# apple/ml-stable-diffusion

Measured on AMD Instinct MI355X. Metric: diffusion iter/s (UNet steps/s), SD2.1-base 512x512 fp16, higher is better.
Workload: dtype fp16; 1 GPU; BASELINE config 2: SD2.1-base (865.9 M-parameter UNet), random-init, denoising iteration at 512x512 (64x64 latents), CFG batch 2 per prompt, DDIM, device-resident loop; unet=sd21-base, latent=64, attention=ORIGINAL, prompts_per_gpu=1, global_batch=2, hip_graph=True, parallelism=dp1 (independent prompts per rank, no data-path collective)

## Files before the change

### include/sd_mi355x.h

```cpp
#ifndef SD_MI355X_H
#define SD_MI355X_H

#include <stddef.h>
#include <stdint.h>

#ifdef __cplusplus
extern "C" {
#endif

typedef enum sd_status {
  SD_OK = 0,
  SD_ERR_INVALID_ARGUMENT = -1,
  SD_ERR_NOT_FOUND = -2,
  SD_ERR_HIP = -3,
  SD_ERR_UNSUPPORTED = -4,
  SD_ERR_INTERNAL = -5
} sd_status;

typedef enum sd_dtype { SD_F16 = 0, SD_F32 = 1 } sd_dtype;

typedef enum sd_attention_impl {
  SD_ATTN_ORIGINAL = 0,
  SD_ATTN_SPLIT_EINSUM = 1,
  SD_ATTN_SPLIT_EINSUM_V2 = 2
// ... 154 lines not shown
                      const void* res, void* out, int B, int Cin, int C1, int H, int W, int Cout, int ksize, int upsample, int nw,
                      int* plan_out, int iters, float* ms);
int sd_op_w8a8_pack(const int8_t* wq, int Cout, int Ctot, int ksize, int8_t* stream, size_t* bytes);
int sd_op_conv2d_w8a8_halo(const void* x, const void* x1, const int8_t* wq, const float* w_scale, float act_absmax, const float* bias,
                           const float* temb, const void* res, void* out, int B, int Cin, int C1, int H, int W, int Cout, int upsample,
                           int staging, int splitk, int* plan_out, int iters, float* ms);
int sd_op_w8a8_pack_halo(const int8_t* wq, int Cout, int Ctot, int8_t* packed, size_t* bytes);
int sd_op_subpixel_fold(const void* w, int w_f32, int Cout, int Cin, void* folded, size_t* halves);
int sd_op_subpixel_refusal(int ksize, int stride, int up, int C0, int C1, int N, int B, int Hi, int Wi, int out_mode, char* text, int text_bytes);
int sd_op_conv2d_subpixel(const void* x, const void* w, const float* bias, const void* res, void* out, int B, int Cin, int H, int W, int Cout,
                          int splitk, int staging, int* plan_out, int iters, float* ms);
int sd_op_gemm_w8a8(const void* x, const int8_t* wq, const float* w_scale, float act_absmax, const float* bias, const void* res, void* out, int B,
                    int Cin, int H, int W, int Cout, int bm, int* plan_out, int iters, float* ms);
int sd_op_w8a8_pack_gemm(const int8_t* wq, int Cout, int K, int8_t* packed, size_t* bytes);
int sd_op_layernorm_q8(const void* x, const float* ln_weight, const float* ln_bias, float act_absmax, float eps, int8_t* xq, int M, int C,
                       int iters, float* ms);
int sd_op_geglu_w8a8(const int8_t* xq, const int8_t* wq, const float* w_scale, float act_absmax, const float* bias, void* out, int M, int C,
                     int N2, int bm, int* plan_out, int iters, float* ms);
int sd_op_w8a8_pack_geglu(const int8_t* wq, int N2, int K, int8_t* packed, size_t* bytes);
int sd_op_qkv_w8a8(const int8_t* xq, const int8_t* wq, const float* w_scale, float act_absmax, const float* bias, void* out_qk, void* out_vt,
                   int B, int HW, int C, float q_scale, int vt_perm, int bm, int* plan_out, int iters, float* ms);
int sd_op_w8a8_pack_qkv(const int8_t* wq, int C, int8_t* packed, size_t* bytes);
int sd_op_quantize_weight(const float* w, int Cout, size_t per_row, int8_t* q, float* w_scale, double* sq_err);
int sd_op_absmax(const void* x, size_t n, float* absmax);
int sd_op_gemm_palettized(const void* x, const void* lut, int nbits, const uint8_t* indices, const float* bias, const void* res, void* out,
                          int B, int Cin, int H, int W, int Cout, int bm, int* plan_out, int iters, float* ms);
int sd_op_palette_pack_gemm(const uint8_t* indices, int Cout, int K, int nbits, uint8_t* stream, size_t* bytes);
int sd_op_geglu_palettized(const void* x, const float* ln_weight, const float* ln_bias, const void* lut, int nbits, const uint8_t* indices,
                           const float* bias, void* out, int M, int C, int N2, float eps, int bm, int* plan_out, int iters, float* ms);
int sd_op_palette_pack_geglu(const uint8_t* indices, int N2, int K, int nbits, uint8_t* stream, size_t* bytes);
int sd_op_conv2d_groupnorm(const void* x, const void* w, const float* bias, const void* res, const float* gn_weight,
                           const float* gn_bias, void* conv_out, void* out, int B, int Cin, int H, int W, int Cout, int ksize,
                           int groups, float eps, int silu, int tile, int producer_stats, int* entries, int iters, float* ms);
int sd_op_conv2d_groupnorm_proj(const void* x, const void* w, const float* bias, const void* res, const float* gn_weight,
                                const float* gn_bias, const void* proj_w, const float* proj_bias, void* conv_out, void* out, int B,
                                int Cin, int H, int W, int Cout, int ksize, int Nproj, int groups, float eps, int fold, int tile,
                                int* entries, int iters, float* ms);
int sd_op_conv2d_groupnorm_conv3x3(const void* x, const void* w, const float* bias, const void* res, const float* gn_weight,
                                   const float* gn_bias, const void* w2, const float* bias2, const void* res2, void* conv_out, void* out,
                                   int B, int Cin, int H, int W, int Cout, int ksize, int N2, int groups, float eps, int silu, int fold,
                                   int tile, int staging2, int* entries, int iters, float* ms);
int sd_op_ffn_out_proj(const void* g, const void* w1, const float* b1, const void* res1, const void* w2, const float* b2, const void* res2,
                       void* out, float* gn_sums, int B, int C, int S, int groups, int fused, int iters, float* ms);
int sd_op_fold_linear(const void* wp, const float* bp, const void* w2, const float* b2, void* wm_out, float* bm_out, int N, int J, int K);
int sd_op_cross_attention_fused(const void* x, const float* ln_weight, const float* ln_bias, const void* wq, const void* k,
                                const void* v, void* out, int B, int heads, int Sq, int Sk, float eps, int nst, int iters,
                                float* ms);
int sd_op_cross_attention_block(const void* x, const float* ln_weight, const float* ln_bias, const void* wq, const void* k, const void* v,
                                const void* wo, const float* bo, const void* a1, const void* wo1, const float* bo1, void* out, int B, int heads,
                                int Sq, int Sk, float eps, int fused, int iters, float* ms);
int sd_op_geglu(const void* x, const void* w, const float* bias, void* out, int M, int C, int N2, int iters, float* ms);
int sd_op_geglu_ln(const void* x, const float* ln_weight, const float* ln_bias, const void* w, const float* bias, void* out, int M, int C,
                   int N2, float eps, int kernel, int iters, float* ms);
int sd_op_qkv_ln(const void* x, const float* ln_weight, const float* ln_bias, const void* w, void* out_qk, void* out_vt, int B, int HW, int C,
                 float eps, float q_scale, int vt_perm, int kernel, int iters, float* ms);
int sd_op_gn_proj_qkv(const void* x_in, const void* conv_w, const float* gn_weight, const float* gn_bias, const void* proj_w,
                      const float* proj_bias, const float* ln_weight, const float* ln_bias, const void* wqkv, void* out_h, void* out_qk,
                      void* out_vt, int B, int H, int W, int C, int groups, float gn_eps, float ln_eps, float q_scale, int vt_perm, int fused,
                      int* entries, int iters, float* ms);
int sd_op_timestep_embedding(const float* t, float* out, int n, int dim, int flip_sin_to_cos, float freq_shift);
int sd_op_posterior_noise(const float* moments, const float* eps, const float* noise, float* out, int Cz, int h, int w, int n_images,
                          float scale_factor, float sa, float sb, int iters, float* ms);
int sd_op_sched_step(const float* noise_pred, float* latents, float* hist, const float* coef, const float* pred, const float* step_noise,
                     float guidance, int cfg, int history, int n_images, int n, float* denoised, int* step_after);
int sd_op_conv_plan(int ksize, int stride, int up, int C0, int C1, int N, int B, int Ho, int Wo, int out_mode, int flags, int n_trans,
                    int n_twins, int gnf_groups, int tile, int staging, int splitk, int copies, int* plan, unsigned long long* workspace_bytes);
int sd_op_conv_plan_kernel(int ksize, int stride, int up, int C0, int C1, int N, int B, int Ho, int Wo, int out_mode, int flags, int n_trans,
                           int n_twins, int gnf_groups, int tile, int staging, int splitk, int copies, char* text, int text_bytes);
int sd_numpy_randn(uint32_t seed, double* out, size_t n);
int sd_torch_randn(uint32_t seed, double* out, size_t n);
int sd_philox_randn(uint64_t seed, uint32_t offset, double* out, size_t n);
int sd_calibrate(int device, float* out9);
int sd_selftest_mfma(void);

typedef struct sd_safety_checker_config {
  int32_t batch, image_size , patch_size , hidden_size, intermediate_size,
          num_hidden_layers, num_attention_heads, projection_dim, num_concepts ,
          num_special , hidden_act ;
  float layer_norm_eps;
  int32_t use_graph;
} sd_safety_checker_config;
typedef struct sd_safety_checker sd_safety_checker;
int sd_safety_checker_create(const sd_safety_checker_config* cfg, const sd_weights* w, int device, sd_safety_checker** out);
void sd_safety_checker_destroy(sd_safety_checker* c);
size_t sd_safety_checker_device_bytes(const sd_safety_checker* c);
int sd_safety_checker_run(sd_safety_checker* c, const void* clip_input, float adjustment, float* has_nsfw,
                          float* concept_scores, float* image_embeds, float* last_hidden_state, int flags);
float sd_safety_checker_last_ms(const sd_safety_checker* c);
int sd_op_vit_attention(const void* qkv, void* out, int B, int S, int heads, int d, int iters, float* ms);
int sd_op_safety_head(const float* image_embeds, const float* concept_embeds, const float* special_embeds,
                      const float* concept_w, const float* special_w, float adjustment, int B, int P,
                      int n_concepts, int n_special, float* has_nsfw, float* concept_scores);

typedef struct sd_image_post {
  int32_t resize_h, resize_w;
  float image_mean[3], image_std[3];
} sd_image_post;
int sd_vae_decode_images(sd_unet* vae, const void* z, sd_dtype z_dtype, float* image, uint8_t* rgb8, sd_safety_checker* checker,
                         const sd_image_post* post, float adjustment, float* has_nsfw, float* concept_scores, int flags);
int sd_op_resample_coeffs(int in_size, int out_size, int* ksize, int32_t* bounds, int32_t* coeffs);
int sd_op_image_rgb8(const float* image, uint8_t* rgb8, int B, int H, int W, int iters, float* ms);
int sd_op_clip_input(const uint8_t* rgb8, void* clip_input, int B, int H, int W, int rh, int rw, int S, const float* mean3,
                     const float* std3, int iters, float* ms);

int sd_op_conv_f32(const float* x, const void* w, int w_kind, const float* bias, const float* res, float* out, int B, int Cin,
                   int H, int W, int N, int ksize, int stride, int upsample, int pad_mode);
int sd_op_groupnorm_f32(const float* x, const float* gamma, const float* beta, float* out, int B, int C, int H, int W, int groups,
                        float eps, int silu);
// ... 16 lines not shown
```

### ml-stable-diffusion_amd/csrc/capi_ops.cpp

```cpp
#include <algorithm>
#include <climits>
#include <cmath>
#include <cstring>
#include <initializer_list>

#include "capi_util.h"
#include "conv_plan.h"
#include "weight_prep.h"

namespace sd {
namespace {

const half_t* f16(const void* p) { return reinterpret_cast<const half_t*>(p); }

half_t* upload_nhwc(Scratch& sc, const void* x, int B, int C, int H, int W) {
  const half_t* src = f16(x);
  std::vector<half_t> t((size_t)B * C * H * W);
  for (int b = 0; b < B; ++b)
    for (int c = 0; c < C; ++c)
      for (int p = 0; p < H * W; ++p) t[((size_t)b * H * W + p) * C + c] = src[((size_t)b * C + c) * H * W + p];
  return sc.dev<half_t>(t.size(), t.data());
}
half_t* upload_tokens(Scratch& sc, const void* x, int B, int C, int S) { return upload_nhwc(sc, x, B, C, 1, S); }

// ... 1237 lines not shown
}

int sd_op_geglu_palettized(const void* x, const float* ln_weight, const float* ln_bias, const void* lut, int nbits, const uint8_t* indices,
                           const float* bias, void* out, int M, int C, int N2, float eps, int bm, int* plan_out, int iters, float* ms) {
  return guarded([&] {
    SD_REQUIRE(palette_bits_ok(nbits), kInvalidArgument, "geglu_palettized: nbits = %d, not one of 1, 2, 4, 6, 8", nbits);
    SD_REQUIRE(bm == 0 || bm == 128 || bm == 256, kInvalidArgument, "geglu_palettized: bm = %d, not 0, 128 or 256", bm);
    SD_REQUIRE(x && lut && indices && out && plan_out, kInvalidArgument, "NULL argument");
    SD_REQUIRE(M > 0 && C > 0 && N2 > 0, kInvalidArgument, "geglu_palettized: empty problem");
    SD_REQUIRE((ln_weight == nullptr) == (ln_bias == nullptr), kInvalidArgument, "geglu_palettized: ln_weight and ln_bias go together");
    palette_check_indices("geglu_palettized", indices, (size_t)N2 * C, nbits);
    static const float present = 0.f;
    ConvDesc d = token_gemm(nullptr, C, nullptr, &present, nullptr, nullptr, 1, M, N2);
    if (ln_weight) d.ln_colsum = &present;
    d.ln_eps = eps;
    d.out_mode = kOutGeglu;
    SD_REQUIRE(conv_fast_path_ok(d) && smgeglu_pal_shape_ok(d, conv_plan_pin(WeightSource::PalGeglu, bm).staging), kInvalidArgument,
               "geglu_palettized: shape not eligible for plan tile 16 (smgeglu.hip: M=%d C=%d N2=%d bm=%d - 128-row tiles only (256 is not "
               "built), C a multiple of 64 up to 2560, N2 of 160, M of 128, at least 2 x 2 tiles and a multiple of 8 of them)", M, C, N2, bm);
    std::vector<half_t> w((size_t)N2 * C), wf(w.size());
    for (size_t i = 0; i < w.size(); ++i) w[i] = f16(lut)[indices[i]];
    std::vector<float> bf(N2), cs(N2);
    fold_layernorm_rows(w.data(), bias, ln_weight, ln_bias, N2, C, 0, true, wf.data(), cs.data(), bf.data());
    Scratch sc;
    half_t* dout = sc.dev<half_t>((size_t)M * (N2 / 2));
    d.x0 = sc.dev<half_t>((size_t)M * C, f16(x));
    d.out = dout;
    d.bias = sc.dev<float>(N2, bf.data());
    HostWeights h;
    h.kind = WeightSource::PalGeglu; h.lut = lut; h.indices = indices; h.bits = nbits;
    upload_compressed(sc, d, "geglu_palettized", h, bm);
    if (ln_weight) {
      d.ln_colsum = sc.dev<float>(N2, cs.data());
      d.cw.ln_gamma = sc.dev<float>(C, ln_weight);
    }
    const ConvPlan p = conv_plan(d);
    plan_out[0] = p.tile; plan_out[1] = p.staging; plan_out[2] = p.splitk; plan_out[3] = p.slab ? 1 : 0;
    ConvWorkspace ws;
    sc.timed(iters, ms, [&] { launch_conv(d, ws, sc.stream); });
    SD_HIP(hipMemcpy(out, dout, (size_t)M * (N2 / 2) * 2, hipMemcpyDeviceToHost));
  });
}

int sd_op_palette_pack_geglu(const uint8_t* indices, int N2, int K, int nbits, uint8_t* stream, size_t* bytes) {
  return guarded([&] {
    SD_REQUIRE(indices && bytes, kInvalidArgument, "NULL argument");
    SD_REQUIRE(palette_bits_ok(nbits) && N2 > 0 && K > 0 && N2 % 32 == 0 && K % 64 == 0, kInvalidArgument,
               "palette_pack_geglu: nbits %d N2 %d K %d", nbits, N2, K);
    *bytes = smgemm_pal_bytes(N2, K, nbits);
    if (stream) smgeglu_pal_pack(indices, N2, K, nbits, stream);
  });
}

int sd_op_qkv_ln(const void* x, const float* ln_weight, const float* ln_bias, const void* w, void* out_qk, void* out_vt, int B, int HW, int C,
                 float eps, float q_scale, int vt_perm, int kernel, int iters, float* ms) {
  return guarded([&] {
    SD_REQUIRE(x && ln_weight && ln_bias && w && out_qk && out_vt && B >= 1 && HW >= 1 && C % 64 == 0 && kernel >= 0 && kernel <= 9,
               kInvalidArgument, "bad q|k|v arguments");
    Scratch sc;
    const int N = 3 * C, M = B * HW;
    const FoldedProj f = upload_ln_folded(sc, w, nullptr, ln_weight, ln_bias, N, C, false);
    half_t* dqk = sc.dev<half_t>((size_t)M * 2 * C);
    half_t* dvt = sc.dev<half_t>((size_t)B * C * HW);
    ConvDesc d = qkv_desc(sc.dev<half_t>((size_t)M * C, f16(x)), f, eps, dqk, dvt, B, 1, HW, C, q_scale, vt_perm);
    SD_REQUIRE(conv_fast_path_ok(d), kUnsupported, "q|k|v shape off the MFMA path (C=%d)", C);
    const ConvWeightCopies copies = conv_plan_copies(d);
    if (kernel == 2 || (kernel == 0 && copies.wsgemm)) {
      SD_REQUIRE(wsgemm_shape_ok(d), kInvalidArgument, "q|k|v shape not eligible for plan tile 10 (wsgemm.hip)");
      tile_for_wsgemm(sc, d);
      if (kernel == 2) d.tile = 10;
    } else if (kernel >= 3 || (kernel == 0 && copies.bvgemm)) {
      tile_for_bvgemm(sc, d, "q|k|v shape not eligible for plan tile 11 (bvgemm.hip)");
      if (kernel >= 3) {
        d.tile = 11;
        d.staging = kernel - 3;
      }
    }
    ConvWorkspace ws;
    sc.timed(iters, ms, [&] { launch_conv(d, ws, sc.stream); });
    SD_HIP(hipMemcpy(out_qk, dqk, (size_t)M * 2 * C * 2, hipMemcpyDeviceToHost));
    SD_HIP(hipMemcpy(out_vt, dvt, (size_t)B * C * HW * 2, hipMemcpyDeviceToHost));
  });
}

int sd_op_gn_proj_qkv(const void* x_in, const void* conv_w, const float* gn_weight, const float* gn_bias, const void* proj_w,
                      const float* proj_bias, const float* ln_weight, const float* ln_bias, const void* wqkv, void* out_h, void* out_qk,
                      void* out_vt, int B, int H, int W, int C, int groups, float gn_eps, float ln_eps, float q_scale, int vt_perm, int fused,
                      int* entries, int iters, float* ms) {
  return guarded([&] {
    SD_REQUIRE(x_in && conv_w && gn_weight && gn_bias && proj_w && proj_bias && ln_weight && ln_bias && wqkv && out_h && out_qk && out_vt,
               kInvalidArgument, "NULL argument");
    const int HW = H * W, M = B * HW, N = 3 * C;
    SD_REQUIRE(gn_proj_qkv_ok(C, C / 64, HW, M, HW, groups), kInvalidArgument, "gn_proj_qkv: C=%d HW=%d groups=%d", C, HW, groups);
    Scratch sc;
    half_t* dx = sc.dev<half_t>((size_t)M * C);
    ConvDesc d = conv_desc(upload_nhwc(sc, x_in, B, C, H, W), C, sc.dev<half_t>((size_t)C * C, f16(conv_w)), nullptr, nullptr, dx, B, H, W, C);
    d.splitk = 1;
    float* partial = poisoned_gn_partial(sc, B, HW, groups);
    d.gn_partial = partial;
    d.gn_groups = groups;
    float* dgw = sc.dev<float>(C, gn_weight);
    float* dgb = sc.dev<float>(C, gn_bias);
    const FoldedProj fq = upload_ln_folded(sc, wqkv, nullptr, ln_weight, ln_bias, N, C, false);
    half_t* dwp = sc.dev<half_t>((size_t)C * C, f16(proj_w));
    float* dpb = sc.dev<float>(C, proj_bias);
    half_t* dnorm = sc.dev<half_t>((size_t)M * C);
    half_t* dh = sc.dev<half_t>((size_t)M * C);
    half_t* dqk = sc.dev<half_t>((size_t)M * 2 * C);
    half_t* dvt = sc.dev<half_t>((size_t)B * C * HW);
    half_t* dwp_t = sc.dev<half_t>((size_t)C * C);
    half_t* dwq_t = sc.dev<half_t>((size_t)N * C);
    launch_xattn_out_retile_nk(dwp, dwp_t, C, C, sc.stream);
    launch_xattn_out_retile_nk(fq.w, dwq_t, N, C, sc.stream);
    ConvDesc pd = conv_desc(dnorm, C, dwp, dpb, nullptr, dh, B, H, W, C);
    ConvDesc qd = qkv_desc(dh, fq, ln_eps, dqk, dvt, B, H, W, C, q_scale, vt_perm);
    SD_REQUIRE(conv_fast_path_ok(d) && conv_fast_path_ok(pd) && conv_fast_path_ok(qd), kInvalidArgument, "gn_proj_qkv: off the MFMA path");
    ConvWorkspace ws = workspace_for(sc, {d, pd, qd});
    int n_entries = 0;
    static const bool want_clk = tune_env_set("SD_GQ_CLOCK");
    const size_t n_clk = (size_t)(M / 32) * 5 * 16;
// ... 19 lines not shown
        launch_gn_proj_qkv(g, sc.stream);
      } else {
        launch_groupnorm(dx, C, nullptr, 0, partial, dgw, dgb, dnorm, B, HW, groups, gn_eps, 0, sc.stream, n_entries);
        launch_conv(pd, ws, sc.stream);
        launch_conv(qd, ws, sc.stream);
      }
    });
    if (entries) *entries = (fused && n_entries >= 1 && n_entries <= 128) ? n_entries : 0;
    if (dclk) {
      std::vector<long long> hc(n_clk);
      SD_HIP(hipMemcpy(hc.data(), dclk, n_clk * sizeof(long long), hipMemcpyDeviceToHost));
      static const char* names[13] = {"start -> group statistics folded", "-> constants in LDS", "-> normalised tile in LDS", "-> proj_in MFMAs issued",
                                      "-> h tile in LDS", "-> q MFMAs", "-> q stored", "-> k MFMAs", "-> k stored", "-> v MFMAs", "-> V^T stored", "", ""};
      const size_t nw = n_clk / 16;
      double total = 0;
      for (int ph = 1; ph <= 11; ++ph) {
        double sum = 0, mx = 0;
        for (size_t w = 0; w < nw; ++w) {
          const double dlt = (double)(hc[w * 16 + ph] - hc[w * 16 + ph - 1]);
          sum += dlt;
          mx = std::max(mx, dlt);
        }
        total += sum / nw;
        fprintf(stderr, "gn_proj_qkv phase %2d  mean %8.0f  max %8.0f cycles   %s\n", ph, sum / nw, mx, names[ph - 1]);
      }
      fprintf(stderr, "gn_proj_qkv mean wave %8.0f cycles (%zu waves; the XCDs' counters are not synchronised: no launch-wide span)\n", total, nw);
    }
    SD_HIP(hipMemcpy(out_h, dh, (size_t)M * C * 2, hipMemcpyDeviceToHost));
    SD_HIP(hipMemcpy(out_qk, dqk, (size_t)M * 2 * C * 2, hipMemcpyDeviceToHost));
    SD_HIP(hipMemcpy(out_vt, dvt, (size_t)B * C * HW * 2, hipMemcpyDeviceToHost));
  });
}

static ConvPlan query_conv_plan(int ksize, int stride, int up, int C0, int C1, int N, int B, int Ho, int Wo, int out_mode, int flags, int n_trans,
                                int n_twins, int gnf_groups, int tile, int staging, int splitk, int copies, ConvWeightCopies& c) {
  SD_REQUIRE(ksize >= 1 && stride >= 1 && up >= 1 && C0 >= 1 && C1 >= 0 && N >= 1 && B >= 1 && Ho >= 1 && Wo >= 1 &&
                 n_trans >= 0 && n_twins >= 0 && n_twins <= 2 && gnf_groups >= 0 && copies >= -1 && copies <= 7,
             kInvalidArgument, "bad conv_plan arguments");
  static const float present[4] = {};
  const half_t* ph = reinterpret_cast<const half_t*>(present);
  ConvDesc d;
  d.x0 = d.w = ph;
  d.C0 = C0;
  if (C1 > 0) d.x1 = ph, d.C1 = C1;
  d.B = B; d.Ho = Ho; d.Wo = Wo; d.Hi = Ho * stride / up; d.Wi = Wo * stride / up;
  d.ksize = ksize; d.stride = stride; d.up = up; d.N = N; d.out_mode = out_mode;
  if (flags & 1) d.ln_colsum = present;
  if (flags & 2) d.temb = present;
  if (flags & 4) d.res = ph;
  if (flags & 8) d.gn_partial = const_cast<float*>(present), d.gn_groups = 32;
  if (flags & 16) d.bias = present;
  if (flags & 32) d.pad = 0;
  if (flags & 64) d.subpix = true;
  if (n_trans > 0) d.out_t = const_cast<half_t*>(ph), d.n_trans = n_trans, d.ldT = Ho * Wo;
  d.n_twins = n_twins;
  if (gnf_groups > 0) {
    d.gnf_partial = d.gnf_gamma = d.gnf_beta = present;
    d.gnf_groups = gnf_groups;
    d.gnf_entries = 1;
    d.gnf_silu = ksize == 3 ? 1 : 0;
  }
  d.tile = tile; d.staging = staging; d.splitk = splitk;
  if (tile == 17) {
    d.w = nullptr;
    d.cw.kind = WeightSource::I8Wstream;
    d.cw.stream = d.cw.scale = present;
    d.cw.inv_s = 1.f;
  }
  if (tile == 18) {
    d.w = nullptr;
    d.cw.kind = WeightSource::I8Halo;
    d.cw.stream = d.cw.scale = present;
    d.cw.inv_s = 1.f;
  }
  if (tile == 19) {
    d.w = nullptr;
    d.cw.kind = WeightSource::I8Gemm;
    d.cw.stream = d.cw.scale = present;
    d.cw.inv_s = 1.f;
  }
  if (tile == 20) {
    d.w = nullptr;
    d.cw.kind = WeightSource::I8Geglu;
    d.cw.stream = d.cw.scale = present;
    d.cw.inv_s = 1.f;
    d.x0_i8 = reinterpret_cast<const int8_t*>(present);
  }
  if (tile == 22) {
    d.w = nullptr;
    d.cw.kind = WeightSource::I8Qkv;
    d.cw.stream = d.cw.scale = present;
    d.cw.inv_s = 1.f;
    d.x0_i8 = reinterpret_cast<const int8_t*>(present);
  }
  c = conv_plan_copies(d);
  if (copies < 0) copies = (c.wstream ? 1 : 0) | (c.wsgemm ? 2 : 0) | (c.bvgemm ? 4 : 0);
  if (copies & 1) d.w_tiled = ph;
  if (copies & 2) d.w_ws = ph;
  if (copies & 4) d.w_bv = ph;
  return conv_plan(d);
}

int sd_op_conv_plan(int ksize, int stride, int up, int C0, int C1, int N, int B, int Ho, int Wo, int out_mode, int flags, int n_trans,
                    int n_twins, int gnf_groups, int tile, int staging, int splitk, int copies, int* plan, unsigned long long* workspace_bytes) {
  return guarded([&] {
    SD_REQUIRE(plan && workspace_bytes, kInvalidArgument, "bad conv_plan arguments");
// ... 477 lines not shown
```

### ml-stable-diffusion_amd/csrc/conv_plan.cpp

```cpp
#include "conv_plan.h"

#include <algorithm>
#include <cstring>

namespace sd {

namespace {

constexpr int BK = kConvBK;

struct Dims {
  int Ctot, M, N, K, HoWo, nk_total, tiles_x, tiles_y;
};
Dims dims_of(const ConvDesc& d) {
  Dims a;
  a.Ctot = d.C0 + (d.x1 ? d.C1 : 0);
  a.M = d.B * d.Ho * d.Wo;
  a.N = d.N;
  a.K = d.ksize * d.ksize * a.Ctot;
  a.HoWo = d.Ho * d.Wo;
  a.nk_total = a.K / BK;
  a.tiles_x = cdiv(d.Wo, 16);
  a.tiles_y = cdiv(d.Ho, 8);
  return a;
}

struct Switches {
  bool wstream, wsgemm, bvgemm, smgemm, smgeglu, reduce_stats, tuning, qkv_i8;
};
const Switches& switches() {
  static const Switches s = {tune_env_int("SD_WSTREAM", 1) != 0, tune_env_int("SD_WSGEMM", 1) != 0, tune_env_int("SD_BVGEMM", 1) != 0,
                             tune_env_int("SD_SMGEMM", 1) != 0, tune_env_int("SD_SMGEGLU", 1) != 0, tune_env_int("SD_REDUCE_STATS", 0) != 0,
                             getenv("SD_TUNE") != nullptr, tune_env_int("SD_QKV_I8", 1) != 0};
  return s;
}

struct Plan {
  int tile;
  int splitk;
  int staging = 0;
};

bool can_split(const ConvDesc& d) { return d.out_mode == kOutHalf && !d.ln_colsum && !d.out_t; }
bool can_stream(const ConvDesc& d) { return d.w_tiled != nullptr && can_split(d) && wstream_shape_ok(d); }
bool pal_stream(const ConvDesc& d) { return d.cw.kind == WeightSource::PalWstream; }
bool i8_stream(const ConvDesc& d) { return d.cw.kind == WeightSource::I8Wstream; }
bool i8_halo(const ConvDesc& d) { return d.cw.kind == WeightSource::I8Halo; }
bool halo_i8_ok(const ConvDesc& d) {
  return halo_ks_ok(d) && can_split(d) && !d.gnf_partial && !d.debug && d.C0 + (d.x1 ? d.C1 : 0) <= kHaloI8MaxCtot;
}
bool pal_gemm(const ConvDesc& d) { return d.cw.kind == WeightSource::PalGemm; }
bool pal_geglu(const ConvDesc& d) { return d.cw.kind == WeightSource::PalGeglu; }
bool i8_gemm(const ConvDesc& d) { return d.cw.kind == WeightSource::I8Gemm; }
bool i8_geglu(const ConvDesc& d) { return d.cw.kind == WeightSource::I8Geglu; }
bool i8_qkv(const ConvDesc& d) { return d.cw.kind == WeightSource::I8Qkv; }
int wstream_waves(int code) { return code == 4 ? 4 : 8; }
size_t slab_bytes(const Dims& a, int splits, bool slab) { return (splits > 1 || slab) ? (size_t)splits * a.M * a.N * sizeof(float) : 0; }

struct TunedConv { int kind, ksize, stride, up, ctot, n, m, tile, staging, splitk; };
#if __has_include("tuned_convs.inc")
static const TunedConv kTuned[] = {
#include "tuned_convs.inc"
};
static const int kNumTuned = sizeof(kTuned) / sizeof(kTuned[0]);
#else
static const TunedConv* kTuned = nullptr;
static const int kNumTuned = 0;
#endif

bool parse_plan_row(const char* line, TunedConv& r) {
  return sscanf(line, " {%d, %d, %d, %d, %d, %d, %d, %d, %d, %d}", &r.kind, &r.ksize, &r.stride, &r.up, &r.ctot, &r.n, &r.m, &r.tile,
                &r.staging, &r.splitk) == 10;
}
std::vector<TunedConv>& runtime_table() {
  static std::vector<TunedConv> table = [] {
    std::vector<TunedConv> t;
    const char* path = tune_env_set("SD_PLAN_TABLE") ? getenv("SD_PLAN_TABLE") : nullptr;
    if (!path) return t;
    FILE* f = fopen(path, "r");
    if (!f) {
      fprintf(stderr, "[sd] SD_PLAN_TABLE=%s cannot be opened - ignored\n", path);
      return t;
    }
    char line[512];
    while (fgets(line, sizeof(line), f)) {
      TunedConv r;
// ... 148 lines not shown
bool subpixel_wanted(const ConvDesc& d) {
  static const int mode = tune_env_int("SD_UP_SUBPIX", 1);
  if (mode == 0 || !halo_sp_ok(d)) return false;
  const int M = d.B * d.Ho * d.Wo;
  static const int only_m = tune_env_int("SD_UP_SUBPIX_M", 0);
  if (mode >= 2) return only_m == 0 || only_m == M;
  struct Shape { int ctot, n, m; };
  static const Shape kMeasured[] = {
      {1280, 1280, 2048},
      {640, 640, 8192},
      {0, 0, 0}};
  for (const Shape& s : kMeasured)
    if (s.ctot == d.C0 && s.n == d.N && s.m == M && s.ctot != 0) return true;
  return false;
}

bool gemm_pipe_ok(int ksize, int stride, int up, int M, int N, int K, int C0, int C1) {
  const size_t lim = (size_t)1 << 31;
  return ksize == 1 && stride == 1 && up == 1 && (size_t)M * std::max(C0, C1) * 2 < lim && (size_t)N * K * 2 < lim;
}

bool conv_fast_path_ok(const ConvDesc& d) {
  const int c1 = d.x1 ? d.C1 : 0;
  if (d.C0 % BK != 0 || c1 % BK != 0) return false;
  if (d.N % 4 != 0) return false;
  if (d.out_mode == kOutGeglu && d.N % 64 != 0) return false;
  if (!(d.ksize == 1 || d.ksize == 3)) return false;
  if (!(d.up == 1 || d.up == 2)) return false;
  return true;
}

int smqkv_i8_bm(const ConvDesc& d, int variant) {
  if (variant == 1) return 128;
  if (variant == 2) return 256;
  const long M = (long)d.B * d.Ho * d.Wo;
  return M % 128 == 0 && M / 128 * (d.N / kSmQkvCols) <= 256 ? 128 : 256;
}
bool smqkv_i8_shape_ok(const ConvDesc& d, int variant) { return smqkv_i8_tiles(d, variant) && d.C0 <= kSmI8MaxK; }
bool smqkv_i8_tiles(const ConvDesc& d, int variant) {
  if (variant < 0 || variant > 2) return false;
  if (!(d.ksize == 1 && d.stride == 1 && d.up == 1 && !d.x1 && d.out_mode == kOutHalf && !d.ln_colsum && !d.temb && !d.res && !d.gnf_partial &&
        !d.gn_partial && d.n_twins == 0 && !d.debug && !d.prof && !d.subpix))
    return false;
  const int C = d.C0;
  if (!(C >= 640 && C % kSmQkvCols == 0 && C % 64 == 0 && d.N == 3 * C && d.n_trans == 2 * C && (d.q_cols == 0 || d.q_cols == C)))
    return false;
  const long S = (long)d.Ho * d.Wo, M = d.B * S;
  if (!(S % 16 == 0 && d.ldT >= S && d.ldT % 8 == 0)) return false;
  const int bm = smqkv_i8_bm(d, variant);
  const long mt = M / bm, nt = d.N / kSmQkvCols;
  return M % bm == 0 && mt >= 2 && (mt * nt) % 8 == 0 && mt * nt <= 65535;
}

namespace {

int subpix_splits(const ConvDesc& d, const Dims& a) {
  const int steps = a.Ctot / BK;
  int s = d.splitk;
  if (s == 0) {
    const long blocks = 4L * d.B * cdiv(d.Wi, 16) * cdiv(d.Hi, 8) * cdiv(a.N, 64);
    s = 1;
    while (blocks * s < 192 && s < 16 && steps / (s * 2) >= 2) s *= 2;
  }
  s = std::min(std::max(s, 1), steps);
  return cdiv(steps, cdiv(steps, s));
}

ConvPlan plan_codes(const ConvDesc& d) {
  const CompressedWeights& cw = d.cw;
  if (i8_halo(d))
    SD_REQUIRE(conv_fast_path_ok(d) && cw.stream && cw.scale && halo_i8_ok(d), kInvalidArgument,
               "plan tile 18 (conv3x3_halo_i8.hip, int8) needs the int8 weights, the scales and a 3x3 / stride-1 shape of the halo conv with "
               "at most %d input channels (k=%d stride=%d up=%d C0=%d C1=%d N=%d)", kHaloI8MaxCtot, d.ksize, d.stride, d.up, d.C0, d.x1 ? d.C1 : 0, d.N);
  if (i8_gemm(d))
    SD_REQUIRE(conv_fast_path_ok(d) && cw.stream && cw.scale && d.staging >= 0 && d.staging <= 2 && smgemm_i8_shape_ok(d, d.staging), kInvalidArgument,
               "plan tile 19 (smgemm_i8.hip, int8) needs the int8 weights, the scales and a single-source shape of the small-M GEMM with K <= %d "
               "(k=%d C0=%d C1=%d N=%d M=%d mode=%d)", kSmI8MaxK, d.ksize, d.C0, d.x1 ? d.C1 : 0, d.N, d.B * d.Ho * d.Wo, d.out_mode);
  if (i8_geglu(d))
    SD_REQUIRE(conv_fast_path_ok(d) && cw.stream && cw.scale && d.staging >= 0 && d.staging <= 2 && smgeglu_i8_shape_ok(d, d.staging), kInvalidArgument,
               "plan tile 20 (smgeglu_i8.hip, int8) needs the int8 weights, the scales and an un-folded shape of the GEGLU kernel with K <= %d "
               "(k=%d C0=%d C1=%d N=%d M=%d mode=%d ln=%d)", kSmI8MaxK, d.ksize, d.C0, d.x1 ? d.C1 : 0, d.N, d.B * d.Ho * d.Wo, d.out_mode, d.ln_colsum ? 1 : 0);
  if (i8_qkv(d))
    SD_REQUIRE(conv_fast_path_ok(d) && switches().qkv_i8 && cw.stream && cw.scale && d.staging >= 0 && d.staging <= 2 && smqkv_i8_shape_ok(d, d.staging),
               kInvalidArgument,
               "plan tile 22 (smqkv_i8.hip, int8) needs the int8 weights, the scales and an un-folded q|k|v shape of its tiles with K <= %d "
               "(k=%d C0=%d C1=%d N=%d n_trans=%d M=%d S=%d mode=%d ln=%d%s)", kSmI8MaxK, d.ksize, d.C0, d.x1 ? d.C1 : 0, d.N, d.n_trans,
               d.B * d.Ho * d.Wo, d.Ho * d.Wo, d.out_mode, d.ln_colsum ? 1 : 0, switches().qkv_i8 ? "" : "; SD_QKV_I8=0");
  if (d.subpix) {
    SD_REQUIRE(conv_fast_path_ok(d) && halo_sp_ok(d) && (d.tile == 0 || d.tile == 21), kInvalidArgument,
               "plan tile 21 (conv3x3_halo_sp.hip) does not take this conv: %s (k=%d stride=%d up=%d C0=%d C1=%d N=%d %dx%d tile=%d)",
               halo_sp_refusal(d) ? halo_sp_refusal(d) : "another tile is pinned", d.ksize, d.stride, d.up, d.C0, d.x1 ? d.C1 : 0, d.N, d.Hi, d.Wi, d.tile);
    const Dims a = dims_of(d);
    ConvPlan r{21, d.staging ? d.staging : 3, 1, false, 0};
    r.splitk = subpix_splits(d, a);
    r.slab = r.splitk > 1;
    r.workspace_bytes = slab_bytes(a, r.splitk, r.slab);
    return r;
  }
  if (!conv_fast_path_ok(d)) return ConvPlan{-1, 0, 1, false, 0};
  switch (cw.kind) {
    case WeightSource::Fp16: break;
    case WeightSource::PalWstream:
    case WeightSource::I8Wstream: {
      const bool i8 = i8_stream(d);
      SD_REQUIRE(cw.stream && (i8 ? cw.scale != nullptr : cw.lut != nullptr) && can_split(d) && wstream_shape_ok(d), kInvalidArgument, "%s",
                 i8 ? "plan tile 17 (wstream.hip, int8) needs the int8 stream, the scales and a shape of the weight stream"
                    : "plan tile 14 (wstream.hip, palettized) needs the index stream, the LUT and a shape of the weight stream");
      ConvPlan r{i8 ? 17 : 14, d.staging, 1, true, 0};
      r.splitk = wstream_splits(d, wstream_waves(d.staging));
      r.workspace_bytes = slab_bytes(dims_of(d), r.splitk, true);
      return r;
    }
    case WeightSource::I8Halo: {
      const Dims a = dims_of(d);
      const Plan p = choose_plan(d, a);
      ConvPlan r{18, p.staging, 1, true, 0};
      const int steps = a.Ctot / BK;
      r.splitk = cdiv(steps, cdiv(steps, p.splitk));
      r.slab = r.splitk > 1 || d.n_twins > 0;
      r.workspace_bytes = slab_bytes(a, r.splitk, r.slab);
      return r;
    }
    case WeightSource::PalGemm:
      SD_REQUIRE(cw.stream && cw.lut && palette_bits_ok(cw.bits) && !d.x1 && d.staging >= 0 && d.staging <= 2 && smgemm_shape_ok(d, d.staging), kInvalidArgument,
                 "plan tile 15 (smgemm.hip, palettized) needs the index stream, the LUT and a single-source shape of the small-M GEMM");
      return ConvPlan{15, smgemm_bm(d, d.staging) == 32 ? 1 : 2, 1, false, 0};
    case WeightSource::I8Gemm:
      return ConvPlan{19, smgemm_bm(d, d.staging) == 32 ? 1 : 2, 1, false, 0};
    case WeightSource::PalGeglu:
      SD_REQUIRE(cw.stream && cw.lut && palette_bits_ok(cw.bits) && (cw.ln_gamma != nullptr) == (d.ln_colsum != nullptr) && smgeglu_pal_shape_ok(d, d.staging),
                 kInvalidArgument,
                 "plan tile 16 (smgeglu.hip, palettized) needs the index stream, the LUT, the norm weight with the LayerNorm fold and a shape of "
                 "the GEGLU kernel with 128-row tiles");
      return ConvPlan{16, 1, 1, false, 0};
    case WeightSource::I8Geglu:
      return ConvPlan{20, smgeglu_bm(d, d.staging) == 128 ? 1 : 2, 1, false, 0};
    case WeightSource::I8Qkv:
      return ConvPlan{22, smqkv_i8_bm(d, d.staging) == 128 ? 1 : 2, 1, false, 0};
  }
  const Switches& sw = switches();
  const bool free_choice = d.tile == 0 && d.splitk == 0 && d.staging == 0 && g_tune.tile == 0;
  if (d.w_ws && wsgemm_shape_ok(d) && (d.tile == 10 || (sw.wsgemm && free_choice && wsgemm_wanted(d)))) return ConvPlan{10, 0, 1, false, 0};
  SD_REQUIRE(d.tile != 10, kInvalidArgument, "plan tile 10 (wsgemm.hip) needs the pre-tiled weights and an eligible GEGLU shape");
  if (sw.bvgemm && d.w_bv && free_choice && bvgemm_wanted(d)) return ConvPlan{11, 0, 1, false, 0};
  if (d.tile == 11) {
    SD_REQUIRE(d.w_bv && bvgemm_shape_ok(d), kInvalidArgument, "plan tile 11 (bvgemm.hip) needs the pre-tiled weights and an eligible 1x1 shape");
    return ConvPlan{11, d.staging, 1, false, 0};
  }
  if (d.tile == 12 || (sw.smgemm && free_choice && smgemm_wanted(d))) return ConvPlan{12, d.tile == 12 ? d.staging : 0, 1, false, 0};
  if (d.tile == 13 || (sw.smgeglu && free_choice && smgeglu_wanted(d))) return ConvPlan{13, d.tile == 13 ? d.staging : 0, 1, false, 0};

  const Dims a = dims_of(d);
  Plan p = choose_plan(d, a);
  const bool twins = d.n_twins > 0;
  if (d.gnf_partial && d.ksize == 3) {
    SD_REQUIRE(conv_gn_loader_ok(d) && d.gnf_silu == 1 && d.gnf_gamma && d.gnf_beta && d.gnf_entries >= 1 && d.gnf_entries <= 128 && !twins, kInvalidArgument,
               "GroupNorm in the conv loader: Ctot=%d groups=%d entries=%d up=%d", a.Ctot, d.gnf_groups, d.gnf_entries, d.up);
    p.tile = 7;
    if (p.staging != 2 && p.staging != 3) p.staging = 3;
    p.splitk = 1;
  } else if (d.gnf_partial) {
    SD_REQUIRE(d.ksize == 1 && d.stride == 1 && !d.x1 && d.out_mode == kOutHalf && !d.ln_colsum && !d.out_t && !twins &&
                   gemm_pipe_ok(d.ksize, d.stride, d.up, a.M, a.N, a.K, d.C0, 0) &&
                   d.gnf_gamma && d.gnf_beta && d.gnf_groups >= 1 && d.gnf_groups <= 32 && a.K % d.gnf_groups == 0 && a.K <= 2048 &&
                   d.gnf_entries >= 1 && d.gnf_entries <= 128 && a.HoWo % 64 == 0,
               kInvalidArgument, "GroupNorm fold: K=%d groups=%d entries=%d HoWo=%d", a.K, d.gnf_groups, d.gnf_entries, a.HoWo);
    p.tile = 3;
    if (p.staging != 6 && p.staging != 7 && p.staging != 8) p.staging = 6;
    p.splitk = 1;
  }
  ConvPlan r{p.tile, p.staging, 1, true, 0};
  if (p.tile == 9) {
    r.splitk = wstream_splits(d, wstream_waves(p.staging));
  } else {
    const int steps = p.tile == 7 ? a.Ctot / BK : a.nk_total;
    r.splitk = cdiv(steps, cdiv(steps, p.splitk));
    r.slab = r.splitk > 1 || twins;
  }
  r.workspace_bytes = slab_bytes(a, r.splitk, r.slab);
  return r;
}

void decode_plan(const ConvDesc& d, ConvPlan& p) {
  const Dims a = dims_of(d);
  int code = p.staging;
  switch (p.tile) {
    case -1: p.kernel = ConvKernel::Generic; return;
    case 9: case 14: case 17:
      p.kernel = p.tile == 9 ? ConvKernel::Wstream : p.tile == 14 ? ConvKernel::WstreamPal : ConvKernel::WstreamI8;
      p.waves = wstream_waves(code);
      return;
    case 10: p.kernel = ConvKernel::Wsgemm; return;
    case 11:
      p.kernel = ConvKernel::Bvgemm;
      p.variant = code >= 1 && code <= 6 ? code : bvgemm_auto_variant(d);
      return;
    case 12: case 15: case 19:
      p.kernel = p.tile == 12 ? ConvKernel::Smgemm : p.tile == 15 ? ConvKernel::SmgemmPal : ConvKernel::SmgemmI8;
      p.bm = code >= 0 && code <= 2 ? smgemm_bm(d, code) : 0;
      return;
    case 13: case 16: case 20:
      p.kernel = p.tile == 13 ? ConvKernel::Smgeglu : p.tile == 16 ? ConvKernel::SmgegluPal : ConvKernel::SmgegluI8;
      p.bm = code >= 0 && code <= 2 ? smgeglu_bm(d, code) : 0;
      return;
    case 22:
      p.kernel = ConvKernel::SmqkvI8;
      p.bm = code >= 0 && code <= 2 ? smqkv_i8_bm(d, code) : 0;
      return;
    default: break;
  }
  if (p.tile == 18) {
    tile_dims(7, p.bm, p.bn);
    p.kernel = ConvKernel::HaloI8;
    p.stages = code >= 3 ? 4 : code == 2 ? 3 : 2;
    return;
  }
  if (p.tile == 21) {
    tile_dims(7, p.bm, p.bn);
    p.kernel = ConvKernel::HaloSubpix;
    p.stages = code == 2 ? 3 : 4;
    return;
  }
  tile_dims(p.tile, p.bm, p.bn);
  if (p.tile == 7) {
    p.kernel = ConvKernel::HaloKs;
    if (d.gnf_partial) p.stages = code >= 3 && halo_gnl_lds_bytes(4, a.Ctot) <= kLdsBudget ? 4 : 3;
    else p.stages = code >= 5 ? 8 : code == 4 ? 6 : code == 3 ? 4 : code == 2 ? 3 : 2;
    return;
  }
  p.kernel = ConvKernel::Igemm;
  p.stages = 2;
  const bool lnf = d.ln_colsum != nullptr;
  auto fits = [&](int nst, int kgroups = 1) { return ring_fits(p.bm, p.bn, nst, kgroups); };
  if (lnf && code == 1) code = 0;
  if (code == 1) {
    p.reg_staged = true;
    return;
  }
  if (!lnf && d.out_mode == kOutHalfT) {
    if (code >= 2) p.stages = 3;
    return;
  }
  if (code == 12 || code == 13) {
    const bool two_groups = !lnf && cdiv(a.nk_total, p.splitk) >= 4;
    if (two_groups && code == 13 && fits(4, 2)) p.stages = 4, p.kgroups = 2;
    else if (two_groups && fits(3, 2)) p.stages = 3, p.kgroups = 2;
    if (p.kgroups == 2) return;
    code -= 10;
  }
  if (code >= 6 && code <= 8 && gemm_pipe_ok(d.ksize, d.stride, d.up, a.M, a.N, a.K, d.C0, d.x1 ? d.C1 : 0)) {
    p.kernel = ConvKernel::GemmPipe;
    p.stages = code == 8 ? 2 : (code == 7 && fits(4)) ? 4 : 3;
    return;
  }
  if (code >= 6) code = 3;
  const int asked = code >= 5 ? 8 : code == 4 ? 6 : code == 3 ? 4 : code == 2 ? 3 : 2;
  for (int nst : {8, 6, 4, 3, 2})
    if (nst <= asked && fits(nst)) {
      p.stages = nst;
      return;
    }
}

}

ConvPlan conv_plan(const ConvDesc& d) {
  ConvPlan p = plan_codes(d);
  decode_plan(d, p);
  return p;
}

std::string conv_plan_kernel_name(const ConvPlan& p) {
  const std::string tile = std::to_string(p.bm) + "x" + std::to_string(p.bn), ring = " ring" + std::to_string(p.stages);
  switch (p.kernel) {
    case ConvKernel::Igemm: return "igemm " + tile + ring + (p.kgroups == 2 ? " kg2" : "") + (p.reg_staged ? " regs" : "");
    case ConvKernel::GemmPipe: return "gemm_pipe " + tile + ring;
    case ConvKernel::HaloKs: return "halo_ks" + ring;
    case ConvKernel::HaloI8: return "halo_i8" + ring;
    case ConvKernel::HaloSubpix: return "conv3x3_halo_sp" + ring;
    case ConvKernel::Wstream: return "wstream waves" + std::to_string(p.waves);
    case ConvKernel::WstreamPal: return "wstream_pal waves" + std::to_string(p.waves);
    case ConvKernel::WstreamI8: return "wstream_i8 waves" + std::to_string(p.waves);
    case ConvKernel::Wsgemm: return "wsgemm";
    case ConvKernel::Bvgemm: return "bvgemm v" + std::to_string(p.variant);
    case ConvKernel::Smgemm: return "smgemm bm" + std::to_string(p.bm);
    case ConvKernel::SmgemmPal: return "smgemm_pal bm" + std::to_string(p.bm);
    case ConvKernel::SmgemmI8: return "smgemm_i8 bm" + std::to_string(p.bm);
    case ConvKernel::Smgeglu: return "smgeglu bm" + std::to_string(p.bm);
    case ConvKernel::SmgegluPal: return "smgeglu_pal bm" + std::to_string(p.bm);
    case ConvKernel::SmgegluI8: return "smgeglu_i8 bm" + std::to_string(p.bm);
    case ConvKernel::SmqkvI8: return "smqkv_i8 bm" + std::to_string(p.bm);
    default: return "generic";
  }
}

size_t conv_workspace_bytes(const ConvDesc& d) {
  if (!conv_fast_path_ok(d) || pal_gemm(d) || pal_geglu(d) || i8_gemm(d) || i8_geglu(d) || i8_qkv(d)) return 0;
  const Dims a = dims_of(d);
  if (d.subpix) return halo_sp_ok(d) ? slab_bytes(a, subpix_splits(d, a), false) : 0;
  const Plan p = choose_plan(d, a);
  int splits = (switches().tuning && can_split(d)) ? std::max(p.splitk, 16) : p.splitk;
  const bool stream = can_stream(d) || ((pal_stream(d) || i8_stream(d)) && can_split(d) && wstream_shape_ok(d));
  if (stream) splits = std::max(splits, wstream_splits(d, 4));
  return slab_bytes(a, splits, d.n_twins > 0 || stream);
}

ConvWeightCopies conv_plan_copies(const ConvDesc& d0) {
  ConvWeightCopies c{false, false, false};
  if (!conv_fast_path_ok(d0) || d0.subpix) return c;
  ConvDesc d = d0;
  d.w_tiled = d.w_ws = d.w_bv = nullptr;
  const Switches& sw = switches();
  const int k = d.ksize, M = d.B * d.Ho * d.Wo;
  const bool ws_candidate = sw.tuning ? ((k == 3 && M <= 512) || (k == 1 && M <= 128)) : plan_is_wstream(d);
  c.wstream = sw.wstream && wstream_shape_ok(d) && ws_candidate;
  c.wsgemm = sw.wsgemm && wsgemm_wanted(d);
  c.bvgemm = sw.bvgemm && !c.wsgemm && bvgemm_wanted(d);
  return c;
}

namespace {
ConvPlan fp16_plan(const ConvDesc& d0, const ConvWeightCopies& c) {
  static const half_t present = 0;
  ConvDesc d = d0;
  d.cw = CompressedWeights{};
  d.w_tiled = c.wstream ? &present : nullptr;
  d.w_ws = c.wsgemm ? &present : nullptr;
  d.w_bv = c.bvgemm ? &present : nullptr;
  return conv_plan(d);
}
}

WeightPin conv_plan_pin(WeightSource kind, int n) {
  switch (kind) {
    case WeightSource::PalWstream: return {kind, 14, n == 4 ? 4 : 0};
    case WeightSource::I8Wstream: return {kind, 17, n == 4 ? 4 : 0};
    case WeightSource::I8Halo: return {kind, 18, n};
    case WeightSource::PalGemm: return {kind, 15, n == 32 ? 1 : n == 64 ? 2 : 0};
    case WeightSource::I8Gemm: return {kind, 19, n == 32 ? 1 : n == 64 ? 2 : 0};
    case WeightSource::PalGeglu: return {kind, 16, n == 128 ? 1 : n == 256 ? 2 : 0};
    case WeightSource::I8Geglu: return {kind, 20, n == 128 ? 1 : n == 256 ? 2 : 0};
    case WeightSource::I8Qkv: return {kind, 22, n == 128 ? 1 : n == 256 ? 2 : 0};
    default: return {};
  }
}

WeightPin conv_plan_weights(const ConvDesc& d, StoredWeights held, bool opt_in) {
  if (held == StoredWeights::Fp16 || !conv_fast_path_ok(d)) return {};
  const Switches& sw = switches();
  const bool palette = held == StoredWeights::Palette, one_by_one = opt_in && palette && d.ksize == 1 && !d.x1;
  if (one_by_one && d.out_mode == kOutGeglu && sw.smgeglu) {
    const ConvPlan p = fp16_plan(d, conv_plan_copies(d));
    if (p.kernel == ConvKernel::Smgeglu && smgeglu_pal_shape_ok(d, 0)) return conv_plan_pin(WeightSource::PalGeglu, p.bm);
  }
  if (opt_in && held == StoredWeights::W8A8 && d.ksize == 1 && !d.x1 && d.out_mode == kOutGeglu && sw.smgeglu) {
    const ConvPlan p = fp16_plan(d, conv_plan_copies(d));
    ConvDesc plain = d;
    plain.ln_colsum = nullptr;
    if (p.kernel == ConvKernel::Smgeglu && smgeglu_i8_shape_ok(plain, p.bm == 128 ? 1 : 2)) return conv_plan_pin(WeightSource::I8Geglu, p.bm);
  }
  if (opt_in && held == StoredWeights::W8A8 && d.ksize == 1 && !d.x1 && d.out_mode == kOutHalf && d.n_trans > 0 && sw.qkv_i8) {
    ConvDesc plain = d;
// ... 12 lines not shown
  if (opt_in && held == StoredWeights::W8A8 && d.ksize == 1 && !d.x1 && d.out_mode == kOutHalf && sw.smgemm && !d.ln_colsum) {
    const ConvPlan p = fp16_plan(d, conv_plan_copies(d));
    if (p.kernel == ConvKernel::Smgemm && smgemm_i8_shape_ok(d, 0)) return conv_plan_pin(WeightSource::I8Gemm, p.bm);
  }
  if (held == StoredWeights::W8A8 && halo_i8_ok(d)) {
    const ConvPlan p = fp16_plan(d, conv_plan_copies(d));
    if (p.kernel == ConvKernel::HaloKs) {
      WeightPin pin = conv_plan_pin(WeightSource::I8Halo, p.staging);
      pin.splitk = p.splitk;
      return pin;
    }
  }
  return {};
}

bool conv_plan_is_tuned(const ConvDesc& d) {
  if (!conv_fast_path_ok(d)) return false;
  const Dims a = dims_of(d);
  for (int i = 0; i < kNumTuned; ++i)
    if (table_match(kTuned[i], d, a)) return true;
  return false;
}

int conv_plan_table_set(const char* text) {
  std::vector<TunedConv>& t = runtime_table();
  t.clear();
  if (!text) return 0;
  const char* p = text;
  while (*p) {
    const char* e = strchr(p, '\n');
    std::string line(p, e ? (size_t)(e - p) : strlen(p));
    TunedConv r;
    if (parse_plan_row(line.c_str(), r)) t.push_back(r);
    if (!e) break;
    p = e + 1;
  }
  return (int)t.size();
}

void conv_tune_set_candidate(int tile, int staging, int splitk) {
  g_tune.tile = tile;
  g_tune.staging = staging;
  g_tune.splitk = splitk;
}

void conv_plan_log(const ConvDesc& d, const ConvPlan& p, int n_fast) {
  static const bool on = tune_env_set("SD_LOG_CONVS");
  if (!on) return;
  const Dims a = dims_of(d);
  const int c1 = d.x1 ? d.C1 : 0;
  if (p.tile == 9 || p.tile == 14 || p.tile == 17)
    fprintf(stderr, "[sd conv] k%d up%d C0=%d C1=%d M=%d N=%d K=%d tile=%d nw=%d slabs=%d twins=%d bits=%d\n", d.ksize, d.up, d.C0, c1, a.M, a.N,
            a.K, p.tile, p.waves, p.splitk, d.n_twins, p.tile == 14 ? d.cw.bits : p.tile == 17 ? 8 : 16);
  else if (p.tile == 12 || p.tile == 13)
    fprintf(stderr, "[sd conv] k1 s1 up1 C0=%d C1=%d M=%d N=%d K=%d mode=%d tile=%d bm=%d n_fast=%d\n", d.C0, c1, a.M, a.N, a.K, d.out_mode, p.tile, p.bm,
            n_fast);
  else if (p.tile == 15 || p.tile == 16)
    fprintf(stderr, "[sd conv] k1 s1 up1 C0=%d C1=%d M=%d N=%d K=%d mode=%d tile=%d bm=%d n_fast=%d bits=%d\n", d.C0, c1, a.M, a.N, a.K, d.out_mode,
            p.tile, p.bm, n_fast, d.cw.bits);
  else if (p.tile == 19 || p.tile == 20 || p.tile == 22)
    fprintf(stderr, "[sd conv] k1 s1 up1 C0=%d C1=%d M=%d N=%d K=%d mode=%d tile=%d bm=%d n_fast=%d bits=8\n", d.C0, c1, a.M, a.N, a.K, d.out_mode, p.tile,
            p.bm, n_fast);
  else if (p.tile == 18)
    fprintf(stderr, "[sd conv] k%d s%d up%d C0=%d C1=%d M=%d N=%d K=%d mode=%d tile=%d splitk=%d bits=8\n", d.ksize, d.stride, d.up, d.C0, c1, a.M, a.N,
            a.K, d.out_mode, p.tile, p.splitk);
  else if (p.tile == 21)
    fprintf(stderr, "[sd conv] k%d s%d up%d C0=%d C1=%d M=%d N=%d K=%d mode=%d tile=%d splitk=%d subpix K'=%d\n", d.ksize, d.stride, d.up, d.C0, c1, a.M,
            a.N, a.K, d.out_mode, p.tile, p.splitk, 4 * a.Ctot);
  else
    fprintf(stderr, "[sd conv] k%d s%d up%d C0=%d C1=%d M=%d N=%d K=%d mode=%d tile=%d splitk=%d\n", d.ksize, d.stride, d.up, d.C0, c1, a.M, a.N,
            a.K, d.out_mode, p.tile, p.splitk);
}

bool choose_tile_order(double a_bytes, double w_bytes, double nbm, double nbn, bool ab_switch) {
  const double l2 = 3.5e6;
  const double m_fast_cost = w_bytes + a_bytes * (a_bytes <= l2 ? std::min(8.0, nbn) : nbn);
  const double n_fast_cost = a_bytes + w_bytes * (w_bytes <= l2 ? std::min(8.0, nbm) : nbm);
  static const int forced = tune_env_int("SD_TILE_ORDER", -1);
  if (ab_switch && forced == 2) return nbn > 1 && a_bytes * (nbn - 1) > 7.0 * w_bytes;
  if (ab_switch && forced >= 0) return forced != 0;
  return nbn > 1 && n_fast_cost < m_fast_cost;
}

bool conv_reduce_stats_on() { return switches().reduce_stats; }

}
```

### ml-stable-diffusion_amd/csrc/conv_plan.h

```cpp
#pragma once
#include <string>

#include "kernels.h"

namespace sd {

enum class ConvKernel { Generic, Igemm, GemmPipe, HaloKs, HaloI8, HaloSubpix, Wstream, WstreamPal, WstreamI8, Wsgemm, Bvgemm, Smgemm, SmgemmPal, SmgemmI8, Smgeglu, SmgegluPal, SmgegluI8, SmqkvI8 };

struct ConvPlan {
  int tile;
  int staging;
  int splitk;
  bool slab;
  size_t workspace_bytes;
  ConvKernel kernel = ConvKernel::Generic;
  int bm = 0, bn = 0;
  int stages = 0;
  int kgroups = 1;
  bool reg_staged = false;
  int waves = 0;
  int variant = 0;
};
ConvPlan conv_plan(const ConvDesc& d);

struct ConvWeightCopies {
  bool wstream, wsgemm, bvgemm;
};
ConvWeightCopies conv_plan_copies(const ConvDesc& d);

enum class StoredWeights { Fp16, Palette, W8A8 };
struct WeightPin {
  WeightSource kind = WeightSource::Fp16;
  int tile = 0, staging = 0;
  int splitk = 0;
};
WeightPin conv_plan_weights(const ConvDesc& d, StoredWeights held, bool opt_in);
WeightPin conv_plan_pin(WeightSource kind, int n);

void conv_plan_log(const ConvDesc& d, const ConvPlan& p, int n_fast = 0);

std::string conv_plan_kernel_name(const ConvPlan& p);

bool choose_tile_order(double a_bytes, double w_bytes, double nbm, double nbn, bool ab_switch);

bool conv_reduce_stats_on();

constexpr int kConvBK = 64;
bool halo_ks_ok(const ConvDesc& d);
const char* halo_sp_refusal(const ConvDesc& d);
inline bool halo_sp_ok(const ConvDesc& d) { return halo_sp_refusal(d) == nullptr; }
bool subpixel_wanted(const ConvDesc& d);
bool gemm_pipe_ok(int ksize, int stride, int up, int M, int N, int K, int C0, int C1);

constexpr size_t kLdsBudget = 160 * 1024;
constexpr size_t ring_bytes(int bm, int bn, int nst) { return (size_t)nst * (bm + bn) * kConvBK * sizeof(half_t); }
constexpr bool ring_fits(int bm, int bn, int nst, int kgroups = 1) { return kgroups * ring_bytes(bm, bn, nst) + 2 * bn * sizeof(float) <= kLdsBudget; }
constexpr int kHaloLdsRows = 184;
constexpr size_t halo_lds_bytes(int bn, int d) {
  return ((size_t)2 * kHaloLdsRows * kConvBK + (size_t)d * bn * kConvBK) * sizeof(half_t) + bn * sizeof(float);
}
constexpr size_t halo_gnl_lds_bytes(int d, int ctot) {
  const size_t k_loop = halo_lds_bytes(64, d) - 64 * sizeof(float) + (((size_t)6 * ctot + 15) & ~(size_t)15);
  const size_t epilogue = 32 * 1024 + 128 * (64 + 8) * 2 + 64 * sizeof(float);
  return k_loop > epilogue ? k_loop : epilogue;
}
constexpr int kHaloI8Pitch = 20, kHaloI8Rows = 204;
constexpr size_t halo_i8_lds_bytes(int d) {
  return (size_t)kHaloLdsRows * kConvBK * sizeof(half_t) + (size_t)2 * kHaloI8Rows * kConvBK + (size_t)d * 64 * kConvBK + 2 * 64 * sizeof(float);
}
constexpr int kHaloI8MaxCtot = 14784;
static_assert(127LL * 127 * 9 * kHaloI8MaxCtot < (1LL << 31) && 127LL * 127 * 9 * (kHaloI8MaxCtot + 64) >= (1LL << 31), "int32 bound of plan tile 18");
constexpr int kSmI8MaxK = 133120;
static_assert(127LL * 127 * kSmI8MaxK < (1LL << 31) && 127LL * 127 * (kSmI8MaxK + 64) >= (1LL << 31), "int32 bound of plan tile 19");

constexpr int kSmQkvCols = 160;
bool smqkv_i8_shape_ok(const ConvDesc& d, int variant);
bool smqkv_i8_tiles(const ConvDesc& d, int variant);
int smqkv_i8_bm(const ConvDesc& d, int variant);

}
```

### ml-stable-diffusion_amd/csrc/igemm.hip

```cpp
#include "igemm_device.h"

namespace sd {

namespace {

template <int BM, int BN, int WGM, int WGN, bool TRANS_OUT, bool GLDS, int NST, int DBG = 0, bool LNF = false, int KG = 1>
__global__ __launch_bounds__(256 * KG) void igemm_kernel(IgemmArgs a) {
  static_assert(WGM * WGN == 4, "4 waves");
  static_assert(KG == 1 || (KG == 2 && GLDS && NST >= 3 && !LNF && !TRANS_OUT && DBG == 0), "in-workgroup split-K: ring variants of the plain epilogue");
  static_assert(!(LNF && TRANS_OUT), "LayerNorm fold uses the in-lane row layout of the non-transposed tile");
  constexpr int TM = BM / WGM / 32;
  constexpr int TN = BN / WGN / 32;
  constexpr int XR = BM / 32;
  constexpr int WR = BN / 32;
  constexpr int ROW = GLDS ? BK : LDS_ROW;

  const bool prof = (DBG & 4) && blockIdx.x == 0 && blockIdx.y == 0 && threadIdx.x == 0;
  long long prof_t[4];
  long long prof_w0 = 0;
  if (prof) { prof_t[0] = clock64(); prof_w0 = wall_clock64(); }
  extern __shared__ __attribute__((aligned(16))) char smem[];
  const int kg = KG > 1 ? __builtin_amdgcn_readfirstlane((int)threadIdx.x >> 8) : 0;
  half_t* Xs = reinterpret_cast<half_t*>(smem) + (size_t)kg * NST * (BM + BN) * ROW;
  half_t* Ws = Xs + NST * BM * ROW;
// ... 934 lines not shown
      a.gn_partial = d.gn_partial;
      a.gn_G = d.gn_groups;
      a.gn_cpg = a.N / d.gn_groups;
      a.gn_T = slabs;
      hipLaunchKernelGGL(splitk_reduce_stats_kernel, dim3(slabs, a.B), dim3(256), lds, s, a, ppb);
      return slabs;
    }
  }
  const size_t total4 = (size_t)a.M * a.N / 4;
  const int blocks = (int)std::min<size_t>((total4 + 255) / 256, 2048);
  hipLaunchKernelGGL(splitk_reduce_kernel, dim3(blocks), dim3(256), 0, s, a);
  return 0;
}

half_t* g_zero_chunk = nullptr;

}

const half_t* device_zero_chunk() {
  if (!g_zero_chunk) {
    SD_HIP(hipMalloc(reinterpret_cast<void**>(&g_zero_chunk), 256));
    SD_HIP(hipMemset(g_zero_chunk, 0, 256));
    SD_HIP(hipDeviceSynchronize());
  }
  return g_zero_chunk;
}

const half_t* zero_chunk() {
  SD_REQUIRE(g_zero_chunk, kInternal, "conv launch before any handle allocated the zero chunk (device_zero_chunk)");
  return g_zero_chunk;
}

int launch_conv(const ConvDesc& d, const ConvWorkspace& ws, hipStream_t s) {
  SD_REQUIRE(conv_fast_path_ok(d), kInvalidArgument, "launch_conv: shape not MFMA-tileable (C0=%d C1=%d N=%d k=%d)",
             d.C0, d.C1, d.N, d.ksize);
  SD_REQUIRE(!d.ln_colsum || (d.ksize == 1 && !d.x1 && d.bias && d.out_mode != kOutHalfT), kInvalidArgument,
             "LayerNorm fold needs a 1x1 single-source GEMM with a (folded) bias");
  SD_REQUIRE(!d.out_t || (d.out_mode == kOutHalf && d.n_trans % 64 == 0 && d.n_trans < d.N && (d.Ho * d.Wo) % 8 == 0 &&
                          d.ldT % 8 == 0 && !d.res && !d.temb),
             kInvalidArgument, "fused q|k|v: n_trans %d N %d HoWo %d ldT %d", d.n_trans, d.N, d.Ho * d.Wo, d.ldT);
  SD_REQUIRE(!d.vt_perm || (d.out_t && (d.Ho * d.Wo) % 16 == 0), kInvalidArgument, "permuted V^T needs the fused q|k|v epilogue and HoWo %% 16 == 0");
  SD_REQUIRE(d.q_cols == 0 || (d.out_t && d.q_cols % 4 == 0 && d.q_cols <= d.n_trans), kInvalidArgument, "pre-scaled queries need the fused q|k|v epilogue (q_cols %d)", d.q_cols);
  const ConvPlan p = conv_plan(d);
  switch (p.kernel) {
    case ConvKernel::Wsgemm: launch_wsgemm(d, s); return 0;
    case ConvKernel::Bvgemm: launch_bvgemm(d, p, s); return 0;
    case ConvKernel::Smgemm: launch_smgemm(d, p, s); return 0;
    case ConvKernel::Smgeglu: launch_smgeglu(d, p, s); return 0;
    case ConvKernel::SmgegluPal: launch_smgeglu_pal(d, p, s); return 0;
    case ConvKernel::SmgemmPal: launch_smgemm_pal(d, p, s); return 0;
    case ConvKernel::SmgemmI8: launch_smgemm_i8(d, p, s); return 0;
    case ConvKernel::SmgegluI8: launch_smgeglu_i8(d, p, s); return 0;
    case ConvKernel::SmqkvI8: launch_smqkv_i8(d, p, s); return 0;
    default: break;
  }
  IgemmArgs a = planned_args(d, p, ws.partial);
  const bool twins = d.n_twins > 0;
  SD_REQUIRE(!twins || (d.out_mode == kOutHalf && !d.ln_colsum && !d.out_t && !d.debug && reduce_twin_ok(a.HoWo, a.N, d.n_twins, d.twin)),
             kInvalidArgument, "GroupNorm twins need a plain fp16 output and whole (sample, group) slices (HoWo=%d N=%d)", a.HoWo, a.N);
  const bool have_ws = !p.slab || (ws.partial && ws.partial_bytes >= p.workspace_bytes);
  if (p.kernel == ConvKernel::Wstream || p.kernel == ConvKernel::WstreamPal || p.kernel == ConvKernel::WstreamI8) SD_REQUIRE(have_ws, kInternal, "wstream workspace too small (%zu < %zu)", ws.partial_bytes, p.workspace_bytes);
  SD_REQUIRE(have_ws, kInternal, "split-K workspace too small (%zu < %zu)", ws.partial_bytes, p.workspace_bytes);
  conv_plan_log(d, p);
  int gn_entries = 0;
  switch (p.kernel) {
    case ConvKernel::Wstream:
      launch_wstream(d, ws.partial, p.waves, s);
      break;
    case ConvKernel::WstreamPal:
      launch_wstream_pal(d, ws.partial, p.waves, s);
      break;
    case ConvKernel::WstreamI8:
      launch_wstream_i8(d, ws.partial, p.waves, s);
      break;
    case ConvKernel::HaloKs: gn_entries = launch_halo_ks(d, p, ws.partial, s); break;
    case ConvKernel::HaloI8: gn_entries = launch_halo_i8(d, p, ws.partial, s); break;
    case ConvKernel::HaloSubpix: gn_entries = launch_halo_sp(d, p, ws.partial, s); break;
    case ConvKernel::Igemm:
    case ConvKernel::GemmPipe: {
      const bool trans = d.out_mode == kOutHalfT;
      set_tile_order(a, p.bm, p.bn);
      if (d.debug && d.debug < 64) {
        const bool ok = p.bm == 128 && p.bn == 128 ? launch_debug_mode<128, 128>(a, d.debug, s) : launch_debug_mode<64, 64>(a, d.debug, s);
        SD_REQUIRE(ok && !trans, kInvalidArgument, "no ablation kernel for debug mode %d", d.debug);
        return 0;
      }
      if (!trans) gn_entries = setup_gn_stats(d, a, p.bm);
      if (p.bm == 128 && p.bn == 128) launch_tile<128, 128>(a, p, trans, s);
      else if (p.bm == 128) launch_tile<128, 64>(a, p, trans, s);
      else if (p.bn == 64) launch_tile<64, 64>(a, p, trans, s);
      else launch_tile<64, 128>(a, p, trans, s);
      break;
    }
    default: SD_REQUIRE(false, kInternal, "launch_conv: plan '%s' has no launcher here", conv_plan_kernel_name(p).c_str());
  }
  if (twins) {
    launch_reduce_twin(a.partial, a.splitk, a.M, a.N, a.HoWo, a.bias, a.temb, a.temb_stride, a.res, a.out, d.n_twins, d.twin, s);
  } else if (a.slab) {
    gn_entries = launch_slab_combine(d, a, s);
  }
  SD_HIP(hipGetLastError());
  return gn_entries;
}

bool gn_side_gemm_ok(const ConvDesc& d) {
  if (!(d.ksize == 1 && d.stride == 1 && d.up == 1 && d.out_mode == kOutHalf && !d.ln_colsum && !d.out_t && d.n_twins == 0 && !d.gnf_partial &&
// ... 57 lines not shown
```

### ml-stable-diffusion_amd/csrc/kernels.h

```cpp
#pragma once
#include "sd_common.h"

namespace sd {

enum OutMode : int {
  kOutHalf = 0,
  kOutHalfT = 1,
  kOutGeglu = 2,
};

struct GnTwin {
  half_t* y = nullptr;
  int ld = 0, c_off = 0;
  int cpg = 0;
  const float* gamma = nullptr;
  const float* beta = nullptr;
  float eps = 1e-5f;
  int silu = 0;
};

enum class WeightSource { Fp16, PalWstream, PalGemm, PalGeglu, I8Wstream, I8Halo, I8Gemm, I8Geglu, I8Qkv };
struct CompressedWeights {
  WeightSource kind = WeightSource::Fp16;
  const void* stream = nullptr;
// ... 3 lines not shown
  const float* scale = nullptr;
  float inv_s = 0.f;
  bool palettized() const { return kind == WeightSource::PalWstream || kind == WeightSource::PalGemm || kind == WeightSource::PalGeglu; }
  const uint8_t* pal() const { return palettized() ? static_cast<const uint8_t*>(stream) : nullptr; }
  bool int8() const { return kind == WeightSource::I8Wstream || kind == WeightSource::I8Halo || kind == WeightSource::I8Gemm || kind == WeightSource::I8Geglu || kind == WeightSource::I8Qkv; }
  const int8_t* i8() const { return int8() ? static_cast<const int8_t*>(stream) : nullptr; }
};

struct ConvDesc {
  const half_t* x0 = nullptr;
  const half_t* x1 = nullptr;
  const int8_t* x0_i8 = nullptr;
  int C0 = 0, C1 = 0;
  const half_t* w = nullptr;
  const float* bias = nullptr;
  const float* temb = nullptr;
  int temb_stride = 0;
  const half_t* res = nullptr;
  half_t* out = nullptr;
  int B = 1, Hi = 1, Wi = 1;
  int Ho = 1, Wo = 1;
  int ksize = 1, stride = 1, up = 1;
  int pad = -1;
  int N = 0;
  int out_mode = kOutHalf;
  int ldT = 0;
  int tile = 0;
  int splitk = 0;
  long long* prof = nullptr;
  int debug = 0;
  int staging = 0;
  const float* ln_colsum = nullptr;
  float ln_eps = 1e-5f;
  half_t* out_t = nullptr;
  int n_trans = 0;
  int vt_perm = 0;
  float q_scale = 1.f;
  int q_cols = 0;
  float* gn_partial = nullptr;
  int gn_groups = 0;
  const float* gnf_partial = nullptr;
  const float* gnf_gamma = nullptr;
  const float* gnf_beta = nullptr;
  float gnf_eps = 1e-6f;
  int gnf_groups = 0, gnf_entries = 0;
  int gnf_silu = 0;
  const half_t* w_tiled = nullptr;
  CompressedWeights cw;
  const half_t* w_ws = nullptr;
  const half_t* w_bv = nullptr;
  GnTwin twin[2];
  int n_twins = 0;
  bool subpix = false;
};

constexpr int kGnMaxSlabs = 256;

struct ConvWorkspace {
  float* partial = nullptr;
  size_t partial_bytes = 0;
};

size_t conv_workspace_bytes(const ConvDesc& d);
const half_t* device_zero_chunk();
int launch_conv(const ConvDesc& d, const ConvWorkspace& ws, hipStream_t s);
struct ConvPlan;
bool conv_fast_path_ok(const ConvDesc& d);
bool conv_gn_loader_ok(const ConvDesc& d);
void conv_tune_set_candidate(int tile, int staging, int splitk);
bool conv_plan_is_tuned(const ConvDesc& d);
int conv_plan_table_set(const char* text);

bool wstream_shape_ok(const ConvDesc& d);
int wstream_splits(const ConvDesc& d, int nw);
size_t wstream_tiled_halves(int N, int Ctot, int ksize);
void launch_wstream_retile(const half_t* w, half_t* wt, int N, int Ctot, int ksize, hipStream_t s);
int launch_wstream(const ConvDesc& d, float* partial, int nw, hipStream_t s);
int launch_wstream_pal(const ConvDesc& d, float* partial, int nw, hipStream_t s);
int launch_wstream_i8(const ConvDesc& d, float* partial, int nw, hipStream_t s);
bool reduce_twin_ok(int HW, int N, int n_twins, const GnTwin* tw);
void launch_reduce_twin(const float* partial, int S, int M, int N, int HW, const float* bias, const float* temb, int temb_stride,
                        const half_t* res, half_t* out, int n_twins, const GnTwin* tw, hipStream_t s);

bool wsgemm_shape_ok(const ConvDesc& d);
bool wsgemm_wanted(const ConvDesc& d);
size_t wsgemm_tiled_halves(int N);
void launch_wsgemm_retile(const half_t* w, half_t* wt, int N, bool geglu, hipStream_t s);
void launch_wsgemm(const ConvDesc& d, hipStream_t s);

bool bvgemm_shape_ok(const ConvDesc& d);
size_t bvgemm_tiled_halves(int N, int K);
void launch_bvgemm_retile(const half_t* w, half_t* wt, int N, int K, bool geglu, hipStream_t s);
void launch_bvgemm(const ConvDesc& d, const ConvPlan& p, hipStream_t s);
int bvgemm_auto_variant(const ConvDesc& d);
bool bvgemm_wanted(const ConvDesc& d);

bool smgemm_shape_ok(const ConvDesc& d, int variant);
bool smgemm_wanted(const ConvDesc& d);
void launch_smgemm(const ConvDesc& d, const ConvPlan& p, hipStream_t s);
int smgemm_bm(const ConvDesc& d, int variant);
void launch_smgemm_pal(const ConvDesc& d, const ConvPlan& p, hipStream_t s);
bool smgemm_i8_shape_ok(const ConvDesc& d, int variant);
void launch_smgemm_i8(const ConvDesc& d, const ConvPlan& p, hipStream_t s);

void launch_wfold(const half_t* wp, const float* bp, const half_t* w2, const float* b2, half_t* merged, float* bm, int N, int J, int K,
                  hipStream_t s);

bool smgeglu_shape_ok(const ConvDesc& d, int variant);
bool smgeglu_wanted(const ConvDesc& d);
int smgeglu_bm(const ConvDesc& d, int variant);
void launch_smgeglu(const ConvDesc& d, const ConvPlan& p, hipStream_t s);
size_t smgeglu_prof_entries(const ConvDesc& d, int variant);
bool smgeglu_pal_shape_ok(const ConvDesc& d, int variant);
void launch_smgeglu_pal(const ConvDesc& d, const ConvPlan& p, hipStream_t s);
bool smgeglu_i8_shape_ok(const ConvDesc& d, int variant);
void launch_smgeglu_i8(const ConvDesc& d, const ConvPlan& p, hipStream_t s);
void launch_smqkv_i8(const ConvDesc& d, const ConvPlan& p, hipStream_t s);

void run_calibration(int device, float* out);

int launch_conv_generic(const ConvDesc& d, int act_silu_out, hipStream_t s);

void launch_conv_small_n(const ConvDesc& d, float* out_nchw_f32, hipStream_t s);

enum AttnImpl : int { kAttnOriginal = 0, kAttnSplitEinsum = 1, kAttnSplitEinsumV2 = 2 };

struct AttnDesc {
  const half_t* q = nullptr;
  const half_t* k = nullptr;
  const half_t* vt = nullptr;
  half_t* out = nullptr;
  int B = 1, heads = 1, d = 64, Sq = 0, Sk = 0;
  int ldq = 0, ldk = 0, ldv = 0, ldo = 0;
  int impl = kAttnOriginal;
  int variant = 0;
  int vt_perm = 0;
  int q_prescaled = 0;
  float* sk_part = nullptr;
  size_t sk_part_bytes = 0;
  unsigned* sk_cnt = nullptr;
  int sk_cnt_n = 0;
  int sk_force = 0;
  int sk_upw = 0;
};
inline float attention_q_prescale(int d) { return 1.4426950408889634f / sqrtf((float)d); }
void launch_attention(const AttnDesc& d, hipStream_t s);
bool attention_supported(int d);
bool attention8_ok(const AttnDesc& d);
bool attention8_shape_ok(int d, int Sq, int Sk);
void launch_attention8(const AttnDesc& d, hipStream_t s);
bool attention8_sk_scratch(const AttnDesc& d, size_t* part_bytes, int* n_counters);

struct XAttnDesc {
  const half_t* x = nullptr;
  const half_t* wq = nullptr;
  const float* bias = nullptr;
  const float* colsum = nullptr;
  const half_t* k = nullptr;
  const half_t* vt = nullptr;
  half_t* out = nullptr;
  int M = 0, C = 0, S = 0, L = 0, ldv = 0, heads = 0;
  float ln_eps = 1e-5f;
  int impl = kAttnOriginal;
  int nst = 0;
};
bool xattn_fused_ok(int C, int heads, int S, int L);
void launch_xattn_fused(const XAttnDesc& d, hipStream_t s);

struct XAttnOutDesc {
  const half_t* x = nullptr;
// ... 77 lines not shown
void launch_groupnorm(const half_t* x0, int C0, const half_t* x1, int C1, float* partial, const float* gamma,
                      const float* beta, half_t* y, int B, int HW, int G, float eps, int silu, hipStream_t s,
                      int producer_entries = 0, const ConvDesc* side = nullptr);
bool gn_side_gemm_ok(const ConvDesc& d);
void launch_gn_apply_side(const half_t* x0, int C0, const half_t* x1, int C1, const float* partial, int entries, const float* gamma,
                          const float* beta, half_t* y, int B, int HW, int G, float eps, int silu, int slabs, int ppb, const ConvDesc& side,
                          hipStream_t s);
void launch_gn_fused_side(int vw, const half_t* x0, int C0, const half_t* x1, int C1, const float* gamma, const float* beta, half_t* y, int B,
                          int HW, int G, float eps, int silu, const ConvDesc& side, hipStream_t s);
bool groupnorm_wants_producer_stats(int HW, int C, int G);

void launch_row_softmax(half_t* x, int rows, int cols, float scale, hipStream_t s);

struct ConvF32Desc {
  const float* x = nullptr;
  const void* w = nullptr;
  int w_kind = 0;
  const float* bias = nullptr;
  const float* res = nullptr;
  float* out = nullptr;
  int B = 1, Hi = 1, Wi = 1, Cin = 0, Ho = 1, Wo = 1, N = 0;
  int ksize = 1, stride = 1, up = 1;
  int pad = -1;
};
void launch_conv_f32(const ConvF32Desc& d, hipStream_t s);
size_t groupnorm_f32_scratch_bytes(int B, int G);
void launch_groupnorm_f32(const float* x, void* scratch, const float* gamma, const float* beta, float* y, int B, int HW, int C, int G,
                          float eps, int silu, hipStream_t s);
void launch_row_softmax_f32(float* x, int rows, int cols, float scale, hipStream_t s);
void launch_nchw_to_nhwc_f32(const void* src, int src_is_f32, float* dst, int B, int C, int H, int W, hipStream_t s);
void launch_nhwc_to_nchw_f32f32(const float* src, float* dst, int B, int C, int H, int W, hipStream_t s);

std::vector<float> timestep_freq_table(int dim, float freq_shift);
void launch_timestep_embedding(const float* t, const float* freq, float* out, int n, int dim, hipStream_t s);
void launch_gemv(const half_t* w, const float* bias, const float* x, int ldx, float* out, int ldo, int B, int N,
                 int K, int silu_in, int silu_out, int accumulate, hipStream_t s);
void launch_nchw_to_nhwc(const void* src, int src_is_f32, half_t* dst, int B, int C, int H, int W, hipStream_t s);
void launch_nhwc_to_nchw_f32(const half_t* src, float* dst, int B, int C, int H, int W, hipStream_t s);
void launch_half_to_float(const half_t* src, float* dst, size_t n, hipStream_t s);
void launch_float_to_half(const float* src, half_t* dst, size_t n, hipStream_t s);
void launch_add_half(const half_t* a, const half_t* b, half_t* y, size_t n, hipStream_t s);
void launch_sum_half(const half_t* const* srcs, int nsrc, half_t* y, size_t n, hipStream_t s);
void launch_bc1s_to_tokens(const half_t* src, half_t* dst, int B, int C, int S, hipStream_t s);

struct LoopTables {
  const float* timesteps;
  const float* coef;
  int* step;
  const float* in_scale;
  unsigned* ticket;
  const float* temb_tab;
  float* temb_dst;
  int temb_rows, temb_ld, temb_n;
  const float* noise_tab = nullptr;
  const float* pred = nullptr;
  float* denoised = nullptr;
};
void launch_loop_prep(const float* latents, half_t* sample, float* tbuf, LoopTables t, int Bimg, int C, int H,
                      int W, int cfg, hipStream_t s);
void launch_cfg_sched_step(const float* noise_pred, float* latents, float* eps_hist, LoopTables t, float guidance,
                           int Bimg, int CHW, int cfg, int hist, hipStream_t s);

void launch_posterior_noise(const float* moments, const float* eps, const float* noise, float* out, size_t n, int n_images,
                            float scale, float sa, float sb, hipStream_t s);

void launch_image_rgb8(const float* image, uint8_t* rgb8, int B, int H, int W, hipStream_t s);
constexpr int kResampleBits = 22;
int resample_ksize(int in_size, int out_size);
void resample_coeffs(int in_size, int out_size, int32_t* bounds, int32_t* coeffs);
struct ClipInputPlan {
  int H = 0, W = 0, rh = 0, rw = 0, S = 0, ksh = 0, ksv = 0;
  std::vector<int32_t> hbounds, hcoeffs, vbounds, vcoeffs;
  size_t lds_bytes = 0;
};
ClipInputPlan plan_clip_input(int H, int W, int rh, int rw, int S);
struct ClipInputDesc {
  const int32_t *hbounds, *hcoeffs, *vbounds, *vcoeffs;
  int H, W, S, top, left, ksh, ksv;
  float mean[3], std[3];
};
void launch_clip_input(const uint8_t* rgb8, half_t* out, int B, const ClipInputDesc& d, size_t lds_bytes, hipStream_t s);

void launch_absmax_half(const half_t* x0, size_t n0, const half_t* x1, size_t n1, float* slot, hipStream_t s);

void launch_lds_poison(hipStream_t s);
void launch_count_nonfinite_half(const void* p, size_t bytes, unsigned long long* out, hipStream_t s);

}
```

### ml-stable-diffusion_amd/csrc/misc.hip

```cpp
#include <cmath>
#include <cstdint>

#include "kernels.h"

namespace sd {
namespace {

__global__ void timestep_embedding_kernel(const float* __restrict__ t, const float* __restrict__ freq,
                                          float* __restrict__ out, int n, int dim) {
  const int half = dim / 2;
  const int idx = blockIdx.x * blockDim.x + threadIdx.x;
  if (idx >= n * half) return;
  const int row = idx / half, i = idx - row * half;
  const float arg = t[row] * freq[i];
  out[(size_t)row * dim + i] = cosf(arg);
  out[(size_t)row * dim + half + i] = sinf(arg);
}

__device__ __forceinline__ float silu_f(float v) {
  return v * __builtin_amdgcn_rcpf(1.0f + __builtin_amdgcn_exp2f(-1.4426950408889634f * v));
}

template <int CTRL>
__device__ __forceinline__ float dpp_mov(float x) {
  return __builtin_bit_cast(float, __builtin_amdgcn_update_dpp(0, __builtin_bit_cast(int, x), CTRL, 0xF, 0xF, true));
}
__device__ __forceinline__ float wave_sum(float v) {
  v += dpp_mov<0xB1>(v);
  v += dpp_mov<0x4E>(v);
  v += dpp_mov<0x141>(v);
  v += dpp_mov<0x140>(v);
  const unsigned u = __float_as_uint(v);
  const auto r = __builtin_amdgcn_permlane16_swap(u, u, false, false);
  const unsigned r0 = r[0], r1 = r[1];
  v = __uint_as_float(r0) + __uint_as_float(r1);
  const unsigned u2 = __float_as_uint(v);
  const auto q = __builtin_amdgcn_permlane32_swap(u2, u2, false, false);
  const unsigned q0 = q[0], q1 = q[1];
  return __uint_as_float(q0) + __uint_as_float(q1);
}

template <int BMAX, int GEMV_KITERS, int ROWS>
__global__ __launch_bounds__(256) void gemv_kernel(const half_t* __restrict__ w, const float* __restrict__ bias,
                                                   const float* __restrict__ x, int ldx, float* __restrict__ out,
                                                   int ldo, int B, int N, int K, int silu_in, int silu_out,
                                                   int accumulate) {
  const int lane = threadIdx.x & 63;
  const int n0 = (blockIdx.x * 4 + (threadIdx.x >> 6)) * ROWS;
  if (n0 >= N) return;
  half8 wv[ROWS][GEMV_KITERS];
#pragma unroll
  for (int r = 0; r < ROWS; ++r) {
    const half_t* wr = w + (size_t)min(n0 + r, N - 1) * K;
#pragma unroll
    for (int i = 0; i < GEMV_KITERS; ++i) {
      const int k = (lane + 64 * i) * 8;
      wv[r][i] = *reinterpret_cast<const half8*>(wr + min(k, K - 8));
    }
  }
  float xr[BMAX][GEMV_KITERS][8];
#pragma unroll
  for (int b = 0; b < BMAX; ++b) {
    const float* xb = x + (size_t)min(b, B - 1) * ldx;
#pragma unroll
    for (int i = 0; i < GEMV_KITERS; ++i) {
      const int k = (lane + 64 * i) * 8;
      const bool in = k < K;
      const floatx4 lo = *reinterpret_cast<const floatx4*>(xb + min(k, K - 8));
      const floatx4 hi = *reinterpret_cast<const floatx4*>(xb + min(k, K - 8) + 4);
#pragma unroll
      for (int e = 0; e < 8; ++e) {
        float v = e < 4 ? lo[e] : hi[e - 4];
        if (silu_in) v = silu_f(v);
        xr[b][i][e] = in ? v : 0.f;
      }
    }
  }
  float acc[ROWS][BMAX];
#pragma unroll
  for (int r = 0; r < ROWS; ++r)
#pragma unroll
    for (int b = 0; b < BMAX; ++b) {
      float s = 0.f;
#pragma unroll
      for (int i = 0; i < GEMV_KITERS; ++i)
#pragma unroll
        for (int e = 0; e < 8; ++e) s = fmaf((float)wv[r][i][e], xr[b][i][e], s);
      acc[r][b] = s;
    }
#pragma unroll
  for (int r = 0; r < ROWS; ++r)
#pragma unroll
    for (int b = 0; b < BMAX; ++b) acc[r][b] = wave_sum(acc[r][b]);
  float mine = 0.f;
#pragma unroll
  for (int r = 0; r < ROWS; ++r)
#pragma unroll
    for (int b = 0; b < BMAX; ++b) mine = (lane == r * BMAX + b) ? acc[r][b] : mine;
  const int n = n0 + lane / BMAX, b = lane % BMAX;
  if (lane < ROWS * BMAX && n < N && b < B) {
    float v = mine + (bias ? bias[n] : 0.f);
    if (silu_out) v = silu_f(v);
    float* dst = out + (size_t)b * ldo + n;
    *dst = accumulate ? (*dst + v) : v;
  }
}

__global__ void nchw_to_nhwc_kernel(const void* __restrict__ src, int src_is_f32, half_t* __restrict__ dst, int B,
                                    int C, int HW) {
  const size_t total = (size_t)B * C * HW;
  for (size_t idx = (size_t)blockIdx.x * blockDim.x + threadIdx.x; idx < total;
       idx += (size_t)gridDim.x * blockDim.x) {
    const int c = (int)(idx % C);
    const size_t bp = idx / C;
    const int p = (int)(bp % HW);
    const int b = (int)(bp / HW);
    const size_t s = ((size_t)b * C + c) * HW + p;
    dst[idx] = src_is_f32 ? (half_t) reinterpret_cast<const float*>(src)[s] : reinterpret_cast<const half_t*>(src)[s];
  }
}

__global__ void nhwc_to_nchw_f32_kernel(const half_t* __restrict__ src, float* __restrict__ dst, int B, int C, int HW) {
  const size_t total = (size_t)B * C * HW;
  for (size_t idx = (size_t)blockIdx.x * blockDim.x + threadIdx.x; idx < total;
       idx += (size_t)gridDim.x * blockDim.x) {
    const int p = (int)(idx % HW);
    const size_t bc = idx / HW;
    const int c = (int)(bc % C);
    const int b = (int)(bc / C);
    dst[idx] = (float)src[((size_t)b * HW + p) * C + c];
  }
}

__global__ void half_to_float_kernel(const half_t* __restrict__ s, float* __restrict__ d, size_t n) {
  for (size_t i = (size_t)blockIdx.x * blockDim.x + threadIdx.x; i < n; i += (size_t)gridDim.x * blockDim.x)
    d[i] = (float)s[i];
}
__global__ void float_to_half_kernel(const float* __restrict__ s, half_t* __restrict__ d, size_t n) {
  for (size_t i = (size_t)blockIdx.x * blockDim.x + threadIdx.x; i < n; i += (size_t)gridDim.x * blockDim.x)
    d[i] = (half_t)s[i];
}
__global__ void add_half_kernel(const half_t* __restrict__ a, const half_t* __restrict__ b, half_t* __restrict__ y,
                                size_t n8) {
  for (size_t i = (size_t)blockIdx.x * blockDim.x + threadIdx.x; i < n8; i += (size_t)gridDim.x * blockDim.x) {
    const half8 x = reinterpret_cast<const half8*>(a)[i], z = reinterpret_cast<const half8*>(b)[i];
    half8 o;
#pragma unroll
    for (int e = 0; e < 8; ++e) o[e] = (half_t)((float)x[e] + (float)z[e]);
    reinterpret_cast<half8*>(y)[i] = o;
  }
}
struct SumSrc {
  const half_t* p[4];
};
__global__ void sum_half_kernel(SumSrc src, int nsrc, half_t* __restrict__ y, size_t n8) {
  for (size_t i = (size_t)blockIdx.x * blockDim.x + threadIdx.x; i < n8; i += (size_t)gridDim.x * blockDim.x) {
    float acc[8];
    const half8 x = reinterpret_cast<const half8*>(src.p[0])[i];
#pragma unroll
    for (int e = 0; e < 8; ++e) acc[e] = (float)x[e];
    for (int k = 1; k < nsrc; ++k) {
      const half8 z = reinterpret_cast<const half8*>(src.p[k])[i];
#pragma unroll
      for (int e = 0; e < 8; ++e) acc[e] += (float)z[e];
    }
    half8 o;
#pragma unroll
    for (int e = 0; e < 8; ++e) o[e] = (half_t)acc[e];
    reinterpret_cast<half8*>(y)[i] = o;
  }
}
__global__ void bc1s_to_tokens_kernel(const half_t* __restrict__ src, half_t* __restrict__ dst, int B, int C, int S) {
  const size_t total = (size_t)B * C * S;
  for (size_t idx = (size_t)blockIdx.x * blockDim.x + threadIdx.x; idx < total;
       idx += (size_t)gridDim.x * blockDim.x) {
    const int c = (int)(idx % C);
    const size_t bs = idx / C;
    const int s = (int)(bs % S);
    const int b = (int)(bs / S);
    dst[idx] = src[((size_t)b * C + c) * S + s];
  }
}

__global__ void loop_prep_kernel(const float* __restrict__ latents, half_t* __restrict__ sample,
                                 float* __restrict__ tbuf, LoopTables t, int Bimg, int C, int HW, int cfg) {
  const int step = *t.step;
  const size_t per = (size_t)C * HW;
  const size_t total = (size_t)Bimg * per;
  for (size_t idx = (size_t)blockIdx.x * blockDim.x + threadIdx.x; idx < total;
       idx += (size_t)gridDim.x * blockDim.x) {
    const int c = (int)(idx % C);
    const size_t bp = idx / C;
    const int p = (int)(bp % HW);
    const int b = (int)(bp / HW);
    const half_t v = (half_t)(latents[((size_t)b * C + c) * HW + p] * (t.in_scale ? t.in_scale[step] : 1.0f));
    for (int r = 0; r < cfg; ++r) sample[((size_t)(r * Bimg + b) * HW + p) * C + c] = v;
  }
  if (blockIdx.x == 0 && threadIdx.x < cfg * Bimg) tbuf[threadIdx.x] = t.timesteps[step];
  if (t.temb_tab) {
    const size_t rowsz = (size_t)t.temb_ld, blk = (size_t)t.temb_rows * rowsz;
    const float* src = t.temb_tab + (size_t)step * blk;
    const size_t n4 = (size_t)t.temb_rows * (t.temb_n / 4);
    for (size_t i = (size_t)blockIdx.x * blockDim.x + threadIdx.x; i < n4; i += (size_t)gridDim.x * blockDim.x) {
      const size_t r = i / (t.temb_n / 4), c = i - r * (t.temb_n / 4);
      reinterpret_cast<floatx4*>(t.temb_dst + r * rowsz)[c] = reinterpret_cast<const floatx4*>(src + r * rowsz)[c];
    }
  }
}

__global__ __launch_bounds__(256) void cfg_sched_step_kernel(const float* __restrict__ noise_pred,
                                                              float* __restrict__ latents, float* __restrict__ eps_hist,
                                                              LoopTables t, float guidance, int Bimg, int CHW, int cfg,
                                                              int hist) {
  const int step = *t.step;
  const float* cf = t.coef + (size_t)step * 8;
  const float cx = cf[0], cm = cf[1], ma = cf[5], mb = cf[6];
  const bool push = cf[7] == 0.f;
  const size_t total = (size_t)Bimg * CHW;
  for (size_t idx = (size_t)blockIdx.x * blockDim.x + threadIdx.x; idx < total; idx += (size_t)gridDim.x * blockDim.x) {
    float eps = noise_pred[idx];
    if (cfg == 2) {
      const float c = noise_pred[total + idx];
      eps = eps + guidance * (c - eps);
    }
    const float x0 = latents[idx];
    if (t.denoised) {
      const float* pr = t.pred + (size_t)step * 8;
      float d = fmaf(pr[0], x0, pr[1] * eps);
      for (int j = 0; j < hist; ++j) d = fmaf(pr[2 + j], eps_hist[(size_t)j * total + idx], d);
      t.denoised[idx] = d;
    }
    const float m = ma * x0 + mb * eps;
    float x = cx * x0 + cm * m;
    for (int j = hist - 1; j >= 0; --j) {
      const float old = eps_hist[(size_t)j * total + idx];
      x += cf[2 + j] * old;
      if (push && j + 1 < hist) eps_hist[(size_t)(j + 1) * total + idx] = old;
    }
    if (push && hist > 0) eps_hist[idx] = m;
    if (t.noise_tab) x += t.noise_tab[(size_t)step * total + idx];
    latents[idx] = x;
  }
  __syncthreads();
  if (threadIdx.x == 0) {
    const unsigned arrived = __hip_atomic_fetch_add(t.ticket, 1u, __ATOMIC_RELAXED, __HIP_MEMORY_SCOPE_AGENT);
    if (arrived == gridDim.x - 1) {
      *t.ticket = 0;
      *t.step = step + 1;
    }
  }
}

__device__ __forceinline__ float posterior_latent(float mean, float logvar, float eps, float scale) {
  const float lv = fminf(fmaxf(logvar, -30.0f), 20.0f);
  return fmaf(expf(0.5f * lv), eps, mean) * scale;
}
template <bool VEC>
__global__ __launch_bounds__(256) void posterior_noise_kernel(const float* __restrict__ moments, const float* __restrict__ eps,
                                                               const float* __restrict__ noise, float* __restrict__ out, size_t n,
                                                               int n_images, float scale, float sa, float sb) {
  const size_t stride = (size_t)gridDim.x * blockDim.x;
  if (VEC) {
    const size_t n4 = n / 4;
    const floatx4* mean4 = reinterpret_cast<const floatx4*>(moments);
    const floatx4* logvar4 = reinterpret_cast<const floatx4*>(moments + n);
    const floatx4* eps4 = reinterpret_cast<const floatx4*>(eps);
    for (size_t i = (size_t)blockIdx.x * blockDim.x + threadIdx.x; i < n4; i += stride) {
      const floatx4 m = mean4[i], lv = logvar4[i], e = eps4[i];
      floatx4 z;
#pragma unroll
      for (int k = 0; k < 4; ++k) z[k] = posterior_latent(m[k], lv[k], e[k], scale);
      for (int b = 0; b < n_images; ++b) {
        const floatx4 nz = reinterpret_cast<const floatx4*>(noise + (size_t)b * n)[i];
        floatx4 o;
#pragma unroll
        for (int k = 0; k < 4; ++k) o[k] = fmaf(sa, z[k], sb * nz[k]);
        reinterpret_cast<floatx4*>(out + (size_t)b * n)[i] = o;
      }
    }
  } else {
    for (size_t i = (size_t)blockIdx.x * blockDim.x + threadIdx.x; i < n; i += stride) {
      const float z = posterior_latent(moments[i], moments[n + i], eps[i], scale);
      for (int b = 0; b < n_images; ++b) out[(size_t)b * n + i] = fmaf(sa, z, sb * noise[(size_t)b * n + i]);
    }
  }
}

inline int grid_for(size_t n) { return (int)std::min<size_t>((n + 255) / 256, 2048); }

}

std::vector<float> timestep_freq_table(int dim, float freq_shift) {
  const int half = dim / 2;
  std::vector<float> f(half);
  for (int i = 0; i < half; ++i) {
    const float exponent = (-9.210340371976184f * (float)i) / ((float)half - freq_shift);
    f[i] = (float)std::exp((double)exponent);
  }
  return f;
}

void launch_timestep_embedding(const float* t, const float* freq, float* out, int n, int dim, hipStream_t s) {
  const int total = n * (dim / 2);
  hipLaunchKernelGGL(timestep_embedding_kernel, dim3(cdiv(total, 256)), dim3(256), 0, s, t, freq, out, n, dim);
  SD_HIP(hipGetLastError());
}

void launch_gemv(const half_t* w, const float* bias, const float* x, int ldx, float* out, int ldo, int B, int N,
                 int K, int silu_in, int silu_out, int accumulate, hipStream_t s) {
  SD_REQUIRE(K % 8 == 0 && K <= 64 * 8 * 6, kUnsupported, "gemv: K=%d must be a multiple of 8 and <= 3072", K);
  for (int b0 = 0; b0 < B; b0 += 4) {
    const int nb = std::min(4, B - b0);
    const float* xp = x + (size_t)b0 * ldx;
    float* op = out + (size_t)b0 * ldo;
    if (K <= 64 * 8 * 3) {
      if (nb <= 2)
        hipLaunchKernelGGL((gemv_kernel<2, 3, 8>), dim3(cdiv(N, 4 * 8)), dim3(256), 0, s, w, bias, xp, ldx, op, ldo, nb, N, K,
                           silu_in, silu_out, accumulate);
      else
        hipLaunchKernelGGL((gemv_kernel<4, 3, 8>), dim3(cdiv(N, 4 * 8)), dim3(256), 0, s, w, bias, xp, ldx, op, ldo, nb, N, K,
                           silu_in, silu_out, accumulate);
    } else {
      hipLaunchKernelGGL((gemv_kernel<4, 6, 4>), dim3(cdiv(N, 4 * 4)), dim3(256), 0, s, w, bias, xp, ldx, op, ldo, nb, N, K,
                         silu_in, silu_out, accumulate);
    }
  }
  SD_HIP(hipGetLastError());
}

void launch_nchw_to_nhwc(const void* src, int src_is_f32, half_t* dst, int B, int C, int H, int W, hipStream_t s) {
  const size_t n = (size_t)B * C * H * W;
  hipLaunchKernelGGL(nchw_to_nhwc_kernel, dim3(grid_for(n)), dim3(256), 0, s, src, src_is_f32, dst, B, C, H * W);
  SD_HIP(hipGetLastError());
}
void launch_nhwc_to_nchw_f32(const half_t* src, float* dst, int B, int C, int H, int W, hipStream_t s) {
  const size_t n = (size_t)B * C * H * W;
  hipLaunchKernelGGL(nhwc_to_nchw_f32_kernel, dim3(grid_for(n)), dim3(256), 0, s, src, dst, B, C, H * W);
  SD_HIP(hipGetLastError());
}
void launch_half_to_float(const half_t* src, float* dst, size_t n, hipStream_t s) {
  hipLaunchKernelGGL(half_to_float_kernel, dim3(grid_for(n)), dim3(256), 0, s, src, dst, n);
  SD_HIP(hipGetLastError());
}
void launch_float_to_half(const float* src, half_t* dst, size_t n, hipStream_t s) {
  hipLaunchKernelGGL(float_to_half_kernel, dim3(grid_for(n)), dim3(256), 0, s, src, dst, n);
  SD_HIP(hipGetLastError());
}
void launch_add_half(const half_t* a, const half_t* b, half_t* y, size_t n, hipStream_t s) {
  SD_REQUIRE(n % 8 == 0, kInvalidArgument, "add_half: n %% 8 != 0");
  hipLaunchKernelGGL(add_half_kernel, dim3(grid_for(n / 8)), dim3(256), 0, s, a, b, y, n / 8);
  SD_HIP(hipGetLastError());
}
void launch_sum_half(const half_t* const* srcs, int nsrc, half_t* y, size_t n, hipStream_t s) {
  SD_REQUIRE(n % 8 == 0 && nsrc >= 1 && nsrc <= 4, kInvalidArgument, "sum_half: n %% 8 != 0 or %d sources", nsrc);
  SumSrc src{};
  for (int i = 0; i < nsrc; ++i) src.p[i] = srcs[i];
  hipLaunchKernelGGL(sum_half_kernel, dim3(grid_for(n / 8)), dim3(256), 0, s, src, nsrc, y, n / 8);
  SD_HIP(hipGetLastError());
}
void launch_bc1s_to_tokens(const half_t* src, half_t* dst, int B, int C, int S, hipStream_t s) {
  const size_t n = (size_t)B * C * S;
  hipLaunchKernelGGL(bc1s_to_tokens_kernel, dim3(grid_for(n)), dim3(256), 0, s, src, dst, B, C, S);
  SD_HIP(hipGetLastError());
}

void launch_loop_prep(const float* latents, half_t* sample, float* tbuf, LoopTables t, int Bimg, int C, int H, int W,
                      int cfg, hipStream_t s) {
  const size_t n = (size_t)Bimg * C * H * W;
  hipLaunchKernelGGL(loop_prep_kernel, dim3(grid_for(n)), dim3(256), 0, s, latents, sample, tbuf, t, Bimg, C, H * W,
                     cfg);
  SD_HIP(hipGetLastError());
}

void launch_cfg_sched_step(const float* noise_pred, float* latents, float* eps_hist, LoopTables t, float guidance,
                           int Bimg, int CHW, int cfg, int hist, hipStream_t s) {
  const size_t n = (size_t)Bimg * CHW;
  hipLaunchKernelGGL(cfg_sched_step_kernel, dim3(std::min(grid_for(n), 64)), dim3(256), 0, s, noise_pred, latents,
                     eps_hist, t, guidance, Bimg, CHW, cfg, hist);
// ... 77 lines not shown
```

### ml-stable-diffusion_amd/csrc/net.cpp

```cpp
#include "net.h"

#include <algorithm>
#include <type_traits>

#include "conv_plan.h"
#include "weight_prep.h"

namespace sd {

Net::Net(const sd_unet_config& cfg, const WeightStore& ws, int device)
    : cfg_(cfg), ws_(&ws), f32_(cfg.compute_fp32 != 0), pal_tensors_((int)ws.palettes()), i8_marked_((int)ws.w8a8_marks()) {
  SD_REQUIRE(cfg.n_levels >= 1 && cfg.n_levels <= SD_MAX_LEVELS, kInvalidArgument, "n_levels=%d", cfg.n_levels);
  SD_REQUIRE(cfg.batch >= 1 && cfg.height >= 1 && cfg.width >= 1, kInvalidArgument, "bad batch/size");
  SD_REQUIRE(cfg.norm_num_groups >= 1 && cfg.norm_num_groups <= 64, kUnsupported, "norm_num_groups=%d",
             cfg.norm_num_groups);
  open(device);
}

void Net::seal() {
  ll_.seal();
  ws_ = nullptr;
}

Tensor Net::new_tensor(int B, int H, int W, int C) {
// ... 224 lines not shown
Tensor Net::conv_f32(std::vector<Op>& ops, const std::string& name, const Tensor& x, const ConvArgs& a) {
  const int cout = a.cout, k = a.k;
  const float* b = a.bias ? upload_vec(name + ".bias", cout) : nullptr;
  SD_REQUIRE(!a.x2 && !a.temb && !a.ln_colsum && a.out_mode == kOutHalf && !a.silu_out, kInternal, "%s: not a VAE conv", name.c_str());
  const float* w = upload_conv_weight_f32(name, cout, x.C, k);
  const ConvGeom g = conv_geom(name, x, a);
  Tensor out = new_tensor(x.B, g.Ho, g.Wo, cout);
  ConvF32Desc fd;
  fd.x = x.f();
  fd.w = w;
  fd.w_kind = 1;
  fd.bias = b;
  fd.res = reinterpret_cast<const float*>(a.res);
  fd.out = out.f();
  fd.B = x.B; fd.Hi = x.H; fd.Wi = x.W; fd.Cin = x.C; fd.Ho = g.Ho; fd.Wo = g.Wo; fd.N = cout;
  fd.ksize = k; fd.stride = a.stride; fd.up = a.up; fd.pad = g.pad;
  ops.push_back([fd](hipStream_t s) { launch_conv_f32(fd, s); });
  char buf[256];
  snprintf(buf, sizeof(buf), "conv%dx%d fp32 %d->%d @%dx%d %s", k, k, x.C, cout, g.Ho, g.Wo, name.c_str());
  ops.back().label = buf;
  ops.back().flop = 2.0 * x.B * g.Ho * g.Wo * (double)cout * x.C * k * k;
  return out;
}

ConvDesc Net::conv_shape(const std::string& name, const Tensor& x, const ConvArgs& a) const {
  const Tensor* x2 = a.x2;
  const bool ln = a.ln_colsum != nullptr;
  ConvDesc d;
  d.x0 = x.p;
  d.C0 = x.C;
  if (x2) {
    SD_REQUIRE(x2->B == x.B && x2->H == x.H && x2->W == x.W, kInternal, "%s: concat shape mismatch", name.c_str());
    d.x1 = x2->p;
    d.C1 = x2->C;
  }
  d.temb = a.temb;
  d.temb_stride = kTembCap;
  d.res = a.res;
  d.B = x.B;
  d.Hi = x.H;
  d.Wi = x.W;
  const ConvGeom g = conv_geom(name, x, a);
  d.Ho = g.Ho;
  d.Wo = g.Wo;
  d.pad = g.pad;
  d.ksize = a.k;
  d.stride = a.stride;
  d.up = a.up;
  d.N = a.cout;
  d.out_mode = a.out_mode;
  d.ldT = a.ldT;
  d.ln_colsum = a.ln_colsum;
  d.x0_i8 = a.x_i8;
  if (ln || a.x_i8) {
    d.vt_perm = a.vt_perm ? 1 : 0;
    d.q_scale = a.q_scale;
    d.q_cols = a.q_cols;
  }
  return d;
}

Tensor Net::conv_w(std::vector<Op>& ops, const std::string& name, const ConvWeights& weights, const float* bias, const Tensor& x, const ConvArgs& a) {
  const Tensor* x2 = a.x2;
  const int cout = a.cout, k = a.k;
  const bool geglu = a.out_mode == kOutGeglu, ln = a.ln_colsum != nullptr;
  const half_t* w = weights.w;
  ConvDesc d = conv_shape(name, x, a);
  d.w = w;
  d.bias = bias;
  d.cw = weights.cw;
  d.tile = weights.pin.tile;
  d.staging = weights.pin.staging;
  d.splitk = weights.pin.splitk;
  d.subpix = weights.subpix;
  Tensor out;
  const bool qkv = (ln || a.x_i8) && a.n_trans > 0;
  if (qkv) {
    out = new_tensor(x.B, d.Ho, d.Wo, a.n_trans);
    *a.vt_out = ll_.arena.alloc_n<half_t>((size_t)x.B * (cout - a.n_trans) * a.ldT);
    d.out_t = *a.vt_out;
    d.n_trans = a.n_trans;
  } else if (a.out_mode == kOutHalfT) {
    out.B = x.B; out.H = 1; out.W = a.ldT; out.C = cout;
    out.p = ll_.arena.alloc_n<half_t>((size_t)x.B * cout * a.ldT);
  } else {
    out = new_tensor(x.B, d.Ho, d.Wo, geglu ? cout / 2 : cout);
  }
  d.out = out.p;
  SD_REQUIRE(!ln || (conv_fast_path_ok(d) && !a.silu_out), kInternal, "%s: LayerNorm fold / fused q|k|v off the MFMA path",
             name.c_str());
  std::shared_ptr<GnHook> hook;
  if (a.out_mode == kOutHalf && !qkv) {
    hook = std::make_shared<GnHook>();
    out.gn = hook;
    hook->ops_pos = (int)ops.size();
    hook->ops_list = &ops;
  }
  auto with_hook = [hook](const ConvDesc& d0) {
    ConvDesc dd = d0;
    if (hook) {
      dd.gn_partial = hook->partial;
      dd.gn_groups = hook->groups;
    }
    return dd;
  };
  const int cin = x.C + (x2 ? x2->C : 0);
// ... 271 lines not shown
```

### ml-stable-diffusion_amd/csrc/net.h

```cpp
#pragma once
#include "../../include/sd_mi355x.h"
#include "conv_plan.h"
#include "launch_list.h"

namespace sd {

constexpr int kTembCap = 65536;
inline int round_up(int x, int a) { return (x + a - 1) / a * a; }

struct GnHook {
  float* partial = nullptr;
  int groups = 0;
  int entries = 0;
  bool fresh = false;
  void produced(int n) {
    entries = n;
    fresh = true;
  }
  int consume() {
    const int n = fresh ? entries : 0;
    fresh = false;
    return n;
  }
  int ops_pos = -1;
  const void* ops_list = nullptr;
};

struct Tensor {
  half_t* p = nullptr;
  int B = 0, H = 0, W = 0, C = 0;
  std::shared_ptr<GnHook> gn;
  int M() const { return B * H * W; }
  size_t numel() const { return (size_t)B * H * W * C; }
  float* f() const { return reinterpret_cast<float*>(p); }
};

struct OpTime {
  std::string label;
  double flop;
  float ms;
};

struct ConvArgs {
  const Tensor* x2 = nullptr;
  int cout = 0;
  int k = 1, stride = 1, up = 1;
  bool bias = true;
  const float* temb = nullptr;
  const half_t* res = nullptr;
  int out_mode = kOutHalf;
  int ldT = 0;
  bool silu_out = false;
  int pad = -1;
  const float* ln_colsum = nullptr;
  int n_trans = 0;
  half_t** vt_out = nullptr;
  bool vt_perm = false;
  float q_scale = 1.f;
  int q_cols = 0;
  bool keep_compressed = false;
  bool subpix = false;
  const int8_t* x_i8 = nullptr;
};

struct ConvWeights {
  const half_t* w = nullptr;
  CompressedWeights cw;
  WeightPin pin;
  bool subpix = false;
  ConvWeights(const half_t* fp16, bool folded = false) : w(fp16), subpix(folded) {}
  ConvWeights(const CompressedWeights& c, const WeightPin& p) : cw(c), pin(p) {}
};

class Net {
 public:
  virtual ~Net() { close(); }
  Net(const Net&) = delete;
  float time_forward(int warmup, int iters);
  std::vector<OpTime> profile(int iters);
  virtual void set_attention(int impl);
  void drop_graphs() { invalidate_graphs(); }
  size_t device_bytes() const { return ll_.arena.bytes(); }
  size_t arena_used_bytes() const { return ll_.arena.used(); }
  void palette_info(int* n_palettized, int* n_streamed, size_t* stream_bytes) const {
    *n_palettized = pal_tensors_;
    *n_streamed = pal_streamed_;
    *stream_bytes = pal_stream_bytes_;
  }
  void w8a8_info(int* n_marked, int* n_applied, size_t* bytes) const {
    *n_marked = i8_marked_;
    *n_applied = i8_applied_;
    *bytes = i8_bytes_;
  }
  int activation_range(int index, std::string* name, float* absmax);
  const std::vector<std::string>& w8a8_applied() const { return i8_names_; }
  const sd_unet_config& config() const { return cfg_; }

 protected:
  Net(const sd_unet_config& cfg, const WeightStore& ws, int device);
  void open(int device) { ll_.open(device); }
  void seal();
  void close() { ll_.close(); }

  Tensor new_tensor(int B, int H, int W, int C);
  half_t* upload_conv_weight(const std::string& name, int cout, int cin, int k, bool geglu);
  float* upload_conv_weight_f32(const std::string& name, int cout, int cin, int k);
  half_t* upload_subpixel_weight(const std::string& name, int cout, int cin);
  float* upload_vec(const std::string& name, int n, bool geglu = false);
  Tensor conv(std::vector<Op>& ops, const std::string& name, const Tensor& x, const ConvArgs& a);
  Tensor conv_w(std::vector<Op>& ops, const std::string& name, const ConvWeights& w, const float* bias, const Tensor& x, const ConvArgs& a);
  WeightPin weight_plan(const std::string& name, const Tensor& x, const ConvArgs& a, bool ln) const;
  ConvWeights upload_compressed(const std::string& name, const WeightPin& pin, int cin, const ConvArgs& a, const std::string& ln_name = std::string());
  bool observes_geglu(const std::string& name, const Tensor& x, const ConvArgs& a, bool ln) const;
  void observe_tensor(std::vector<Op>& ops, const std::string& name, const Tensor& t, const std::vector<std::string>& report_as = {});
// ... 56 lines not shown
```

### ml-stable-diffusion_amd/csrc/unet.cpp

```cpp
#include "unet.h"
#include "conv_plan.h"
#include "weight_prep.h"

#ifndef SD_GN_QKV_DEFAULT
#define SD_GN_QKV_DEFAULT 1
#endif

#include <algorithm>
#include <cmath>
#include <cstdlib>
#include <cstring>

namespace sd {

namespace {

const sd_unet_config& checked_size(const sd_unet_config& cfg) {
  if (!cfg.is_controlnet && cfg.n_levels >= 1 && cfg.n_levels <= SD_MAX_LEVELS) {
    const int q = 1 << (cfg.n_levels - 1);
    SD_REQUIRE(cfg.height % q == 0 && cfg.width % q == 0, kInvalidArgument,
               "latent size %dx%d: a UNet of %d levels needs height and width that divide by %d", cfg.height, cfg.width, cfg.n_levels, q);
  }
  return cfg;
}
// ... 146 lines not shown
  ops.back().flop = 4.0 * q.B * (double)q.C * Sq * Sk;
  return o;
}

Tensor UNet::transformer_block(std::vector<Op>& ops, const std::string& b, const Tensor& h, int heads, const std::string* proj_out,
                               const Tensor* tres, bool* tail_done, const PreQkv* pre) {
  const int C = h.C, S = h.H * h.W, L = cfg_.context_len;
  const int ldv = round_up(S, 8);
  Tensor qk;
  bool vt_perm = false;
  bool q_pre = false;
  half_t* vtp;
  if (pre) {
    qk = pre->qk;
    vtp = pre->vt;
    vt_perm = pre->vt_perm;
    q_pre = pre->q_pre;
  } else if (can_fold_ln(h, 3 * C, false) && S % 8 == 0 && (2 * C) % 64 == 0) {
    const std::string qname = b + ".attn1.to_qkv";
    const std::vector<std::string> parts = {b + ".attn1.to_q", b + ".attn1.to_k", b + ".attn1.to_v"};
    vt_perm = attention8_shape_ok(C / heads, S, S) && S % 16 == 0;
    q_pre = vt_perm;
    ConvArgs qa{.cout = 3 * C, .ldT = ldv, .n_trans = 2 * C, .vt_out = &vtp, .vt_perm = vt_perm,
                .q_scale = q_pre ? attention_q_prescale(C / heads) : 1.f, .q_cols = q_pre ? C : 0};
    const WeightPin qpin = qkv_plan(qname, parts, h, qa);
    if (observes_qkv(qname, parts, h, qa)) observe_tensor(ops, qname, layer_norm(ops, b + ".norm1", h), parts);
    if (qpin.kind == WeightSource::I8Qkv) {
      const ConvWeights qw = upload_qkv_i8(parts, qpin, C, C);
      float* qb = nullptr;
      if (ws_->has(parts[0] + ".bias") || ws_->has(parts[1] + ".bias") || ws_->has(parts[2] + ".bias")) {
        std::vector<float> hb((size_t)3 * C, 0.f);
        for (int i = 0; i < 3; ++i)
          if (ws_->has(parts[i] + ".bias")) {
            const HostTensor& tb = ws_->get(parts[i] + ".bias");
            SD_REQUIRE((int)tb.numel() == C, kInvalidArgument, "%s.bias: bad shape", parts[i].c_str());
            std::copy(tb.data.begin(), tb.data.end(), hb.begin() + (size_t)i * C);
          }
        qb = ll_.arena.alloc_n<float>(hb.size());
        SD_HIP(hipMemcpy(qb, hb.data(), hb.size() * sizeof(float), hipMemcpyHostToDevice));
      }
      const float* nw = upload_vec(b + ".norm1.weight", C);
      const float* nb = upload_vec(b + ".norm1.bias", C);
      const int M = h.M();
      int8_t* xq = ll_.arena.alloc_n<int8_t>((size_t)M * C);
      const half_t* xp = h.p;
      const float inv_s = qw.cw.inv_s;
      ops.push_back([=](hipStream_t s) { launch_layernorm_q8(xp, nw, nb, xq, M, C, 1e-5f, inv_s, s); });
      ops.back().label = "layernorm_q8 " + b + ".norm1";
      qa.x_i8 = xq;
      qk = conv_w(ops, qname, qw, qb, h, qa);
    } else {
      LnFold f = fold_layernorm(b + ".norm1", parts, C, C, false);
      qa.ln_colsum = f.colsum;
      qk = conv_w(ops, qname, f.w, f.bias, h, qa);
    }
  } else {
    Tensor n1 = layer_norm(ops, b + ".norm1", h);
    qk = conv_stacked(ops, {b + ".attn1.to_q", b + ".attn1.to_k"}, n1, C);
    vtp = conv(ops, b + ".attn1.to_v", n1, {.cout = C, .bias = false, .out_mode = kOutHalfT, .ldT = ldv}).p;
  }
  Tensor q = qk;
  q.C = C;
  Tensor a1 = attention(ops, q, qk.p + C, vtp, heads, S, S, 2 * C, ldv, 2 * C, vt_perm, q_pre);
  static const int xo_mode = tune_env_int("SD_XATTN_OUT", 3);
  const bool xo_branch = xo_mode != 0 && can_fold_ln(h, C, false) && xattn_fused_ok(C, heads, S, L) && xattn_out_ok(C, heads, S, L) &&
                         (heads == 5 || xo_mode == 2);
  const bool xo_pre = xo_branch && xo_mode == 3 && heads == 5;
  Tensor h1;
  if (!xo_pre) h1 = conv(ops, b + ".attn1.to_out.0", a1, {.cout = C, .res = h.p, .keep_compressed = true});
  const int ldvc = round_up(L, 8);
  Tensor k2 = conv(ctx_ops_, b + ".attn2.to_k", ctx_, {.cout = C, .bias = false});
  Tensor vt2 = conv(ctx_ops_, b + ".attn2.to_v", ctx_, {.cout = C, .bias = false, .out_mode = kOutHalfT, .ldT = ldvc});
  Tensor a2;
  Tensor h2;
  bool branch_done = false;
  if (xo_branch) {
    LnFold f = fold_layernorm(b + ".norm2", {b + ".attn2.to_q"}, C, C, false);
    half_t* wq_t = ll_.arena.alloc_n<half_t>((size_t)C * C);
    launch_xattn_out_retile(f.w, wq_t, C, ll_.stream);
    const half_t* wo = upload_conv_weight(b + ".attn2.to_out.0", C, C, 1, false);
    half_t* wo_t = ll_.arena.alloc_n<half_t>((size_t)C * C);
    launch_xattn_out_retile(wo, wo_t, C, ll_.stream);
    h2 = new_tensor(h.B, h.H, h.W, C);
    XAttnOutDesc xd;
    xd.x = xo_pre ? a1.p : h1.p;
    if (xo_pre) {
      const half_t* wo1 = upload_conv_weight(b + ".attn1.to_out.0", C, C, 1, false);
      half_t* wo1_t = ll_.arena.alloc_n<half_t>((size_t)C * C);
      launch_xattn_out_retile(wo1, wo1_t, C, ll_.stream);
      xd.h0 = h.p;
      xd.wo1_t = wo1_t;
      xd.o1_bias = upload_vec(b + ".attn1.to_out.0.bias", C);
    }
    xd.wq_t = wq_t;
    xd.q_bias = f.bias;
    xd.q_colsum = f.colsum;
    xd.k = k2.p;
    xd.vt = vt2.p;
    xd.wo_t = wo_t;
    xd.o_bias = upload_vec(b + ".attn2.to_out.0.bias", C);
    xd.out = h2.p;
    xd.M = h.M();
    xd.C = C;
    xd.S = S;
    xd.L = L;
    xd.ldv = ldvc;
// ... 677 lines not shown
      SD_HIP(hipMemcpyAsync(io.residual_outputs[i], res_out_[i], cn_out_[i].numel() * sizeof(float), kind, ll_.stream));
  } else {
    SD_REQUIRE(io.noise_pred != nullptr, kInvalidArgument, "missing output 'noise_pred'");
    SD_HIP(hipMemcpyAsync(io.noise_pred, noise_pred_,
                          (size_t)cfg_.batch * cfg_.out_channels * cfg_.height * cfg_.width * sizeof(float), kind,
                          ll_.stream));
  }
  SD_HIP(hipStreamSynchronize(ll_.stream));
}

void UNet::denoise_loop(const sd_unet_io& io, float* latents, int n_images, int n_steps, const float* timesteps,
                        const float* coef, const float* sample_scale, int history, float guidance, float* history_io,
                        float* ms_per_step, const float* pred, int every, sd_progress_fn fn, void* user, int* steps_done) {
  SD_HIP(hipSetDevice(ll_.device));
  SD_REQUIRE(!cfg_.is_controlnet, kInvalidArgument, "denoise_loop needs a UNet handle");
  const int cfgmul = guidance > 1.0f ? 2 : 1;
  SD_REQUIRE(cfgmul * n_images == cfg_.batch, kInvalidArgument,
             "UNet batch %d != %d images x %d (guidance_scale %s 1)", cfg_.batch, n_images, cfgmul,
             cfgmul == 2 ? ">" : "<=");
  SD_REQUIRE(cfg_.in_channels == cfg_.out_channels, kInvalidArgument, "loop needs in_channels == out_channels");
  SD_REQUIRE(history >= 0 && history <= 3 && n_steps >= 1, kInvalidArgument, "bad history (%d, max 3) / n_steps (%d)",
             history, n_steps);
  SD_REQUIRE(in_res_nchw_.empty() || !attached_.empty(), kInvalidArgument,
             "a UNet built with support_controlnet needs attached ControlNets for the device-resident loop "
             "(sd_unet_attach_controlnets); host residuals only travel through sd_unet_forward");
  const int C = cfg_.in_channels, H = cfg_.height, W = cfg_.width;
  const size_t lat_n = (size_t)n_images * C * H * W;
  const size_t hist_n = (size_t)3 * cfg_.batch * C * H * W;
  if (!latents_) {
    latents_ = ll_.arena.alloc_n<float>((size_t)cfg_.batch * C * H * W);
    eps_hist_ = ll_.arena.alloc_n<float>(hist_n);
    step_ = ll_.arena.alloc_n<int>(2);
  }
  if (tab_cap_ < n_steps) {
    tab_cap_ = std::max(n_steps, 1024);
    tab_timesteps_ = ll_.arena.alloc_n<float>(tab_cap_);
    tab_coef_ = ll_.arena.alloc_n<float>((size_t)tab_cap_ * 8);
    tab_scale_ = ll_.arena.alloc_n<float>(tab_cap_);
    if (loop_graph_) { (void)hipGraphExecDestroy(loop_graph_); loop_graph_ = nullptr; }
  }
  upload_inputs(io, true);
  SD_HIP(hipMemcpyAsync(latents_, latents, lat_n * sizeof(float), hipMemcpyHostToDevice, ll_.stream));
  SD_HIP(hipMemcpyAsync(tab_timesteps_, timesteps, (size_t)n_steps * sizeof(float), hipMemcpyHostToDevice, ll_.stream));
  SD_HIP(hipMemcpyAsync(tab_coef_, coef, (size_t)n_steps * 8 * sizeof(float), hipMemcpyHostToDevice, ll_.stream));
  SD_HIP(hipMemsetAsync(step_, 0, 2 * sizeof(int), ll_.stream));
  SD_HIP(hipMemsetAsync(eps_hist_, 0, hist_n * sizeof(float), ll_.stream));
  if (history_io && history > 0)
    for (int j = 0; j < history; ++j)
      SD_HIP(hipMemcpyAsync(eps_hist_ + (size_t)j * lat_n, history_io + (size_t)j * lat_n, lat_n * sizeof(float),
                            hipMemcpyHostToDevice, ll_.stream));
  if (sample_scale)
    SD_HIP(hipMemcpyAsync(tab_scale_, sample_scale, (size_t)n_steps * sizeof(float), hipMemcpyHostToDevice, ll_.stream));
  static const bool hoist_off = tune_env_set("SD_NO_TEMB_TABLE");
  const bool hoist = !hoist_off && tpath_.ok && temb_w_all_ && temb_used_ > 0 && temb_used_ % 4 == 0;
  if (hoist) {
    const int Bt = cfg_.batch, rows = n_steps * Bt;
    if (temb_tab_cap_ < n_steps) {
      temb_tab_cap_ = std::max(n_steps, 64);
      const size_t r = (size_t)temb_tab_cap_ * Bt;
      temb_tab_ = ll_.arena.alloc_n<float>(r * kTembCap);
      tt_tab_ = ll_.arena.alloc_n<float>(r);
      tsin_tab_ = ll_.arena.alloc_n<float>(r * tpath_.c0);
      e1_tab_ = ll_.arena.alloc_n<float>(r * tpath_.tdim);
      emb_tab_ = ll_.arena.alloc_n<float>(r * tpath_.tdim);
      if (loop_graph_) { (void)hipGraphExecDestroy(loop_graph_); loop_graph_ = nullptr; }
    }
    std::vector<float> tt((size_t)rows);
    for (int i = 0; i < n_steps; ++i)
      for (int b = 0; b < Bt; ++b) tt[(size_t)i * Bt + b] = timesteps[i];
    SD_HIP(hipMemcpyAsync(tt_tab_, tt.data(), tt.size() * sizeof(float), hipMemcpyHostToDevice, ll_.stream));
    SD_HIP(hipStreamSynchronize(ll_.stream));
    const int c0 = tpath_.c0, td = tpath_.tdim;
    launch_timestep_embedding(tt_tab_, tpath_.freq, tsin_tab_, rows, c0, ll_.stream);
    launch_gemv(tpath_.w1, tpath_.b1, tsin_tab_, c0, e1_tab_, td, rows, td, c0, 0, 1, 0, ll_.stream);
    launch_gemv(tpath_.w2, tpath_.b2, e1_tab_, td, emb_tab_, td, rows, td, td, 0, 0, 0, ll_.stream);
    launch_gemv(temb_w_all_, temb_b_all_, emb_tab_, td, temb_tab_, kTembCap, rows, temb_used_, td, 1, 0, 0, ll_.stream);
  }
  LoopTables tab{tab_timesteps_, tab_coef_, step_, sample_scale ? tab_scale_ : nullptr,
                 reinterpret_cast<unsigned*>(step_ + 1), hoist ? temb_tab_ : nullptr, temb_all_, cfg_.batch, kTembCap, temb_used_};
  if (io.step_noise) {
    const size_t need = (size_t)n_steps * lat_n;
    if (noise_cap_ < need) {
      const size_t cap = std::max(need + need / 2, (size_t)64 * lat_n);
      noise_tab_ = ll_.arena.alloc_n<float>(cap);
      noise_cap_ = cap;
      if (loop_graph_) { (void)hipGraphExecDestroy(loop_graph_); loop_graph_ = nullptr; }
    }
    SD_HIP(hipMemcpyAsync(noise_tab_, io.step_noise, need * sizeof(float), hipMemcpyHostToDevice, ll_.stream));
    tab.noise_tab = noise_tab_;
  }
  const bool tap = pred != nullptr;
  if (tap) {
    if (pred_cap_ < n_steps) {
      pred_cap_ = std::max(n_steps, 1024);
      tab_pred_ = ll_.arena.alloc_n<float>((size_t)pred_cap_ * 8);
      if (!denoised_) denoised_ = ll_.arena.alloc_n<float>((size_t)cfg_.batch * C * H * W);
      if (loop_graph_) { (void)hipGraphExecDestroy(loop_graph_); loop_graph_ = nullptr; }
    }
    SD_HIP(hipMemcpyAsync(tab_pred_, pred, (size_t)n_steps * 8 * sizeof(float), hipMemcpyHostToDevice, ll_.stream));
    tab.pred = tab_pred_;
    tab.denoised = denoised_;
  }
  auto step_ops = [&]() {
    launch_loop_prep(latents_, x_in_.p, tbuf_, tab, n_images, C, H, W, cfgmul, ll_.stream);
    run_attached();
    run_main(!hoist);
    launch_cfg_sched_step(noise_pred_, latents_, eps_hist_, tab, guidance, n_images, C * H * W, cfgmul, history,
                          ll_.stream);
  };
  const int key = n_images * 128 + (io.step_noise ? 64 : 0) + (hoist ? 32 : 0) + (tap ? 16 : 0) + history * 4 + (cfgmul - 1) * 2 +
                  (sample_scale ? 1 : 0);
  const bool pairs = fn != nullptr;
  std::unique_ptr<EventList> ev;
  if (ms_per_step) ev = std::make_unique<EventList>(pairs ? (size_t)n_steps * 2 : (size_t)n_steps + 1);
  if (cfg_.use_graph) {
    int gbits;
    std::memcpy(&gbits, &guidance, 4);
    const int full_key = key ^ (gbits * 31);
    if (!loop_graph_ || loop_graph_key_ != full_key) {
      if (loop_graph_) { (void)hipGraphExecDestroy(loop_graph_); loop_graph_ = nullptr; }
      if (!ll_.graph) {
        launch_loop_prep(latents_, x_in_.p, tbuf_, tab, n_images, C, H, W, cfgmul, ll_.stream);
        run_attached();
        run_main(true);
        SD_HIP(hipStreamSynchronize(ll_.stream));
      }
      loop_graph_ = capture_graph(ll_.stream, step_ops);
      loop_graph_key_ = full_key;
    }
  }
  if (fn) {
    snap_latents_.resize(lat_n);
// ... 45 lines not shown
```

### ml-stable-diffusion_amd/csrc/unet.h

```cpp
#pragma once
#include "net.h"

namespace sd {

struct PreQkv {
  Tensor qk;
  half_t* vt = nullptr;
  bool vt_perm = false;
  bool q_pre = false;
};

class UNet : public Net {
 public:
  UNet(const sd_unet_config& cfg, const WeightStore& ws, int device);
  ~UNet() override;

  void forward(const sd_unet_io& io);
  void denoise_loop(const sd_unet_io& io, float* latents, int n_images, int n_steps, const float* timesteps,
                    const float* coef, const float* sample_scale, int history, float guidance, float* history_io,
                    float* ms_per_step, const float* pred = nullptr, int every = 1, sd_progress_fn fn = nullptr,
                    void* user = nullptr, int* steps_done = nullptr);
  bool in_progress_handler() const { return in_handler_; }
  void attach_controlnets(const std::vector<UNet*>& cns);
  void set_controlnet_cond(const void* cond, int flags);
// ... 9 lines not shown
  };
  LnFold fold_layernorm(const std::string& ln, const std::vector<std::string>& names, int cin, int cout_each,
                        bool geglu, bool upload_w = true);
  bool can_fold_ln(const Tensor& x, int cout, bool geglu) const;
  Tensor conv_stacked(std::vector<Op>& ops, const std::vector<std::string>& names, const Tensor& x, int cout_each);
  Tensor layer_norm(std::vector<Op>& ops, const std::string& name, const Tensor& x);
  Tensor time_resnet(std::vector<Op>& ops, const std::string& p, const Tensor& x, const Tensor* x2, int cout);
  Tensor transformer(std::vector<Op>& ops, const std::string& p, const Tensor& x, int heads, int depth);
  Tensor transformer_block(std::vector<Op>& ops, const std::string& b, const Tensor& h, int heads, const std::string* proj_out = nullptr,
                           const Tensor* tres = nullptr, bool* tail_done = nullptr, const PreQkv* pre = nullptr);
  Tensor attention(std::vector<Op>& ops, const Tensor& q, const half_t* k, const half_t* vt, int heads, int Sq,
                   int Sk, int ldk, int ldv, int ldq, bool vt_perm = false, bool q_prescaled = false);
  float* sk_part_ = nullptr;
  size_t sk_part_bytes_ = 0;
  unsigned* sk_cnt_ = nullptr;
  int sk_cnt_n_ = 0;
  void down_and_mid(std::vector<Op>& ops, Tensor& h, std::vector<Tensor>& skips);
  const float* register_temb(const std::string& name, int cout);
  void finalize_temb();
  void upload_inputs(const sd_unet_io& io, bool loop_mode);
  void run_as_controlnet(hipStream_t s, const half_t* x_nhwc, const float* tbuf);
  void set_context_from(const half_t* ehs_dev, hipStream_t s);
  void run_attached();
  void invalidate_graphs() override;
  void run_eager() override;
  void run_main(bool with_time);
  std::vector<const std::vector<Op>*> forward_lists() const override { return {&in_ops_, &time_ops_, &ll_.ops, &out_ops_}; }

  hipStream_t cn_stream_ = nullptr;
  hipEvent_t ev_cn_fork_ = nullptr, ev_cn_join_ = nullptr;
  int cn_join_pos_ = -1;
  bool cn_forked_ = false;

  half_t* in_sample_ = nullptr;
  half_t* in_timestep_ = nullptr;
  half_t* in_ehs_ = nullptr;
  half_t* in_time_ids_ = nullptr;
  half_t* in_text_embeds_ = nullptr;
  half_t* in_cond_ = nullptr;
  std::vector<half_t*> in_res_nchw_;
  std::vector<Tensor> res_nhwc_;
  std::vector<std::vector<int>> res_shapes_;
  float* noise_pred_ = nullptr;
  std::vector<float*> res_out_;
  std::vector<Tensor> cn_out_;

  Tensor x_in_;
  float* tbuf_ = nullptr;
  float* emb_ = nullptr;
  float* temb_all_ = nullptr;
  float* temb_tab_ = nullptr;
  int temb_tab_cap_ = 0;
  float *tt_tab_ = nullptr, *tsin_tab_ = nullptr, *e1_tab_ = nullptr, *emb_tab_ = nullptr;
  struct TimePath {
    const float* freq = nullptr;
    const half_t *w1 = nullptr, *w2 = nullptr;
    const float *b1 = nullptr, *b2 = nullptr;
    int c0 = 0, tdim = 0;
    bool ok = false;
  } tpath_;
  int temb_used_ = 0;
  std::vector<std::pair<std::string, int>> temb_layers_;
  half_t* temb_w_all_ = nullptr;
  float* temb_b_all_ = nullptr;
  Tensor ctx_;

  std::vector<Op> in_ops_, time_ops_, ctx_ops_, cond_ops_;
  std::vector<Op> out_ops_;
  std::vector<UNet*> attached_;
  std::vector<uint16_t> last_ehs_, last_cond_;
  bool have_ctx_ = false, have_cond_ = false;
  hipGraphExec_t loop_graph_ = nullptr;
  int loop_graph_key_ = -1;

  float* latents_ = nullptr;
  float* eps_hist_ = nullptr;
  float* tab_timesteps_ = nullptr;
  float* tab_coef_ = nullptr;
  float* tab_scale_ = nullptr;
  int* step_ = nullptr;
  int tab_cap_ = 0;
  float* noise_tab_ = nullptr;
  size_t noise_cap_ = 0;
  float* tab_pred_ = nullptr;
  int pred_cap_ = 0;
  float* denoised_ = nullptr;
  std::vector<float> snap_latents_, snap_denoised_;
  bool in_handler_ = false;
};

}
```

### ml-stable-diffusion_amd/python_hip_stable_diffusion/_lib.py

```python
import ctypes as C
import os

import numpy as np

_HERE = os.path.dirname(os.path.abspath(__file__))
LIB_PATH = os.environ.get("SD_MI355X_LIB", os.path.join(os.path.dirname(_HERE), "lib", "libsdmi355.so"))

SD_MAX_LEVELS = 6
SD_FLAG_DEVICE_PTRS = 1
ATTENTION_IMPLEMENTATIONS = {"ORIGINAL": 0, "SPLIT_EINSUM": 1, "SPLIT_EINSUM_V2": 2}


class LibraryNotBuilt(ImportError):
    pass


class UNetConfig(C.Structure):
    _fields_ = [
        ("batch", C.c_int32), ("in_channels", C.c_int32), ("out_channels", C.c_int32),
        ("height", C.c_int32), ("width", C.c_int32), ("n_levels", C.c_int32),
        ("block_out_channels", C.c_int32 * SD_MAX_LEVELS),
        ("down_cross_attn", C.c_int32 * SD_MAX_LEVELS),
        ("up_cross_attn", C.c_int32 * SD_MAX_LEVELS),
        ("layers_per_block", C.c_int32),
# ... 83 lines not shown
    ("sd_op_qkv_w8a8", _I, [_P, _P, _FP, _F, _FP, _P, _P, _I, _I, _I, _F, _I, _I, C.POINTER(_I), _I, _FP]),
    ("sd_op_w8a8_pack_qkv", _I, [_P, _I, _P, C.POINTER(C.c_size_t)]),
    ("sd_op_quantize_weight", _I, [_FP, _I, C.c_size_t, _P, _FP, C.POINTER(C.c_double)]),
    ("sd_op_absmax", _I, [_P, C.c_size_t, _FP]),
    ("sd_unet_create", _I, [C.POINTER(UNetConfig), _P, _I, C.POINTER(_P)]),
    ("sd_unet_destroy", None, [_P]),
    ("sd_unet_set_attention", _I, [_P, _I]),
    ("sd_unet_num_residuals", _I, [_P]),
    ("sd_unet_device_bytes", C.c_size_t, [_P]),
    ("sd_unet_arena_used_bytes", C.c_size_t, [_P]),
    ("sd_unet_palette_info", _I, [_P, C.POINTER(_I), C.POINTER(_I), C.POINTER(C.c_size_t)]),
    ("sd_unet_forward", _I, [_P, C.POINTER(UNetIO)]),
    ("sd_unet_time_forward", _I, [_P, _I, _I, _FP]),
    ("sd_unet_denoise_loop", _I, [_P, C.POINTER(UNetIO), _FP, _I, _I, _FP, _FP, _FP, _I, _F, _FP, _FP]),
    ("sd_unet_denoise_loop_progress", _I, [_P, C.POINTER(UNetIO), _FP, _I, _I, _FP, _FP, _FP, _I, _F, _FP, _FP, _FP, _I, _P, _P,
                                           C.POINTER(_I)]),
    ("sd_tune_set_candidate", _I, [_I, _I, _I]),
    ("sd_tune_set_plan_table", _I, [C.c_char_p, C.c_void_p, C.POINTER(C.c_int)]),
    ("sd_unet_profile", _I, [_P, _I, _I, _FP, C.POINTER(C.c_double), C.c_char_p, _I, C.POINTER(_I)]),
    ("sd_unet_attach_controlnets", _I, [_P, C.POINTER(_P), _I]),
    ("sd_controlnet_set_cond", _I, [_P, _P, _I]),
    ("sd_vae_decoder_create", _I, [C.POINTER(UNetConfig), _P, _I, C.POINTER(_P)]),
    ("sd_vae_decode", _I, [_P, _P, _I, _FP, _I]),
    ("sd_vae_encoder_create", _I, [C.POINTER(UNetConfig), _P, _I, C.POINTER(_P)]),
    ("sd_vae_encode", _I, [_P, _P, _I, _FP, _I]),
    ("sd_vae_encode_latents", _I, [_P, _P, _I, _FP, _FP, _I, _F, _F, _F, _FP, _I]),
    ("sd_text_encoder_create", _I, [_P, _P, _I, C.POINTER(_P)]),
    ("sd_text_encoder_destroy", None, [_P]),
    ("sd_text_encoder_device_bytes", C.c_size_t, [_P]),
    ("sd_text_encoder_encode", _I, [_P, C.POINTER(C.c_int32), _I, _FP, _FP, _FP]),
    ("sd_op_attention", _I, [_I, _P, _P, _P, _P, _I, _I, _I, _I, _I, _I, _I, _FP]),
    ("sd_op_layernorm", _I, [_P, _FP, _FP, _P, _I, _I, _I, _F, _I, _FP]),
    ("sd_op_groupnorm", _I, [_P, _FP, _FP, _P, _I, _I, _I, _I, _I, _F, _I, _I, _FP]),
    ("sd_op_groupnorm_shortcut", _I, [_P, _P, _FP, _FP, _P, _FP, _P, _P, _I, _I, _I, _I, _I, _I, _I, _F, _I, _I, _I, _FP]),
    ("sd_op_conv2d", _I, [_P, _P, _FP, _P, _P, _I, _I, _I, _I, _I, _I, _I, _I, _I, _I, _I, _I, _FP]),
    ("sd_op_conv2d_ex", _I, [_P, _P, _P, _FP, _FP, _P, _P, _I, _I, _I, _I, _I, _I, _I, _I, _I, _I, _I, _FP, _FP, _F, _I, _P, _I, _I, _I,
                             C.POINTER(_I), _I, _FP]),
    ("sd_op_conv2d_palettized", _I, [_P, _P, _P, _I, _P, _FP, _P, _P, _I, _I, _I, _I, _I, _I, _I, _I, _I, C.POINTER(_I), _I, _FP]),
    ("sd_op_palette_pack", _I, [_P, _I, _I, _I, _I, _P, C.POINTER(C.c_size_t)]),
    ("sd_op_gemm_palettized", _I, [_P, _P, _I, _P, _FP, _P, _P, _I, _I, _I, _I, _I, _I, C.POINTER(_I), _I, _FP]),
    ("sd_op_palette_pack_gemm", _I, [_P, _I, _I, _I, _P, C.POINTER(C.c_size_t)]),
    ("sd_op_geglu_palettized", _I, [_P, _FP, _FP, _P, _I, _P, _FP, _P, _I, _I, _I, C.c_float, _I, C.POINTER(_I), _I, _FP]),
    ("sd_op_palette_pack_geglu", _I, [_P, _I, _I, _I, _P, C.POINTER(C.c_size_t)]),
    ("sd_op_conv2d_groupnorm", _I, [_P, _P, _FP, _P, _FP, _FP, _P, _P, _I, _I, _I, _I, _I, _I, _I, _F, _I, _I, _I, C.POINTER(_I), _I, _FP]),
    ("sd_op_conv2d_groupnorm_proj", _I, [_P, _P, _FP, _P, _FP, _FP, _P, _FP, _P, _P, _I, _I, _I, _I, _I, _I, _I, _I, _F, _I, _I, C.POINTER(_I), _I, _FP]),
    ("sd_op_conv2d_groupnorm_conv3x3", _I, [_P, _P, _FP, _P, _FP, _FP, _P, _FP, _P, _P, _P, _I, _I, _I, _I, _I, _I, _I, _I, _F, _I, _I, _I, _I,
                                            C.POINTER(_I), _I, _FP]),
    ("sd_op_cross_attention_fused", _I, [_P, _FP, _FP, _P, _P, _P, _P, _I, _I, _I, _I, _F, _I, _I, _FP]),
    ("sd_op_ffn_out_proj", _I, [_P, _P, _FP, _P, _P, _FP, _P, _P, _FP, _I, _I, _I, _I, _I, _I, _FP]),
    ("sd_op_fold_linear", _I, [_P, _FP, _P, _FP, _P, _FP, _I, _I, _I]),
    ("sd_op_cross_attention_block", _I, [_P, _FP, _FP, _P, _P, _P, _P, _FP, _P, _P, _FP, _P, _I, _I, _I, _I, _F, _I, _I, _FP]),
    ("sd_op_geglu", _I, [_P, _P, _FP, _P, _I, _I, _I, _I, _FP]),
    ("sd_op_geglu_ln", _I, [_P, _FP, _FP, _P, _FP, _P, _I, _I, _I, C.c_float, _I, _I, _FP]),
    ("sd_op_qkv_ln", _I, [_P, _FP, _FP, _P, _P, _P, _I, _I, _I, C.c_float, C.c_float, _I, _I, _I, _FP]),
    ("sd_op_gn_proj_qkv", _I, [_P, _P, _FP, _FP, _P, _FP, _FP, _FP, _P, _P, _P, _P, _I, _I, _I, _I, _I, C.c_float, C.c_float, C.c_float, _I, _I,
                               C.POINTER(C.c_int), _I, _FP]),
    ("sd_op_timestep_embedding", _I, [_FP, _FP, _I, _I, _I, _F]),
    ("sd_op_posterior_noise", _I, [_FP, _FP, _FP, _FP, _I, _I, _I, _I, _F, _F, _F, _I, _FP]),
    ("sd_op_sched_step", _I, [_FP, _FP, _FP, _FP, _FP, _FP, _F, _I, _I, _I, _I, _FP, C.POINTER(_I)]),
    ("sd_op_conv_plan", _I, [_I] * 18 + [C.POINTER(C.c_int), C.POINTER(C.c_ulonglong)]),
    ("sd_op_conv_plan_kernel", _I, [_I] * 18 + [C.c_char_p, _I]),
    ("sd_numpy_randn", _I, [C.c_uint32, C.POINTER(C.c_double), C.c_size_t]),
    ("sd_torch_randn", _I, [C.c_uint32, C.POINTER(C.c_double), C.c_size_t]),
    ("sd_philox_randn", _I, [C.c_uint64, C.c_uint32, C.POINTER(C.c_double), C.c_size_t]),
    ("sd_calibrate", _I, [_I, _FP]),
    ("sd_selftest_mfma", _I, []),
    ("sd_safety_checker_create", _I, [C.POINTER(SafetyCheckerConfig), _P, _I, C.POINTER(_P)]),
    ("sd_safety_checker_destroy", None, [_P]),
    ("sd_safety_checker_device_bytes", C.c_size_t, [_P]),
    ("sd_safety_checker_last_ms", C.c_float, [_P]),
    ("sd_safety_checker_run", _I, [_P, _P, _F, _FP, _FP, _FP, _FP, _I]),
    ("sd_op_vit_attention", _I, [_P, _P, _I, _I, _I, _I, _I, _FP]),
    ("sd_op_safety_head", _I, [_FP, _FP, _FP, _FP, _FP, _F, _I, _I, _I, _I, _FP, _FP]),
    ("sd_op_vae_attention", _I, [_P, _P, _P, _P, _I, _I, _I, _I, _FP]),
    ("sd_vae_decode_images", _I, [_P, _P, _I, _FP, _P, _P, C.POINTER(ImagePost), _F, _FP, _FP, _I]),
    ("sd_op_resample_coeffs", _I, [_I, _I, C.POINTER(_I), _P, _P]),
    ("sd_op_image_rgb8", _I, [_FP, _P, _I, _I, _I, _I, _FP]),
    ("sd_op_clip_input", _I, [_P, _P, _I, _I, _I, _I, _I, _I, _FP, _FP, _I, _FP]),
    ("sd_op_conv_f32", _I, [_FP, _P, _I, _FP, _FP, _FP, _I, _I, _I, _I, _I, _I, _I, _I, _I]),
    ("sd_op_groupnorm_f32", _I, [_FP, _FP, _FP, _FP, _I, _I, _I, _I, _I, _F, _I]),
    ("sd_op_row_softmax", _I, [_P, _I, _I, _F, _I]),
    ("sd_op_gemv", _I, [_P, _FP, _FP, _FP, _I, _I, _I, _I, _I, _I]),
    ("sd_op_clip_attention", _I, [_P, _P, _I, _I, _I]),
    ("sd_op_clip_embed", _I, [C.POINTER(C.c_int32), _P, _P, _P, _I, _I, _I]),
    ("sd_op_clip_act", _I, [_P, C.c_size_t, _I]),
    ("sd_op_layout", _I, [_I, _P, _P, _I, _I, _I, _I]),
    ("sd_op_sum_half", _I, [C.POINTER(_P), _I, _P, C.c_size_t, _I]),
    ("sd_op_vit_patch_rows", _I, [_P, _P, _I, _I, _I, _I]),
    ("sd_op_vit_tokens", _I, [_P, _P, _P, _P, _I, _I, _I]),
]


def lib():
    global _lib
    if _lib is not None:
        return _lib
    if not os.path.exists(LIB_PATH):
        raise LibraryNotBuilt(
            f"{LIB_PATH} is missing - build it with `python -c 'import __graft_entry__ as g; g.build()'` "
            f"or `make -C ml-stable-diffusion_amd/csrc`. There is no CPU fallback.")
    if not os.environ.get("SD_MI355X_NO_TORCH"):
        try:
            import torch
        except Exception:
            pass
    handle = C.CDLL(LIB_PATH, mode=C.RTLD_GLOBAL)
    for name, restype, argtypes in SYMBOLS:
# ... 719 lines not shown


def fold_linear(wp, bp, w2, b2):
    wp, w2, bp, b2 = f16(wp), f16(w2), f32(bp), f32(b2)
    N, J = wp.shape
    K = w2.shape[1]
    if w2.shape[0] != J or bp.shape != (N,) or b2.shape != (J,):
        raise ValueError("fold_linear: inconsistent shapes")
    wm = np.empty((N, K), np.float16)
    bm = np.empty(N, np.float32)
    check(lib().sd_op_fold_linear(ptr(wp), fptr(bp), ptr(w2), fptr(b2), ptr(wm), fptr(bm), N, J, K))
    return wm, bm


def cross_attention_fused(x, ln_weight, ln_bias, wq, k, v, heads, eps=1e-5, nst=0, iters=1):
    x, k, v, wq = f16(x), f16(k), f16(v), f16(wq)
    B, Cn, _, Sq = x.shape
    Sk = k.shape[3]
    if Cn != heads * 64 or k.shape[1] != Cn or v.shape != k.shape or wq.shape != (Cn, Cn):
        raise ValueError("cross_attention_fused: inconsistent shapes")
    ln_weight, ln_bias = f32(ln_weight), f32(ln_bias)
    out = np.empty_like(x)
    ms = C.c_float(0)
    check(lib().sd_op_cross_attention_fused(ptr(x), fptr(ln_weight), fptr(ln_bias), ptr(wq), ptr(k), ptr(v), ptr(out), B, heads,
                                            Sq, Sk, eps, nst, iters, C.byref(ms)))
    return out, ms.value


def geglu(x, w, bias=None, iters=1):
    x, w = f16(x), f16(w)
    M, Cn = x.shape
    N2 = w.shape[0]
    bias = None if bias is None else f32(bias)
    out = np.empty((M, N2 // 2), np.float16)
    ms = C.c_float(0)
    check(lib().sd_op_geglu(ptr(x), ptr(w), fptr(bias), ptr(out), M, Cn, N2, iters, C.byref(ms)))
    return out, ms.value


def geglu_ln(x, w, bias=None, ln_weight=None, ln_bias=None, eps=1e-5, kernel=0, iters=1):
    x, w = f16(x), f16(w)
    M, Cn = x.shape
    N2 = w.shape[0]
    bias = None if bias is None else f32(bias)
    ln_weight = None if ln_weight is None else f32(ln_weight)
    ln_bias = None if ln_bias is None else f32(ln_bias)
    out = np.empty((M, N2 // 2), np.float16)
    ms = C.c_float(0)
    check(lib().sd_op_geglu_ln(ptr(x), fptr(ln_weight), fptr(ln_bias), ptr(w), fptr(bias), ptr(out), M, Cn, N2, eps, kernel, iters,
                               C.byref(ms)))
    return out, ms.value


def qkv_ln(x, ln_weight, ln_bias, w, batch, q_scale=1.0, vt_perm=True, eps=1e-5, kernel=0, iters=1):
    x, w = f16(x), f16(w)
    M, Cn = x.shape
    HW = M // batch
    out_qk = np.empty((M, 2 * Cn), np.float16)
    out_vt = np.empty((batch, Cn, HW), np.float16)
    ms = C.c_float(0)
    check(lib().sd_op_qkv_ln(ptr(x), fptr(f32(ln_weight)), fptr(f32(ln_bias)), ptr(w), ptr(out_qk), ptr(out_vt), batch, HW, Cn, eps, q_scale,
                             int(vt_perm), kernel, iters, C.byref(ms)))
    return out_qk, out_vt, ms.value


def gn_proj_qkv(x_in, conv_w, gn_weight, gn_bias, proj_w, proj_bias, ln_weight, ln_bias, wqkv, groups=32, gn_eps=1e-6, ln_eps=1e-5,
                q_scale=1.0, vt_perm=True, fused=True, iters=1):
    x_in, conv_w, proj_w, wqkv = f16(x_in), f16(conv_w), f16(proj_w), f16(wqkv)
    B, Cn, H, W = x_in.shape
    M = B * H * W
    h = np.empty((M, Cn), np.float16)
    qk = np.empty((M, 2 * Cn), np.float16)
    vt = np.empty((B, Cn, H * W), np.float16)
    ms, entries = C.c_float(0), C.c_int(0)
    check(lib().sd_op_gn_proj_qkv(ptr(x_in), ptr(conv_w), fptr(f32(gn_weight)), fptr(f32(gn_bias)), ptr(proj_w), fptr(f32(proj_bias)),
                                  fptr(f32(ln_weight)), fptr(f32(ln_bias)), ptr(wqkv), ptr(h), ptr(qk), ptr(vt), B, H, W, Cn, groups, gn_eps,
                                  ln_eps, q_scale, int(vt_perm), int(fused), C.byref(entries), iters, C.byref(ms)))
    return h, qk, vt, entries.value, ms.value


def conv_plan(ksize, stride, up, C0, C1, N, B, Ho, Wo, out_mode=0, flags=0, n_trans=0, n_twins=0, gnf_groups=0, tile=0, staging=0, splitk=0,
              copies=-1):
    plan = (C.c_int * 7)()
    ws = C.c_ulonglong(0)
    desc = (ksize, stride, up, C0, C1, N, B, Ho, Wo, out_mode, flags, n_trans, n_twins, gnf_groups, tile, staging, splitk, copies)
    check(lib().sd_op_conv_plan(*desc, plan, C.byref(ws)))
    text = C.create_string_buffer(64)
    check(lib().sd_op_conv_plan_kernel(*desc, text, len(text)))
    return {"tile": plan[0], "staging": plan[1], "splitk": plan[2], "slab": bool(plan[3]), "workspace_bytes": int(ws.value),
            "copies": (bool(plan[4]), bool(plan[5]), bool(plan[6])), "kernel": text.value.decode()}


def timestep_embedding(t, dim, flip_sin_to_cos=True, freq_shift=0.0):
    t = f32(t)
    out = np.empty((t.shape[0], dim), np.float32)
    check(lib().sd_op_timestep_embedding(fptr(t), fptr(out), t.shape[0], dim, int(flip_sin_to_cos), freq_shift))
    return out


def posterior_noise(moments, eps, noise, scale_factor, sa, sb, iters=1):
    moments, eps, noise = f32(moments), f32(eps), f32(noise)
    if noise.ndim != 4:
        raise ValueError("posterior_noise: noise must be (n_images, Cz, h, w)")
    n_images, Cz, h, w = noise.shape
    if moments.size != 2 * Cz * h * w or moments.shape[-3:] != (2 * Cz, h, w) or eps.shape[-3:] != (Cz, h, w) or eps.size != Cz * h * w:
        raise ValueError("posterior_noise: moments must be (2*Cz, h, w) and eps (Cz, h, w) for noise (n_images, Cz, h, w)")
    out = np.empty_like(noise)
    ms = C.c_float(0)
    check(lib().sd_op_posterior_noise(fptr(moments), fptr(eps), fptr(noise), fptr(out), Cz, h, w, n_images, float(scale_factor), float(sa),
                                      float(sb), iters, C.byref(ms)))
    return out, ms.value


def sched_step(noise_pred, latents, coef, guidance=1.0, hist=None, pred=None, step_noise=None):
    noise_pred, lat, coef = f32(noise_pred), f32(latents).copy(), f32(coef)
# ... 202 lines not shown
```

Measured before the change: 244.1 it/s.

## Add fp16 LayerNorm-folded q|k|v kernel and dedupe timestep-embedding table rows

Adds a new fp16 smqkv kernel (plan tile 23) for the LayerNorm-folded q|k|v projection. It applies the LN statistics, bias and q scaling in the epilogue and writes V transposed. The planner picks it automatically for the measured shape M=2048, C=640 when weights are plain fp16. Separately, the precomputed timestep-embedding table now keeps one row per step instead of one per batch element, and the gemv kernel gains a loop mode; the old duplicated layout stays behind an env flag. This adds a kernel specialised to one shape, and the per-step loop kernel now broadcasts a single row to every batch entry.

New measurement: 245.3 it/s (median of 6 runs). About the same (+0.5%).

```diff
diff --git a/include/sd_mi355x.h b/include/sd_mi355x.h
--- a/include/sd_mi355x.h
+++ b/include/sd_mi355x.h
@@ -230,8 +230,8 @@
 int sd_op_geglu(const void* x, const void* w, const float* bias, void* out, int M, int C, int N2, int iters, float* ms);
 int sd_op_geglu_ln(const void* x, const float* ln_weight, const float* ln_bias, const void* w, const float* bias, void* out, int M, int C,
                    int N2, float eps, int kernel, int iters, float* ms);
-int sd_op_qkv_ln(const void* x, const float* ln_weight, const float* ln_bias, const void* w, void* out_qk, void* out_vt, int B, int HW, int C,
-                 float eps, float q_scale, int vt_perm, int kernel, int iters, float* ms);
+int sd_op_qkv_ln(const void* x, const float* ln_weight, const float* ln_bias, const void* w, const float* bias, void* out_qk, void* out_vt, int B,
+                 int HW, int C, float eps, float q_scale, int vt_perm, int kernel, int iters, float* ms);
 int sd_op_gn_proj_qkv(const void* x_in, const void* conv_w, const float* gn_weight, const float* gn_bias, const void* proj_w,
                       const float* proj_bias, const float* ln_weight, const float* ln_bias, const void* wqkv, void* out_h, void* out_qk,
                       void* out_vt, int B, int H, int W, int C, int groups, float gn_eps, float ln_eps, float q_scale, int vt_perm, int fused,
diff --git a/ml-stable-diffusion_amd/csrc/capi_ops.cpp b/ml-stable-diffusion_amd/csrc/capi_ops.cpp
--- a/ml-stable-diffusion_amd/csrc/capi_ops.cpp
+++ b/ml-stable-diffusion_amd/csrc/capi_ops.cpp
@@ -1313,20 +1313,25 @@
   });
 }
 
-int sd_op_qkv_ln(const void* x, const float* ln_weight, const float* ln_bias, const void* w, void* out_qk, void* out_vt, int B, int HW, int C,
-                 float eps, float q_scale, int vt_perm, int kernel, int iters, float* ms) {
-  return guarded([&] {
-    SD_REQUIRE(x && ln_weight && ln_bias && w && out_qk && out_vt && B >= 1 && HW >= 1 && C % 64 == 0 && kernel >= 0 && kernel <= 9,
+int sd_op_qkv_ln(const void* x, const float* ln_weight, const float* ln_bias, const void* w, const float* bias, void* out_qk, void* out_vt, int B,
+                 int HW, int C, float eps, float q_scale, int vt_perm, int kernel, int iters, float* ms) {
+  return guarded([&] {
+    SD_REQUIRE(x && ln_weight && ln_bias && w && out_qk && out_vt && B >= 1 && HW >= 1 && C % 64 == 0 &&
+                   ((kernel >= 0 && kernel <= 9) || (kernel >= 100 && kernel <= 102)),
                kInvalidArgument, "bad q|k|v arguments");
     Scratch sc;
     const int N = 3 * C, M = B * HW;
-    const FoldedProj f = upload_ln_folded(sc, w, nullptr, ln_weight, ln_bias, N, C, false);
+    const FoldedProj f = upload_ln_folded(sc, w, bias, ln_weight, ln_bias, N, C, false);
     half_t* dqk = sc.dev<half_t>((size_t)M * 2 * C);
     half_t* dvt = sc.dev<half_t>((size_t)B * C * HW);
     ConvDesc d = qkv_desc(sc.dev<half_t>((size_t)M * C, f16(x)), f, eps, dqk, dvt, B, 1, HW, C, q_scale, vt_perm);
     SD_REQUIRE(conv_fast_path_ok(d), kUnsupported, "q|k|v shape off the MFMA path (C=%d)", C);
     const ConvWeightCopies copies = conv_plan_copies(d);
-    if (kernel == 2 || (kernel == 0 && copies.wsgemm)) {
+    if (kernel >= 100) {
+      SD_REQUIRE(smqkv_shape_ok(d, kernel - 100), kInvalidArgument, "q|k|v shape not eligible for plan tile 23 (smqkv.hip): C=%d M=%d HW=%d", C, M, HW);
+      d.tile = 23;
+      d.staging = kernel - 100;
+    } else if (kernel == 2 || (kernel == 0 && copies.wsgemm)) {
       SD_REQUIRE(wsgemm_shape_ok(d), kInvalidArgument, "q|k|v shape not eligible for plan tile 10 (wsgemm.hip)");
       tile_for_wsgemm(sc, d);
       if (kernel == 2) d.tile = 10;
@@ -1452,6 +1457,7 @@
   if (flags & 16) d.bias = present;
   if (flags & 32) d.pad = 0;
   if (flags & 64) d.subpix = true;
+  if (flags & 128) d.smqkv = true;
   if (n_trans > 0) d.out_t = const_cast<half_t*>(ph), d.n_trans = n_trans, d.ldT = Ho * Wo;
   d.n_twins = n_twins;
   if (gnf_groups > 0) {
diff --git a/ml-stable-diffusion_amd/csrc/conv_plan.cpp b/ml-stable-diffusion_amd/csrc/conv_plan.cpp
--- a/ml-stable-diffusion_amd/csrc/conv_plan.cpp
+++ b/ml-stable-diffusion_amd/csrc/conv_plan.cpp
@@ -26,12 +26,12 @@
 }
 
 struct Switches {
-  bool wstream, wsgemm, bvgemm, smgemm, smgeglu, reduce_stats, tuning, qkv_i8;
+  bool wstream, wsgemm, bvgemm, smgemm, smgeglu, reduce_stats, tuning, qkv_i8, smqkv;
 };
 const Switches& switches() {
   static const Switches s = {tune_env_int("SD_WSTREAM", 1) != 0, tune_env_int("SD_WSGEMM", 1) != 0, tune_env_int("SD_BVGEMM", 1) != 0,
                              tune_env_int("SD_SMGEMM", 1) != 0, tune_env_int("SD_SMGEGLU", 1) != 0, tune_env_int("SD_REDUCE_STATS", 0) != 0,
-                             getenv("SD_TUNE") != nullptr, tune_env_int("SD_QKV_I8", 1) != 0};
+                             getenv("SD_TUNE") != nullptr, tune_env_int("SD_QKV_I8", 1) != 0, tune_env_int("SD_SMQKV", 1) != 0};
   return s;
 }
 
@@ -286,7 +286,28 @@
   return M % bm == 0 && mt >= 2 && (mt * nt) % 8 == 0 && mt * nt <= 65535;
 }
 
+bool smqkv_shape_ok(const ConvDesc& d, int variant) {
+  if (!(d.cw.kind == WeightSource::Fp16 && d.ln_colsum && d.bias && !d.x0_i8)) return false;
+  ConvDesc plain = d;
+  plain.ln_colsum = nullptr;
+  return smqkv_i8_tiles(plain, variant);
+}
+bool smqkv_wanted(int M, int C) {
+  struct Shape { int m, c; };
+  static const Shape kMeasured[] = {
+      {2048, 640},
+      {0, 0}};
+  for (const Shape& s : kMeasured)
+    if (s.m == M && s.c == C && s.m != 0) return true;
+  return false;
+}
+
 namespace {
+
+bool takes_smqkv(const ConvDesc& d) {
+  return d.smqkv && switches().smqkv && d.tile == 0 && d.splitk == 0 && d.staging == 0 && g_tune.tile == 0 && smqkv_shape_ok(d, 0) &&
+         smqkv_wanted(d.B * d.Ho * d.Wo, d.C0);
+}
 
 int subpix_splits(const ConvDesc& d, const Dims& a) {
   const int steps = a.Ctot / BK;
@@ -373,6 +394,13 @@
       return ConvPlan{22, smqkv_i8_bm(d, d.staging) == 128 ? 1 : 2, 1, false, 0};
   }
   const Switches& sw = switches();
+  if (d.tile == 23) {
+    SD_REQUIRE(d.staging >= 0 && d.staging <= 2 && smqkv_shape_ok(d, d.staging), kInvalidArgument,
+               "plan tile 23 (smqkv.hip) needs fp16 weights, the LayerNorm fold and a q|k|v shape of tile 22's tiles (C0=%d N=%d n_trans=%d M=%d S=%d "
+               "ln=%d code=%d)", d.C0, d.N, d.n_trans, d.B * d.Ho * d.Wo, d.Ho * d.Wo, d.ln_colsum ? 1 : 0, d.staging);
+    return ConvPlan{23, d.staging, 1, false, 0};
+  }
+  if (takes_smqkv(d)) return ConvPlan{23, 0, 1, false, 0};
   const bool free_choice = d.tile == 0 && d.splitk == 0 && d.staging == 0 && g_tune.tile == 0;
   if (d.w_ws && wsgemm_shape_ok(d) && (d.tile == 10 || (sw.wsgemm && free_choice && wsgemm_wanted(d)))) return ConvPlan{10, 0, 1, false, 0};
   SD_REQUIRE(d.tile != 10, kInvalidArgument, "plan tile 10 (wsgemm.hip) needs the pre-tiled weights and an eligible GEGLU shape");
@@ -437,8 +465,8 @@
       p.kernel = p.tile == 13 ? ConvKernel::Smgeglu : p.tile == 16 ? ConvKernel::SmgegluPal : ConvKernel::SmgegluI8;
       p.bm = code >= 0 && code <= 2 ? smgeglu_bm(d, code) : 0;
       return;
-    case 22:
-      p.kernel = ConvKernel::SmqkvI8;
+    case 22: case 23:
+      p.kernel = p.tile == 22 ? ConvKernel::SmqkvI8 : ConvKernel::Smqkv;
       p.bm = code >= 0 && code <= 2 ? smqkv_i8_bm(d, code) : 0;
       return;
     default: break;
@@ -524,6 +552,7 @@
     case ConvKernel::SmgegluPal: return "smgeglu_pal bm" + std::to_string(p.bm);
     case ConvKernel::SmgegluI8: return "smgeglu_i8 bm" + std::to_string(p.bm);
     case ConvKernel::SmqkvI8: return "smqkv_i8 bm" + std::to_string(p.bm);
+    case ConvKernel::Smqkv: return "smqkv bm" + std::to_string(p.bm);
     default: return "generic";
   }
 }
@@ -542,6 +571,7 @@
 ConvWeightCopies conv_plan_copies(const ConvDesc& d0) {
   ConvWeightCopies c{false, false, false};
   if (!conv_fast_path_ok(d0) || d0.subpix) return c;
+  if (d0.tile == 23 || takes_smqkv(d0)) return c;
   ConvDesc d = d0;
   d.w_tiled = d.w_ws = d.w_bv = nullptr;
   const Switches& sw = switches();
@@ -660,7 +690,7 @@
   if (p.tile == 9 || p.tile == 14 || p.tile == 17)
     fprintf(stderr, "[sd conv] k%d up%d C0=%d C1=%d M=%d N=%d K=%d tile=%d nw=%d slabs=%d twins=%d bits=%d\n", d.ksize, d.up, d.C0, c1, a.M, a.N,
             a.K, p.tile, p.waves, p.splitk, d.n_twins, p.tile == 14 ? d.cw.bits : p.tile == 17 ? 8 : 16);
-  else if (p.tile == 12 || p.tile == 13)
+  else if (p.tile == 12 || p.tile == 13 || p.tile == 23)
     fprintf(stderr, "[sd conv] k1 s1 up1 C0=%d C1=%d M=%d N=%d K=%d mode=%d tile=%d bm=%d n_fast=%d\n", d.C0, c1, a.M, a.N, a.K, d.out_mode, p.tile, p.bm,
             n_fast);
   else if (p.tile == 15 || p.tile == 16)
diff --git a/ml-stable-diffusion_amd/csrc/conv_plan.h b/ml-stable-diffusion_amd/csrc/conv_plan.h
--- a/ml-stable-diffusion_amd/csrc/conv_plan.h
+++ b/ml-stable-diffusion_amd/csrc/conv_plan.h
@@ -5,7 +5,7 @@
 
 namespace sd {
 
-enum class ConvKernel { Generic, Igemm, GemmPipe, HaloKs, HaloI8, HaloSubpix, Wstream, WstreamPal, WstreamI8, Wsgemm, Bvgemm, Smgemm, SmgemmPal, SmgemmI8, Smgeglu, SmgegluPal, SmgegluI8, SmqkvI8 };
+enum class ConvKernel { Generic, Igemm, GemmPipe, HaloKs, HaloI8, HaloSubpix, Wstream, WstreamPal, WstreamI8, Wsgemm, Bvgemm, Smgemm, SmgemmPal, SmgemmI8, Smgeglu, SmgegluPal, SmgegluI8, SmqkvI8, Smqkv };
 
 struct ConvPlan {
   int tile;
@@ -77,5 +77,7 @@
 bool smqkv_i8_shape_ok(const ConvDesc& d, int variant);
 bool smqkv_i8_tiles(const ConvDesc& d, int variant);
 int smqkv_i8_bm(const ConvDesc& d, int variant);
+bool smqkv_shape_ok(const ConvDesc& d, int variant);
+bool smqkv_wanted(int M, int C);
 
 }
diff --git a/ml-stable-diffusion_amd/csrc/igemm.hip b/ml-stable-diffusion_amd/csrc/igemm.hip
--- a/ml-stable-diffusion_amd/csrc/igemm.hip
+++ b/ml-stable-diffusion_amd/csrc/igemm.hip
@@ -1010,6 +1010,7 @@
     case ConvKernel::SmgemmI8: launch_smgemm_i8(d, p, s); return 0;
     case ConvKernel::SmgegluI8: launch_smgeglu_i8(d, p, s); return 0;
     case ConvKernel::SmqkvI8: launch_smqkv_i8(d, p, s); return 0;
+    case ConvKernel::Smqkv: launch_smqkv(d, p, s); return 0;
     default: break;
   }
   IgemmArgs a = planned_args(d, p, ws.partial);
diff --git a/ml-stable-diffusion_amd/csrc/kernels.h b/ml-stable-diffusion_amd/csrc/kernels.h
--- a/ml-stable-diffusion_amd/csrc/kernels.h
+++ b/ml-stable-diffusion_amd/csrc/kernels.h
@@ -79,6 +79,7 @@
   GnTwin twin[2];
   int n_twins = 0;
   bool subpix = false;
+  bool smqkv = false;
 };
 
 constexpr int kGnMaxSlabs = 256;
@@ -143,6 +144,7 @@
 bool smgeglu_i8_shape_ok(const ConvDesc& d, int variant);
 void launch_smgeglu_i8(const ConvDesc& d, const ConvPlan& p, hipStream_t s);
 void launch_smqkv_i8(const ConvDesc& d, const ConvPlan& p, hipStream_t s);
+void launch_smqkv(const ConvDesc& d, const ConvPlan& p, hipStream_t s);
 
 void run_calibration(int device, float* out);
 
@@ -326,6 +328,7 @@
   const float* temb_tab;
   float* temb_dst;
   int temb_rows, temb_ld, temb_n;
+  int temb_dup = 0;
   const float* noise_tab = nullptr;
   const float* pred = nullptr;
   float* denoised = nullptr;
diff --git a/ml-stable-diffusion_amd/csrc/misc.hip b/ml-stable-diffusion_amd/csrc/misc.hip
--- a/ml-stable-diffusion_amd/csrc/misc.hip
+++ b/ml-stable-diffusion_amd/csrc/misc.hip
@@ -40,7 +40,7 @@
   return __uint_as_float(q0) + __uint_as_float(q1);
 }
 
-template <int BMAX, int GEMV_KITERS, int ROWS>
+template <int BMAX, int GEMV_KITERS, int ROWS, bool LOOP>
 __global__ __launch_bounds__(256) void gemv_kernel(const half_t* __restrict__ w, const float* __restrict__ bias,
                                                    const float* __restrict__ x, int ldx, float* __restrict__ out,
                                                    int ldo, int B, int N, int K, int silu_in, int silu_out,
@@ -58,51 +58,60 @@
       wv[r][i] = *reinterpret_cast<const half8*>(wr + min(k, K - 8));
     }
   }
-  float xr[BMAX][GEMV_KITERS][8];
-#pragma unroll
-  for (int b = 0; b < BMAX; ++b) {
-    const float* xb = x + (size_t)min(b, B - 1) * ldx;
-#pragma unroll
-    for (int i = 0; i < GEMV_KITERS; ++i) {
-      const int k = (lane + 64 * i) * 8;
-      const bool in = k < K;
-      const floatx4 lo = *reinterpret_cast<const floatx4*>(xb + min(k, K - 8));
-      const floatx4 hi = *reinterpret_cast<const floatx4*>(xb + min(k, K - 8) + 4);
-#pragma unroll
-      for (int e = 0; e < 8; ++e) {
-        float v = e < 4 ? lo[e] : hi[e - 4];
-        if (silu_in) v = silu_f(v);
-        xr[b][i][e] = in ? v : 0.f;
+  for (int b0 = 0; b0 < (LOOP ? B : 1); b0 += BMAX) {
+    const int nb = min(BMAX, B - b0);
+    if constexpr (LOOP) {
+#pragma unroll
+      for (int r = 0; r < ROWS; ++r)
+#pragma unroll
+        for (int i = 0; i < GEMV_KITERS; ++i) asm volatile("" : "+v"(wv[r][i]));
+    }
+    float xr[BMAX][GEMV_KITERS][8];
+#pragma unroll
+    for (int b = 0; b < BMAX; ++b) {
+      const float* xb = x + (size_t)(b0 + min(b, nb - 1)) * ldx;
+#pragma unroll
+      for (int i = 0; i < GEMV_KITERS; ++i) {
+        const int k = (lane + 64 * i) * 8;
+        const bool in = k < K;
+        const floatx4 lo = *reinterpret_cast<const floatx4*>(xb + min(k, K - 8));
+        const floatx4 hi = *reinterpret_cast<const floatx4*>(xb + min(k, K - 8) + 4);
+#pragma unroll
+        for (int e = 0; e < 8; ++e) {
+          float v = e < 4 ? lo[e] : hi[e - 4];
+          if (silu_in) v = silu_f(v);
+          xr[b][i][e] = in ? v : 0.f;
+        }
       }
     }
-  }
-  float acc[ROWS][BMAX];
-#pragma unroll
-  for (int r = 0; r < ROWS; ++r)
-#pragma unroll
-    for (int b = 0; b < BMAX; ++b) {
-      float s = 0.f;
-#pragma unroll
-      for (int i = 0; i < GEMV_KITERS; ++i)
-#pragma unroll
-        for (int e = 0; e < 8; ++e) s = fmaf((float)wv[r][i][e], xr[b][i][e], s);
-      acc[r][b] = s;
-    }
-#pragma unroll
-  for (int r = 0; r < ROWS; ++r)
-#pragma unroll
-    for (int b = 0; b < BMAX; ++b) acc[r][b] = wave_sum(acc[r][b]);
-  float mine = 0.f;
-#pragma unroll
-  for (int r = 0; r < ROWS; ++r)
-#pragma unroll
-    for (int b = 0; b < BMAX; ++b) mine = (lane == r * BMAX + b) ? acc[r][b] : mine;
-  const int n = n0 + lane / BMAX, b = lane % BMAX;
-  if (lane < ROWS * BMAX && n < N && b < B) {
-    float v = mine + (bias ? bias[n] : 0.f);
-    if (silu_out) v = silu_f(v);
-    float* dst = out + (size_t)b * ldo + n;
-    *dst = accumulate ? (*dst + v) : v;
+    float acc[ROWS][BMAX];
+#pragma unroll
+    for (int r = 0; r < ROWS; ++r)
+#pragma unroll
+      for (int b = 0; b < BMAX; ++b) {
+        float s = 0.f;
+#pragma unroll
+        for (int i = 0; i < GEMV_KITERS; ++i)
+#pragma unroll
+          for (int e = 0; e < 8; ++e) s = fmaf((float)wv[r][i][e], xr[b][i][e], s);
+        acc[r][b] = s;
+      }
+#pragma unroll
+    for (int r = 0; r < ROWS; ++r)
+#pragma unroll
+      for (int b = 0; b < BMAX; ++b) acc[r][b] = wave_sum(acc[r][b]);
+    float mine = 0.f;
+#pragma unroll
+    for (int r = 0; r < ROWS; ++r)
+#pragma unroll
+      for (int b = 0; b < BMAX; ++b) mine = (lane == r * BMAX + b) ? acc[r][b] : mine;
+    const int n = n0 + lane / BMAX, b = lane % BMAX;
+    if (lane < ROWS * BMAX && n < N && b < nb) {
+      float v = mine + (bias ? bias[n] : 0.f);
+      if (silu_out) v = silu_f(v);
+      float* dst = out + (size_t)(b0 + b) * ldo + n;
+      *dst = accumulate ? (*dst + v) : v;
+    }
   }
 }
 
@@ -198,12 +207,12 @@
   }
   if (blockIdx.x == 0 && threadIdx.x < cfg * Bimg) tbuf[threadIdx.x] = t.timesteps[step];
   if (t.temb_tab) {
-    const size_t rowsz = (size_t)t.temb_ld, blk = (size_t)t.temb_rows * rowsz;
+    const size_t rowsz = (size_t)t.temb_ld, blk = (t.temb_dup ? (size_t)t.temb_rows : 1) * rowsz;
     const float* src = t.temb_tab + (size_t)step * blk;
     const size_t n4 = (size_t)t.temb_rows * (t.temb_n / 4);
     for (size_t i = (size_t)blockIdx.x * blockDim.x + threadIdx.x; i < n4; i += (size_t)gridDim.x * blockDim.x) {
       const size_t r = i / (t.temb_n / 4), c = i - r * (t.temb_n / 4);
-      reinterpret_cast<floatx4*>(t.temb_dst + r * rowsz)[c] = reinterpret_cast<const floatx4*>(src + r * rowsz)[c];
+      reinterpret_cast<floatx4*>(t.temb_dst + r * rowsz)[c] = reinterpret_cast<const floatx4*>(src + (t.temb_dup ? r : 0) * rowsz)[c];
     }
   }
 }
@@ -309,21 +318,17 @@
 void launch_gemv(const half_t* w, const float* bias, const float* x, int ldx, float* out, int ldo, int B, int N,
                  int K, int silu_in, int silu_out, int accumulate, hipStream_t s) {
   SD_REQUIRE(K % 8 == 0 && K <= 64 * 8 * 6, kUnsupported, "gemv: K=%d must be a multiple of 8 and <= 3072", K);
-  for (int b0 = 0; b0 < B; b0 += 4) {
-    const int nb = std::min(4, B - b0);
-    const float* xp = x + (size_t)b0 * ldx;
-    float* op = out + (size_t)b0 * ldo;
-    if (K <= 64 * 8 * 3) {
-      if (nb <= 2)
-        hipLaunchKernelGGL((gemv_kernel<2, 3, 8>), dim3(cdiv(N, 4 * 8)), dim3(256), 0, s, w, bias, xp, ldx, op, ldo, nb, N, K,
-                           silu_in, silu_out, accumulate);
-      else
-        hipLaunchKernelGGL((gemv_kernel<4, 3, 8>), dim3(cdiv(N, 4 * 8)), dim3(256), 0, s, w, bias, xp, ldx, op, ldo, nb, N, K,
-                           silu_in, silu_out, accumulate);
-    } else {
-      hipLaunchKernelGGL((gemv_kernel<4, 6, 4>), dim3(cdiv(N, 4 * 4)), dim3(256), 0, s, w, bias, xp, ldx, op, ldo, nb, N, K,
-                         silu_in, silu_out, accumulate);
-    }
+  auto go = [&](auto kernel, int rows_per_wg) {
+    hipLaunchKernelGGL(kernel, dim3(cdiv(N, rows_per_wg)), dim3(256), 0, s, w, bias, x, ldx, out, ldo, B, N, K, silu_in, silu_out,
+                       accumulate);
+  };
+  if (K <= 64 * 8 * 3) {
+    if (B <= 2) go(gemv_kernel<2, 3, 8, false>, 4 * 8);
+    else if (B <= 4) go(gemv_kernel<4, 3, 8, false>, 4 * 8);
+    else go(gemv_kernel<4, 3, 8, true>, 4 * 8);
+  } else {
+    if (B <= 4) go(gemv_kernel<4, 6, 4, false>, 4 * 4);
+    else go(gemv_kernel<4, 6, 4, true>, 4 * 4);
   }
   SD_HIP(hipGetLastError());
 }
diff --git a/ml-stable-diffusion_amd/csrc/net.cpp b/ml-stable-diffusion_amd/csrc/net.cpp
--- a/ml-stable-diffusion_amd/csrc/net.cpp
+++ b/ml-stable-diffusion_amd/csrc/net.cpp
@@ -300,6 +300,7 @@
   d.ldT = a.ldT;
   d.ln_colsum = a.ln_colsum;
   d.x0_i8 = a.x_i8;
+  d.smqkv = a.smqkv;
   if (ln || a.x_i8) {
     d.vt_perm = a.vt_perm ? 1 : 0;
     d.q_scale = a.q_scale;
diff --git a/ml-stable-diffusion_amd/csrc/net.h b/ml-stable-diffusion_amd/csrc/net.h
--- a/ml-stable-diffusion_amd/csrc/net.h
+++ b/ml-stable-diffusion_amd/csrc/net.h
@@ -60,6 +60,7 @@
   int q_cols = 0;
   bool keep_compressed = false;
   bool subpix = false;
+  bool smqkv = false;
   const int8_t* x_i8 = nullptr;
 };
 
diff --git a/ml-stable-diffusion_amd/csrc/smqkv.hip b/ml-stable-diffusion_amd/csrc/smqkv.hip
--- /dev/null
+++ b/ml-stable-diffusion_amd/csrc/smqkv.hip
@@ -0,0 +1,313 @@
+#include <type_traits>
+
+#include "conv_plan.h"
+#include "kernels.h"
+#include "sm_ring.h"
+#include "sm_tile.h"
+
+namespace sd {
+
+namespace {
+
+constexpr int SQ_BK = 64;
+constexpr int SQ_PAIRS = kSmQkvCols / 32;
+constexpr int SQ_WROWS = kSmQkvCols;
+constexpr int SQ_NW = 2 * SQ_PAIRS;
+constexpr int SQ_LDS = 160 * 1024;
+
+struct SqArgs {
+  const half_t* x;
+  const half_t* w;
+  const float* bias;
+  const float* colsum;
+  half_t* out_qk;
+  half_t* out_vt;
+  int K, nk, C, S, ldT;
+  int vt_perm, q_mul;
+  float q_scale;
+  float ln_eps;
+  SmTileOrder order;
+};
+
+template <int BM>
+struct SqCfg {
+  static constexpr int ROWS = SQ_WROWS + BM;
+  static constexpr int PIECES = ROWS / 8;
+  static constexpr int PPW = (PIECES + SQ_NW - 1) / SQ_NW;
+  static constexpr int FULL = PIECES - SQ_NW * (PPW - 1);
+  static constexpr int STAGE = PIECES * 1024;
+  static constexpr int NST = (SQ_LDS - BM * 8) / STAGE;
+  static constexpr int TM = BM / 32;
+  static constexpr int SB = TM / 4;
+  static constexpr int EPI = BM == 256 ? 0 : 4;
+  static constexpr size_t LDS = (size_t)NST * STAGE + BM * 8;
+  static_assert(BM % 128 == 0 && ROWS % 8 == 0 && PPW >= 2 && FULL >= 1 && FULL <= SQ_NW, "tile");
+  static_assert(NST >= 3 && LDS <= SQ_LDS, "ring");
+  static_assert(PPW * (NST - 2) + EPI <= 63, "vmcnt range");
+};
+
+template <int BM>
+__global__ __launch_bounds__(64 * SQ_NW, 1) void smqkv_kernel(SqArgs a) {
+  using C = SqCfg<BM>;
+  constexpr int NST = C::NST, PPW = C::PPW, TM = C::TM, SB = C::SB;
+  extern __shared__ __attribute__((aligned(16))) char smem[];
+  const int lane = threadIdx.x & 63;
+  const int wave = __builtin_amdgcn_readfirstlane((int)threadIdx.x >> 6);
+  const int u = wave % SQ_PAIRS, h = wave / SQ_PAIRS;
+
+  int m_tile, n_tile;
+  sm_tile_coords(a.order, m_tile, n_tile);
+  const int m_blk = m_tile * BM, n_blk = n_tile * kSmQkvCols;
+  const bool is_v = n_blk >= 2 * a.C;
+  const bool q_mul = a.q_mul != 0 && n_blk < a.C;
+
+  const bool full = wave < C::FULL;
+  const half_t* src[PPW];
+  int pdst[PPW];
+#pragma unroll
+  for (int j = 0; j < PPW; ++j) {
+    int p = wave + SQ_NW * j;
+    if (p >= C::PIECES) p -= C::PIECES;
+    pdst[j] = p * 1024;
+    const int r = p * 8 + (lane >> 3);
+    const int chunk = (lane & 7) ^ ((r >> 1) & 7);
+    src[j] = (r < SQ_WROWS ? a.w + (size_t)(n_blk + r) * a.K : a.x + (size_t)(m_blk + r - SQ_WROWS) * a.K) + chunk * 8;
+  }
+  auto issue = [&](int slot) {
+    char* st = smem + slot * C::STAGE;
+#pragma unroll
+    for (int j = 0; j < PPW; ++j) {
+      if (j == PPW - 1 && !full) break;
+      __builtin_amdgcn_global_load_lds((const __attribute__((address_space(1))) void*)src[j],
+                                       (__attribute__((address_space(3))) void*)(st + pdst[j]), 16, 0, 0);
+      src[j] += SQ_BK;
+    }
+  };
+
+#pragma unroll
+  for (int p = 0; p < NST - 1; ++p)
+    if (p < a.nk) issue(p);
+  const int g = lane >> 4, r16 = lane & 15;
+  const int n0 = n_blk + 32 * u + (is_v ? (r16 & ~3) : 4 * g);
+  floatx4 bias0, bias1, cs0, cs1;
+  auto load_epi = [&]() __attribute__((always_inline)) {
+    __builtin_amdgcn_sched_barrier(0);
+    bias0 = *reinterpret_cast<const floatx4*>(a.bias + n0);
+    bias1 = *reinterpret_cast<const floatx4*>(a.bias + n0 + 16);
+    cs0 = *reinterpret_cast<const floatx4*>(a.colsum + n0);
+    cs1 = *reinterpret_cast<const floatx4*>(a.colsum + n0 + 16);
+    __builtin_amdgcn_sched_barrier(0);
+  };
+  if constexpr (C::EPI > 0) load_epi();
+
+  int foff[2];
+#pragma unroll
+  for (int kk = 0; kk < 2; ++kk) foff[kk] = r16 * 128 + (((4 * kk + g) ^ ((r16 >> 1) & 7)) * 16);
+  const int w_off = 32 * u * 128;
+  const int x_off = (SQ_WROWS + h * (BM / 2)) * 128;
+
+  floatx4 acc0[TM], acc1[TM];
+#pragma unroll
+  for (int i = 0; i < TM; ++i) acc0[i] = acc1[i] = floatx4{0.f, 0.f, 0.f, 0.f};
+  float ln_s1[SB], ln_s2[SB];
+#pragma unroll
+  for (int s = 0; s < SB; ++s) ln_s1[s] = ln_s2[s] = 0.f;
+  const half2v one2 = {(half_t)1.f, (half_t)1.f};
+
+  constexpr int NG = TM / 4, NQ = 2 * NG;
+  auto wait_stage = [&](int s) {
+    const int ahead = min(NST - 2, a.nk - 1 - s);
+    if (full) {
+      if (s <= NST - 2) sm_wait<PPW, C::EPI, NST - 2>(ahead);
+      else sm_wait<PPW, 0, NST - 2>(ahead);
+    } else {
+      if (s <= NST - 2) sm_wait<PPW - 1, C::EPI, NST - 2>(ahead);
+      else sm_wait<PPW - 1, 0, NST - 2>(ahead);
+    }
+  };
+
+  auto k_loop = [&](auto vt) __attribute__((always_inline)) {
+    constexpr bool VT = decltype(vt)::value;
+    auto mfma = [](half8 w, half8 x, floatx4 c) __attribute__((always_inline)) {
+      if constexpr (VT) return __builtin_amdgcn_mfma_f32_16x16x32_f16(x, w, c, 0, 0, 0);
+      else return __builtin_amdgcn_mfma_f32_16x16x32_f16(w, x, c, 0, 0, 0);
+    };
+    half8 w0[2], w1[2], w0n[2], w1n[2], xq[2][4];
+    auto read_w = [&](const char* st, half8 (&v0)[2], half8 (&v1)[2]) {
+  #pragma unroll
+      for (int kk = 0; kk < 2; ++kk) {
+        v0[kk] = *reinterpret_cast<const half8*>(st + w_off + foff[kk]);
+        v1[kk] = *reinterpret_cast<const half8*>(st + w_off + 16 * 128 + foff[kk]);
+      }
+    };
+    auto read_q = [&](const char* st, int q) {
+  #pragma unroll
+      for (int i = 0; i < 4; ++i)
+        xq[q & 1][i] = *reinterpret_cast<const half8*>(st + x_off + 16 * (4 * (q % NG) + i) * 128 + foff[q / NG]);
+    };
+    wait_stage(0);
+    if (NST - 1 < a.nk) issue(NST - 1);
+    read_w(smem, w0, w1);
+    read_q(smem, 0);
+    __builtin_amdgcn_sched_barrier(0);
+    int slot = 0;
+    for (int rel = 0; rel < a.nk; ++rel) {
+      const char* st = smem + slot * C::STAGE;
+      const int nslot = slot + 1 == NST ? 0 : slot + 1;
+#pragma unroll
+      for (int q = 0; q < NQ; ++q) {
+        const int kk = q / NG;
+        const bool next_stage = q + 1 == NQ && rel + 1 < a.nk;
+        if (next_stage) {
+          asm volatile("s_waitcnt lgkmcnt(0)" ::: "memory");
+          wait_stage(rel + 1);
+          if (rel + NST < a.nk) issue(slot);
+        }
+        __builtin_amdgcn_sched_barrier(0);
+        acc0[4 * (q % NG)] = mfma(w0[kk], xq[q & 1][0], acc0[4 * (q % NG)]);
+        __builtin_amdgcn_sched_barrier(0);
+        if (q + 1 < NQ) {
+          read_q(st, q + 1);
+        } else if (next_stage) {
+          read_w(smem + nslot * C::STAGE, w0n, w1n);
+          read_q(smem + nslot * C::STAGE, 0);
+        }
+        __builtin_amdgcn_sched_barrier(0);
+#pragma unroll
+        for (int i = 0; i < 4; ++i) {
+          const int blk = 4 * (q % NG) + i;
+          if (i > 0) acc0[blk] = mfma(w0[kk], xq[q & 1][i], acc0[blk]);
+          acc1[blk] = mfma(w1[kk], xq[q & 1][i], acc1[blk]);
+        }
+#pragma unroll
+        for (int i = 0; i < 4; ++i) {
+          const int blk = 4 * (q % NG) + i;
+          if (blk / SB == u) {
+#pragma unroll
+            for (int e = 0; e < 4; ++e) {
+              const half2v p2 = {xq[q & 1][i][2 * e], xq[q & 1][i][2 * e + 1]};
+              ln_s2[blk % SB] = __builtin_amdgcn_fdot2(p2, p2, ln_s2[blk % SB], false);
+              ln_s1[blk % SB] = __builtin_amdgcn_fdot2(p2, one2, ln_s1[blk % SB], false);
+            }
+          }
+        }
+        __builtin_amdgcn_sched_barrier(0);
+      }
+#pragma unroll
+      for (int kk = 0; kk < 2; ++kk) w0[kk] = w0n[kk], w1[kk] = w1n[kk];
+      slot = nslot;
+    }
+  };
+  if (is_v) k_loop(std::true_type{});
+  else k_loop(std::false_type{});
+  if constexpr (C::EPI == 0) load_epi();
+
+  float2* stat = reinterpret_cast<float2*>(smem + NST * C::STAGE);
+  const float inv_k = 1.0f / (float)a.K;
+#pragma unroll
+  for (int s = 0; s < SB; ++s) {
+    float s1 = ln_s1[s], s2 = ln_s2[s];
+    s1 += __shfl_xor(s1, 16);
+    s2 += __shfl_xor(s2, 16);
+    s1 += __shfl_xor(s1, 32);
+    s2 += __shfl_xor(s2, 32);
+    const float mean = s1 * inv_k;
+    const float var = fmaxf(s2 * inv_k - mean * mean, 0.f);
+    const float la = rsqrtf(var + a.ln_eps);
+    if (u < 4 && g == 0) stat[h * (BM / 2) + 16 * (u * SB + s) + r16] = make_float2(la, -la * mean);
+  }
+  __syncthreads();
+  const float2* hstat = stat + h * (BM / 2);
+  const int m_half = m_blk + h * (BM / 2);
+
+  if (is_v) {
+    const int e4 = r16 & 3;
+    const float c0 = cs0[e4], c1 = cs1[e4], b0 = bias0[e4], b1 = bias1[e4];
+    const int pg = a.vt_perm ? ((0xd8 >> (2 * g)) & 3) : g;
+    const int nv = n_blk - 2 * a.C + 32 * u + r16;
+#pragma unroll
+    for (int i = 0; i < TM; ++i) {
+      const int m16 = m_half + 16 * i;
+      const int b = m16 / a.S, sp = m16 - b * a.S + 4 * pg;
+      half4 o0, o1;
+#pragma unroll
+      for (int e = 0; e < 4; ++e) {
+        const float2 ab = hstat[16 * i + 4 * g + e];
+        o0[e] = (half_t)fmaf(acc0[i][e], ab.x, fmaf(ab.y, c0, b0));
+        o1[e] = (half_t)fmaf(acc1[i][e], ab.x, fmaf(ab.y, c1, b1));
+      }
+      half_t* dst = a.out_vt + ((size_t)b * a.C + nv) * a.ldT + sp;
+      *reinterpret_cast<half4*>(dst) = o0;
+      *reinterpret_cast<half4*>(dst + (size_t)16 * a.ldT) = o1;
+    }
+  } else {
+    const int ldo = 2 * a.C;
+#pragma unroll
+    for (int p = 0; p < TM / 2; ++p) {
+      const int m = m_half + 32 * p + 16 * (g & 1) + r16;
+      const float2 ab0 = hstat[32 * p + r16], ab1 = hstat[32 * p + 16 + r16];
+#pragma unroll
+      for (int j = 0; j < 2; ++j) {
+        const floatx4 cs = j ? cs1 : cs0, bias = j ? bias1 : bias0;
+        uintx2 ho[2];
+#pragma unroll
+        for (int b = 0; b < 2; ++b) {
+          const floatx4 acc = j ? acc1[2 * p + b] : acc0[2 * p + b];
+          const float2 ab = b ? ab1 : ab0;
+          floatx4 o;
+#pragma unroll
+          for (int e = 0; e < 4; ++e) {
+            o[e] = fmaf(acc[e], ab.x, fmaf(ab.y, cs[e], bias[e]));
+            if (q_mul) o[e] *= a.q_scale;
+          }
+          ho[b] = sm_round4(o);
+        }
+        const half8 o8 = sm_pack16(ho[0], ho[1]);
+        const int n = n_blk + 32 * u + 16 * j + 8 * (g >> 1);
+        out_store(reinterpret_cast<half8*>(a.out_qk + (size_t)m * ldo + n), o8);
+      }
+    }
+  }
+}
+
+template <int BM>
+void sq_launch(const SqArgs& a, unsigned nwg, hipStream_t s) {
+  auto k = smqkv_kernel<BM>;
+  static DynLdsOnce once;
+  once.set(k, SqCfg<BM>::LDS);
+  hipLaunchKernelGGL(k, dim3(nwg), dim3(64 * SQ_NW), SqCfg<BM>::LDS, s, a);
+}
+
+}
+
+void launch_smqkv(const ConvDesc& d, const ConvPlan& p, hipStream_t s) {
+  const int bm = p.bm;
+  SD_REQUIRE((bm == 128 || bm == 256) && smqkv_shape_ok(d, bm == 128 ? 1 : 2) && d.x0 && d.w && d.out && d.out_t, kInvalidArgument,
+             "plan tile 23 (smqkv.hip): not a LayerNorm-folded fp16 q|k|v projection it tiles (C0=%d N=%d n_trans=%d M=%d S=%d bm=%d ln=%d)", d.C0,
+             d.N, d.n_trans, d.B * d.Ho * d.Wo, d.Ho * d.Wo, bm, d.ln_colsum ? 1 : 0);
+  const int M = d.B * d.Ho * d.Wo, K = d.C0;
+  SqArgs a;
+  a.x = d.x0;
+  a.w = d.w;
+  a.bias = d.bias;
+  a.colsum = d.ln_colsum;
+  a.out_qk = d.out;
+  a.out_vt = d.out_t;
+  a.K = K;
+  a.nk = K / SQ_BK;
+  a.C = d.C0;
+  a.S = d.Ho * d.Wo;
+  a.ldT = d.ldT;
+  a.vt_perm = d.vt_perm ? 1 : 0;
+  a.q_mul = d.q_cols > 0 ? 1 : 0;
+  a.q_scale = d.q_scale;
+  a.ln_eps = d.ln_eps;
+  a.order = sm_tile_order(M, d.N, K, M / bm, d.N / kSmQkvCols);
+  const unsigned nwg = (unsigned)(M / bm) * (d.N / kSmQkvCols);
+  conv_plan_log(d, p, a.order.n_fast);
+  if (bm == 128) sq_launch<128>(a, nwg, s);
+  else sq_launch<256>(a, nwg, s);
+  SD_HIP(hipGetLastError());
+}
+
+}
diff --git a/ml-stable-diffusion_amd/csrc/unet.cpp b/ml-stable-diffusion_amd/csrc/unet.cpp
--- a/ml-stable-diffusion_amd/csrc/unet.cpp
+++ b/ml-stable-diffusion_amd/csrc/unet.cpp
@@ -222,6 +222,8 @@
     } else {
       LnFold f = fold_layernorm(b + ".norm1", parts, C, C, false);
       qa.ln_colsum = f.colsum;
+      qa.smqkv = true;
+      for (const std::string& part : parts) qa.smqkv = qa.smqkv && !ws_->palette(part + ".weight") && !ws_->w8a8(part + ".weight");
       qk = conv_w(ops, qname, f.w, f.bias, h, qa);
     }
   } else {
@@ -1005,9 +1007,10 @@
   if (sample_scale)
     SD_HIP(hipMemcpyAsync(tab_scale_, sample_scale, (size_t)n_steps * sizeof(float), hipMemcpyHostToDevice, ll_.stream));
   static const bool hoist_off = tune_env_set("SD_NO_TEMB_TABLE");
+  static const bool dup = tune_env_set("SD_TEMB_DUP");
   const bool hoist = !hoist_off && tpath_.ok && temb_w_all_ && temb_used_ > 0 && temb_used_ % 4 == 0;
   if (hoist) {
-    const int Bt = cfg_.batch, rows = n_steps * Bt;
+    const int Bt = cfg_.batch, rows = dup ? n_steps * Bt : n_steps;
     if (temb_tab_cap_ < n_steps) {
       temb_tab_cap_ = std::max(n_steps, 64);
       const size_t r = (size_t)temb_tab_cap_ * Bt;
@@ -1018,19 +1021,28 @@
       emb_tab_ = ll_.arena.alloc_n<float>(r * tpath_.tdim);
       if (loop_graph_) { (void)hipGraphExecDestroy(loop_graph_); loop_graph_ = nullptr; }
     }
-    std::vector<float> tt((size_t)rows);
-    for (int i = 0; i < n_steps; ++i)
-      for (int b = 0; b < Bt; ++b) tt[(size_t)i * Bt + b] = timesteps[i];
-    SD_HIP(hipMemcpyAsync(tt_tab_, tt.data(), tt.size() * sizeof(float), hipMemcpyHostToDevice, ll_.stream));
-    SD_HIP(hipStreamSynchronize(ll_.stream));
+    const float* tt_dev = tab_timesteps_;
+    if (dup) {
+      tt_host_.resize((size_t)rows);
+      for (int i = 0; i < n_steps; ++i)
+        for (int b = 0; b < Bt; ++b) tt_host_[(size_t)i * Bt + b] = timesteps[i];
+      SD_HIP(hipMemcpyAsync(tt_tab_, tt_host_.data(), tt_host_.size() * sizeof(float), hipMemcpyHostToDevice, ll_.stream));
+      tt_dev = tt_tab_;
+    }
     const int c0 = tpath_.c0, td = tpath_.tdim;
-    launch_timestep_embedding(tt_tab_, tpath_.freq, tsin_tab_, rows, c0, ll_.stream);
-    launch_gemv(tpath_.w1, tpath_.b1, tsin_tab_, c0, e1_tab_, td, rows, td, c0, 0, 1, 0, ll_.stream);
-    launch_gemv(tpath_.w2, tpath_.b2, e1_tab_, td, emb_tab_, td, rows, td, td, 0, 0, 0, ll_.stream);
-    launch_gemv(temb_w_all_, temb_b_all_, emb_tab_, td, temb_tab_, kTembCap, rows, temb_used_, td, 1, 0, 0, ll_.stream);
+    launch_timestep_embedding(tt_dev, tpath_.freq, tsin_tab_, rows, c0, ll_.stream);
+    auto gemv = [&](const half_t* w, const float* b, const float* x, int ldx, float* o, int ldo, int N, int K, int si, int so) {
+      for (int r0 = 0; r0 < rows; r0 += dup ? 4 : rows)
+        launch_gemv(w, b, x + (size_t)r0 * ldx, ldx, o + (size_t)r0 * ldo, ldo, std::min(dup ? 4 : rows, rows - r0), N, K, si, so, 0,
+                    ll_.stream);
+    };
+    gemv(tpath_.w1, tpath_.b1, tsin_tab_, c0, e1_tab_, td, td, c0, 0, 1);
+    gemv(tpath_.w2, tpath_.b2, e1_tab_, td, emb_tab_, td, td, td, 0, 0);
+    gemv(temb_w_all_, temb_b_all_, emb_tab_, td, temb_tab_, kTembCap, temb_used_, td, 1, 0);
   }
   LoopTables tab{tab_timesteps_, tab_coef_, step_, sample_scale ? tab_scale_ : nullptr,
-                 reinterpret_cast<unsigned*>(step_ + 1), hoist ? temb_tab_ : nullptr, temb_all_, cfg_.batch, kTembCap, temb_used_};
+                 reinterpret_cast<unsigned*>(step_ + 1), hoist ? temb_tab_ : nullptr, temb_all_, cfg_.batch, kTembCap, temb_used_,
+                 dup ? 1 : 0};
   if (io.step_noise) {
     const size_t need = (size_t)n_steps * lat_n;
     if (noise_cap_ < need) {
diff --git a/ml-stable-diffusion_amd/csrc/unet.h b/ml-stable-diffusion_amd/csrc/unet.h
--- a/ml-stable-diffusion_amd/csrc/unet.h
+++ b/ml-stable-diffusion_amd/csrc/unet.h
@@ -85,6 +85,7 @@
   float* temb_tab_ = nullptr;
   int temb_tab_cap_ = 0;
   float *tt_tab_ = nullptr, *tsin_tab_ = nullptr, *e1_tab_ = nullptr, *emb_tab_ = nullptr;
+  std::vector<float> tt_host_;
   struct TimePath {
     const float* freq = nullptr;
     const half_t *w1 = nullptr, *w2 = nullptr;
diff --git a/ml-stable-diffusion_amd/python_hip_stable_diffusion/_lib.py b/ml-stable-diffusion_amd/python_hip_stable_diffusion/_lib.py
--- a/ml-stable-diffusion_amd/python_hip_stable_diffusion/_lib.py
+++ b/ml-stable-diffusion_amd/python_hip_stable_diffusion/_lib.py
@@ -159,7 +159,7 @@
     ("sd_op_cross_attention_block", _I, [_P, _FP, _FP, _P, _P, _P, _P, _FP, _P, _P, _FP, _P, _I, _I, _I, _I, _F, _I, _I, _FP]),
     ("sd_op_geglu", _I, [_P, _P, _FP, _P, _I, _I, _I, _I, _FP]),
     ("sd_op_geglu_ln", _I, [_P, _FP, _FP, _P, _FP, _P, _I, _I, _I, C.c_float, _I, _I, _FP]),
-    ("sd_op_qkv_ln", _I, [_P, _FP, _FP, _P, _P, _P, _I, _I, _I, C.c_float, C.c_float, _I, _I, _I, _FP]),
+    ("sd_op_qkv_ln", _I, [_P, _FP, _FP, _P, _FP, _P, _P, _I, _I, _I, C.c_float, C.c_float, _I, _I, _I, _FP]),
     ("sd_op_gn_proj_qkv", _I, [_P, _P, _FP, _FP, _P, _FP, _FP, _FP, _P, _P, _P, _P, _I, _I, _I, _I, _I, C.c_float, C.c_float, C.c_float, _I, _I,
                                C.POINTER(C.c_int), _I, _FP]),
     ("sd_op_timestep_embedding", _I, [_FP, _FP, _I, _I, _I, _F]),
@@ -985,15 +985,18 @@
     return out, ms.value
 
 
-def qkv_ln(x, ln_weight, ln_bias, w, batch, q_scale=1.0, vt_perm=True, eps=1e-5, kernel=0, iters=1):
+def qkv_ln(x, ln_weight, ln_bias, w, batch, q_scale=1.0, vt_perm=True, eps=1e-5, kernel=0, iters=1, bias=None):
     x, w = f16(x), f16(w)
     M, Cn = x.shape
     HW = M // batch
+    bias = None if bias is None else f32(bias)
+    if bias is not None and bias.shape != (3 * Cn,):
+        raise ValueError("qkv_ln: bias must be (3C,)")
     out_qk = np.empty((M, 2 * Cn), np.float16)
     out_vt = np.empty((batch, Cn, HW), np.float16)
     ms = C.c_float(0)
-    check(lib().sd_op_qkv_ln(ptr(x), fptr(f32(ln_weight)), fptr(f32(ln_bias)), ptr(w), ptr(out_qk), ptr(out_vt), batch, HW, Cn, eps, q_scale,
-                             int(vt_perm), kernel, iters, C.byref(ms)))
+    check(lib().sd_op_qkv_ln(ptr(x), fptr(f32(ln_weight)), fptr(f32(ln_bias)), ptr(w), fptr(bias), ptr(out_qk), ptr(out_vt), batch, HW, Cn, eps,
+                             q_scale, int(vt_perm), kernel, iters, C.byref(ms)))
     return out_qk, out_vt, ms.value
 
 
```
